# monkey0head/RePlay_cql

Measured on NVIDIA B200. Metric: CQL updates/sec (batch 1024), higher is better.
Workload: dtype f32 (f16x3: tensor-core fp16 hi/lo 3-term split with exact power-of-two row scales, fp32 accumulate, 1e-4 parity-gated)

## Files before the change

### replay_cql_b200/csrc/engine.cuh

```cuda
#pragma once
#include <cstdlib>
#include <vector>
#include <string>
#include "common.cuh"
#include "mlp_simt.cuh"
#include "dp_peer.cuh"
#include <nvtx3/nvToolsExt.h>

namespace cql {

constexpr int N_NOISE_PARTS = 8;

struct StepInfo {
  double bc1, bc2_sqrt;
  long long step;
};

struct NvtxRange {
  explicit NvtxRange(const char* name) { nvtxRangePushA(name); }
  ~NvtxRange() { nvtxRangePop(); }
  NvtxRange(const NvtxRange&) = delete;
  NvtxRange& operator=(const NvtxRange&) = delete;
};

struct Affine {
  int on;
  float off, den;
};
struct Prep {
  Affine obs[2];
  Affine act;
  Affine rew;
  __host__ __device__ bool any() const { return obs[0].on | obs[1].on | act.on | rew.on; }
};
__device__ __forceinline__ float prep_fwd(const Affine& p, float x) {
  return p.on ? __fdiv_rn(__fsub_rn(x, p.off), p.den) : x;
}
__device__ __forceinline__ float act_fwd(const Affine& p, float a) {
  return p.on ? __fsub_rn(__fmul_rn(__fdiv_rn(__fsub_rn(a, p.off), p.den), 2.f), 1.f) : a;
}
__device__ __forceinline__ float act_rev(const Affine& p, float a) {
  return p.on ? __fadd_rn(__fmul_rn(__fdiv_rn(__fadd_rn(a, 1.f), 2.f), p.den), p.off) : a;
}
__device__ __forceinline__ float4 prep_row0(const Prep& p, float4 r) {
  return make_float4(prep_fwd(p.obs[0], r.x), prep_fwd(p.obs[1], r.y), act_fwd(p.act, r.z), prep_fwd(p.rew, r.w));
}
__device__ __forceinline__ float4 prep_row1(const Prep& p, float4 r) {
  return make_float4(prep_fwd(p.obs[0], r.x), prep_fwd(p.obs[1], r.y), r.z, r.w);
}

constexpr int STATS_MAX_BLOCKS = 1024;
constexpr size_t STATS_DEV_DOUBLES = (STATS_MAX_BLOCKS + 1) * 4 * 5;

struct Switches {
  int skip;
  bool no_pdl;
  bool no_pair;
  bool no_pair_bwd1;
  bool no_pair_bwd2;
  bool no_pair_bwd2_small;
  bool no_small;
  bool no_fold;
  bool no_fused_adam;
  bool no_fork;
  int big_fork;
  int h2_cost;
  int pair_swap;
  int dp_debug;
  bool no_fused_dp;
};
inline const Switches& switches() {
  static const Switches s = [] {
    auto set = [](const char* name) { return std::getenv(name) != nullptr; };
    auto num = [](const char* name, int unset) { const char* v = std::getenv(name); return v ? std::atoi(v) : unset; };
    Switches w{};
    w.skip = num("CQL_SKIP", 0);
    w.no_pdl = set("CQL_NO_PDL");
    w.no_pair = set("CQL_NO_PAIR");
    w.no_pair_bwd1 = set("CQL_NO_PAIR_BWD1");
    w.no_pair_bwd2 = set("CQL_NO_PAIR_BWD2");
    w.no_pair_bwd2_small = set("CQL_NO_PAIR_BWD2_SMALL");
    w.no_small = set("CQL_NO_SMALL");
    w.no_fold = set("CQL_NO_FOLD");
    w.no_fused_adam = set("CQL_NO_FUSED_ADAM");
    w.no_fork = set("CQL_NO_FORK");
    w.big_fork = num("CQL_BIG_FORK", -1);
    w.h2_cost = num("CQL_H2_COST", 0);
    w.pair_swap = num("CQL_PAIR_SWAP", 0);
    w.dp_debug = num("CQL_DP_DEBUG", 0);
    w.no_fused_dp = set("CQL_NO_FUSED_DP");
    return w;
  }();
  return s;
}

struct MdpSession;
int64_t seen_csr_on_device(struct Handle& h, const int32_t* users_h, const int32_t* items_h, int64_t n, int64_t n_users,
                           const uint8_t* wanted_h, int64_t* indptr_d, int32_t* seen_d, cudaStream_t st);
void mdp_session_free(MdpSession*);

struct Handle {
  cql_config cfg{};
  std::string err;
  cudaStream_t own_stream = nullptr;
  cudaStream_t side_stream = nullptr;
  cudaEvent_t ev_fork = nullptr, ev_join = nullptr;
  int num_sms = 148;
  int64_t launches = 0;

  float* params = nullptr;
  float* adam_m = nullptr;
  float* adam_v = nullptr;
  float* grads = nullptr;
  long long* step_dev = nullptr;
  StepInfo* stepinfo = nullptr;
  float* metrics = nullptr;
  float* metrics_host = nullptr;

  float* table = nullptr;
  int64_t n_trans = 0;
  int n_steps = 1;
  int64_t table_cap = 0;
  bool table_sharded = false;
  int64_t sample_pos_host = 0;
  long long* sample_pos = nullptr;
  cql_table_stats stats{};
  double* stats_dev = nullptr;
  double* stats_host = nullptr;
  bool stats_pending = false;
  bool stats_rew_ok = false;
  cql_preprocessing prep_cfg{};
  Prep prep{};

  int B = 0, n = 0, C = 0;
  int rsA = 0, rsC = 0;
  float* batch = nullptr;
  float* batch_host = nullptr;
  float* batch_in = nullptr;
  float* noise = nullptr;
  float* noise_host = nullptr;
  int64_t noise_floats = 0;
  float4* XA = nullptr;
  float* outA = nullptr;
  float* h2A = nullptr;
  float4* XAl = nullptr;
  float* offAl = nullptr;
  float* QAl = nullptr;
  float4* XC = nullptr;
  float* offC = nullptr;
  float* QC = nullptr;
  float* h2C = nullptr;
  float* dQ = nullptr;
  float4* XT = nullptr;
  float* QT = nullptr;
  float4* XP = nullptr;
  float* QP = nullptr;
  float* h2P = nullptr;
  float* dQP = nullptr;
  float4* dXP = nullptr;
  float* dOutA = nullptr;
  float* perb = nullptr;
  float* pairv = nullptr;
  float* loss_sums = nullptr;
  float* actor_part = nullptr;
  float* smallC = nullptr;
  float* smallA = nullptr;
  float* pw2C = nullptr;
  float* pw2A = nullptr;
  int splitsC = 1, splitsA = 1;

  uint8_t* packed_fwd = nullptr;
  size_t packed_net_bytes = 0;
  size_t packed_net_bytes_bwd = 0;
  float* part = nullptr;
  size_t part_floats = 0;
  uint8_t* packed_bwd = nullptr;
  float* small1 = nullptr;
  float* small2 = nullptr;
  float* pw2_tc = nullptr;
  float4* dX_part = nullptr;
  int slots1 = 0, splits_tc = 0, tc_slices = 1;
  uint8_t* packed_fwd2 = nullptr;
  uint8_t* packed_bwd2 = nullptr;
  size_t packed_net_bytes2 = 0;
  DpPeer dp;
  bool dp_fused = false;
  int* w2max = nullptr;
  int* ap_wmax = nullptr;
  int pair_swap_b = 0;

  bool timing = false;
  bool pdl_off = false;
  cudaEvent_t ev[16] = {};

  MdpSession* mdp = nullptr;
  uint8_t* mdp_ring = nullptr;
  std::vector<void*> allocs;

  template <typename T>
  T* dalloc(size_t count) {
    void* p = nullptr;
    CQL_CUDA(cudaMalloc(&p, count * sizeof(T)));
    CQL_CUDA(cudaMemset(p, 0, count * sizeof(T)));
    allocs.push_back(p);
    return reinterpret_cast<T*>(p);
  }
  void free_all() {
    for (void* p : allocs) cudaFree(p);
    allocs.clear();
    if (mdp) { mdp_session_free(mdp); mdp = nullptr; }
    if (mdp_ring) { cudaFreeHost(mdp_ring); mdp_ring = nullptr; }
    if (table) { cudaFree(table); table = nullptr; table_cap = 0; }
    if (metrics_host) { cudaFreeHost(metrics_host); metrics_host = nullptr; }
    if (batch_host) { cudaFreeHost(batch_host); batch_host = nullptr; }
    if (stats_host) { cudaFreeHost(stats_host); stats_host = nullptr; }
    if (noise_host) { cudaFreeHost(noise_host); noise_host = nullptr; }
    if (own_stream) { cudaStreamDestroy(own_stream); own_stream = nullptr; }
    if (side_stream) { cudaStreamDestroy(side_stream); side_stream = nullptr; }
    if (ev_fork) { cudaEventDestroy(ev_fork); ev_fork = nullptr; }
    if (ev_join) { cudaEventDestroy(ev_join); ev_join = nullptr; }
    for (auto& e : ev) if (e) { cudaEventDestroy(e); e = nullptr; }
  }

  float* staged_batch() const { return prep.any() ? batch_in : batch; }
  float* net_params(int slot) const { return params + (size_t)slot * NET_STRIDE; }
  float* scalars() const { return params + scalars_off(C); }
  float* g_actor() const { return grads; }
  float* g_critics() const { return grads + NET_STRIDE; }
  float* g_scalars() const { return grads + (size_t)(1 + C) * NET_STRIDE; }
};

void mdp_begin(Handle& h, int64_t n);
void mdp_append(Handle& h, int col, int dtype, const void* host, int64_t count);
int64_t mdp_finish(Handle& h, int top_k, float noise_scale, float* obs_out, float* act_out, float* rew_out, float* term_out,
                   int64_t* order_out);

inline void ensure_table(Handle& h, int64_t n) {
  h.n_trans = 0;
  h.stats = cql_table_stats{};
  h.stats_pending = false;
  if (h.table != nullptr && h.table_cap >= n) return;
  if (h.table) { CQL_CUDA(cudaFree(h.table)); h.table = nullptr; h.table_cap = 0; }
  CQL_CUDA(cudaMalloc(&h.table, (size_t)n * 8 * sizeof(float)));
  h.table_cap = n;
}

void expand_n_steps(Handle& h, const float* one_step, int64_t n, cudaStream_t st);
int table_stats(Handle& h, const float* rows, int64_t n, bool rew_ok, cudaStream_t st);

inline void mark(Handle* h, cudaStream_t st, int i) {
  if (h->timing) CQL_CUDA(cudaEventRecord(h->ev[i], st));
}

inline cudaStream_t pick_stream(Handle* h, void* stream) {
  return stream ? reinterpret_cast<cudaStream_t>(stream) : h->own_stream;
}

#define CQL_LAUNCH_CHECK(h)                 \
  do {                                      \
    (h)->launches++;                        \
    CQL_CUDA(cudaGetLastError());           \
  } while (0)

}
```

### replay_cql_b200/csrc/mlp_tc.cuh

```cuda
#pragma once
#include "tc_common.cuh"
#include "engine.cuh"

namespace cql {
namespace tc {

constexpr int TM = 128;

template <bool TF32>
struct Cfg {
  static constexpr int ES = TF32 ? 4 : 2;
  static constexpr int EPC = 16 / ES;
  static constexpr int UK = 32 / ES;
  static constexpr int TERMS = TF32 ? 2 : 1;
  static constexpr int NS = TF32 ? 64 : 256;
  static constexpr int SLICES = H / NS;
  static constexpr uint32_t B_TERM_BYTES = NS * H * ES;
  static constexpr uint32_t B_BYTES = TERMS * B_TERM_BYTES;
  static constexpr uint32_t TMEM_COLS = 2 * NS < 32 ? 32 : 2 * NS;
  static constexpr size_t PACKED_NET_BYTES = (size_t)SLICES * B_BYTES;
};

template <bool TF32, int NPW>
struct Pipe : Cfg<TF32> {
  using C = Cfg<TF32>;
  static constexpr int KC = TF32 ? 16 : 64;
  static constexpr int STAGES = TF32 ? 5 : 4;
  static constexpr int PIECES = KC / C::EPC;
  static constexpr int GROUPS = NPW / PIECES;
  static constexpr int NCHUNK = H / KC;
  static constexpr uint32_t A_TERM_BYTES = TM * KC * C::ES;
  static constexpr uint32_t A_STAGE_BYTES = C::TERMS * A_TERM_BYTES;
  static constexpr int MMA_WARP = 4 + NPW;
  static constexpr int THREADS = (5 + NPW) * 32;
  static constexpr int PROD_THREADS = NPW * 32;
};
constexpr int FWD_NPW = 16;
constexpr int BWD1_NPW = 8;

template <bool TF32, bool TRANSPOSE>
__global__ void k_pack_w2(const float* __restrict__ params, int in_dim, int n_nets, uint8_t* __restrict__ packed) {
  using C = Cfg<TF32>;
  const int net = blockIdx.y;
  const int c = blockIdx.x * blockDim.x + threadIdx.x;
  if (net >= n_nets || c >= H * (H / C::EPC)) return;
  const int n = c / (H / C::EPC), kc = c % (H / C::EPC);
  const float* W2 = params + (size_t)net * NET_STRIDE + off_W2(in_dim);
  float v[C::EPC];
#pragma unroll
  for (int i = 0; i < C::EPC; ++i) {
    const int k = kc * C::EPC + i;
    v[i] = TRANSPOSE ? W2[(size_t)k * H + n] : W2[(size_t)n * H + k];
  }
  const int slice = n / C::NS, nl = n % C::NS;
  uint8_t* base = packed + (size_t)net * C::PACKED_NET_BYTES + (size_t)slice * C::B_BYTES + chunk_off(C::NS, nl, kc);
  if (TF32) {
    float4 h, l;
    split_tf32(v[0], h.x, l.x); split_tf32(v[1], h.y, l.y); split_tf32(v[2], h.z, l.z); split_tf32(v[3], h.w, l.w);
    *reinterpret_cast<float4*>(base) = h;
    *reinterpret_cast<float4*>(base + C::B_TERM_BYTES) = l;
  } else {
    __nv_bfloat162 p[4];
#pragma unroll
    for (int i = 0; i < 4; ++i) p[i] = __floats2bfloat162_rn(v[2 * i], v[2 * i + 1]);
    *reinterpret_cast<uint4*>(base) = *reinterpret_cast<uint4*>(p);
  }
}

struct PackJobs {
  struct J { const float* net; uint8_t* dst; int in_dim, transpose; } j[12];
  int n;
};
template <bool TF32>
__global__ void k_pack_multi(const PackJobs jobs) {
  using C = Cfg<TF32>;
  const PackJobs::J jb = jobs.j[blockIdx.y];
  const int c = blockIdx.x * blockDim.x + threadIdx.x;
  if (c >= H * (H / C::EPC)) return;
  const int n = c / (H / C::EPC), kc = c % (H / C::EPC);
  const float* W2 = jb.net + off_W2(jb.in_dim);
  float v[C::EPC];
#pragma unroll
  for (int i = 0; i < C::EPC; ++i) {
    const int k = kc * C::EPC + i;
    v[i] = jb.transpose ? W2[(size_t)k * H + n] : W2[(size_t)n * H + k];
  }
  const int slice = n / C::NS, nl = n % C::NS;
  uint8_t* base = jb.dst + (size_t)slice * C::B_BYTES + chunk_off(C::NS, nl, kc);
  if constexpr (TF32) {
    float4 h, l;
    split_tf32(v[0], h.x, l.x); split_tf32(v[1], h.y, l.y); split_tf32(v[2], h.z, l.z); split_tf32(v[3], h.w, l.w);
    *reinterpret_cast<float4*>(base) = h;
    *reinterpret_cast<float4*>(base + C::B_TERM_BYTES) = l;
  } else {
    __nv_bfloat162 p[4];
#pragma unroll
    for (int i = 0; i < 4; ++i) p[i] = __floats2bfloat162_rn(v[2 * i], v[2 * i + 1]);
    *reinterpret_cast<uint4*>(base) = *reinterpret_cast<uint4*>(p);
  }
}

struct TcFwdJob {
  const float4* X;
  const float* params;
  const uint8_t* packed;
  float* out_part;
  float* h2;
  int rows, n_nets;
};
struct TcFwdJobs {
  TcFwdJob j[3];
  int n;
  int item_begin[4];
  int h2_cost = 0;
};

struct ItemInfo { int job, net, slice, tile, pair_id; };

template <bool TF32>
__device__ __forceinline__ ItemInfo decode_item(const TcFwdJobs& jobs, int item) {
  using C = Cfg<TF32>;
  ItemInfo it;
  it.job = 0;
  while (it.job + 1 < jobs.n && item >= jobs.item_begin[it.job + 1]) ++it.job;
  const int local = item - jobs.item_begin[it.job];
  const int tiles = (jobs.j[it.job].rows + TM - 1) / TM;
  const int pair = local / tiles;
  it.tile = local % tiles;
  it.net = pair / C::SLICES;
  it.slice = pair % C::SLICES;
  it.pair_id = it.job * 64 + pair;
  return it;
}

template <bool TF32, int NPW>
struct FwdSmem {
  using C = Pipe<TF32, NPW>;
  static constexpr uint32_t OFF_B = 0;
  static constexpr uint32_t OFF_A = C::B_BYTES;
  static constexpr uint32_t OFF_W1 = OFF_A + C::STAGES * C::A_STAGE_BYTES;
  static constexpr uint32_t OFF_EB = OFF_W1 + H * 16;
  static constexpr uint32_t OFF_BAR = OFF_EB + C::NS * 16;
  static constexpr uint32_t N_BARS = 2 * C::STAGES + 4 + 2;
  static constexpr uint32_t OFF_SLOT = OFF_BAR + N_BARS * 8;
  static constexpr uint32_t BYTES = OFF_SLOT + 16;
};

__device__ __forceinline__ float2 ffma2(float2 a, float2 b, float2 c) {
  float2 d;
  asm("{\n\t.reg .b64 ra, rb, rc, rd;\n\tmov.b64 ra, {%2, %3};\n\tmov.b64 rb, {%4, %5};\n\tmov.b64 rc, {%6, %7};\n\t"
      "fma.rn.f32x2 rd, ra, rb, rc;\n\tmov.b64 {%0, %1}, rd;\n\t}"
      : "=f"(d.x), "=f"(d.y)
      : "f"(a.x), "f"(a.y), "f"(b.x), "f"(b.y), "f"(c.x), "f"(c.y));
  return d;
}
__device__ __forceinline__ void split_tf32_fast(float x, float& hi, float& lo) {
  hi = rn_tf32(x);
  lo = x - hi;
}

template <bool TF32, int IN, int OUT>
__global__ void __launch_bounds__(Pipe<TF32, FWD_NPW>::THREADS, 1) tc_fwd_kernel(const TcFwdJobs jobs) {
  using C = Pipe<TF32, FWD_NPW>;
  using S = FwdSmem<TF32, FWD_NPW>;
  extern __shared__ __align__(1024) uint8_t sm[];
  uint8_t* Bs = sm + S::OFF_B;
  uint8_t* As = sm + S::OFF_A;
  float4* w1s = reinterpret_cast<float4*>(sm + S::OFF_W1);
  float4* ebs = reinterpret_cast<float4*>(sm + S::OFF_EB);
  uint64_t* bars = reinterpret_cast<uint64_t*>(sm + S::OFF_BAR);
  uint64_t* full = bars;
  uint64_t* empty = bars + C::STAGES;
  uint64_t* tfull = bars + 2 * C::STAGES;
  uint64_t* tempty = tfull + 2;
  uint64_t* bload = tempty + 2;
  uint64_t* drain = bload + 1;
  uint32_t* slot = reinterpret_cast<uint32_t*>(sm + S::OFF_SLOT);

  const int tid = threadIdx.x, warp = tid >> 5, lane = tid & 31;
  const int total = jobs.item_begin[jobs.n];
  const int item_lo = (int)((long long)total * blockIdx.x / gridDim.x);
  const int item_hi = (int)((long long)total * (blockIdx.x + 1) / gridDim.x);

  if (warp == C::MMA_WARP) {
    tmem_alloc(slot, C::TMEM_COLS);
    if (lane == 0) {
      for (int s = 0; s < C::STAGES; ++s) { mbar_init(&full[s], C::PIECES); mbar_init(&empty[s], 1); }
      for (int a = 0; a < 2; ++a) { mbar_init(&tfull[a], 1); mbar_init(&tempty[a], 4); }
      mbar_init(bload, 1);
      mbar_init(drain, 1);
      fence_mbar_init();
    }
  }
  tc_fence_before();
  __syncthreads();
  tc_fence_after();
  const uint32_t tmem = *slot;

  if (warp == C::MMA_WARP) {
    {
      const uint32_t idesc = instr_desc(TF32 ? FMT_TF32 : FMT_BF16, TM, C::NS);
      const uint32_t a_lbo = TM * 16, b_lbo = C::NS * 16;
      const uint32_t b_base = smem_u32(Bs);
      int cur_pair = -1;
      uint32_t it = 0, nb = 0, nd = 0, tcount = 0;
      for (int item = item_lo; item < item_hi; ++item) {
        const ItemInfo ii = decode_item<TF32>(jobs, item);
        if (ii.pair_id != cur_pair) {
          if (cur_pair >= 0) {
            if (elect_one()) umma_commit(drain);
            __syncwarp();
            mbar_wait(drain, nd & 1);
            ++nd;
          }
          const TcFwdJob& jb = jobs.j[ii.job];
          const uint8_t* src = jb.packed + (size_t)ii.net * C::PACKED_NET_BYTES + (size_t)ii.slice * C::B_BYTES;
          if (elect_one()) {
            mbar_arrive_expect_tx(bload, C::B_BYTES);
            for (uint32_t o = 0; o < C::B_BYTES; o += 32768) bulk_g2s(Bs + o, src + o, 32768, bload);
          }
          __syncwarp();
          mbar_wait(bload, nb & 1);
          ++nb;
          cur_pair = ii.pair_id;
        }
        const uint32_t acc = tcount & 1;
        mbar_wait(&tempty[acc], ((tcount >> 1) & 1) ^ 1);
        tc_fence_after();
        const uint32_t d_tmem = tmem + acc * C::NS;
        for (int c = 0; c < C::NCHUNK; ++c, ++it) {
          const uint32_t s = it % C::STAGES;
          mbar_wait(&full[s], (it / C::STAGES) & 1);
          tc_fence_after();
          const uint32_t a_base = smem_u32(As + s * C::A_STAGE_BYTES);
          if (elect_one()) {
#pragma unroll
          for (int j = 0; j < C::KC / C::UK; ++j) {
            const uint32_t g = c * (C::KC / C::UK) + j;
            const uint64_t a_hi = smem_desc(a_base + 2 * j * a_lbo, a_lbo, 128);
            const uint64_t b_hi = smem_desc(b_base + 2 * g * b_lbo, b_lbo, 128);
            const uint32_t first = (c == 0 && j == 0) ? 0u : 1u;
            if constexpr (TF32) {
              const uint64_t a_lo = smem_desc(a_base + C::A_TERM_BYTES + 2 * j * a_lbo, a_lbo, 128);
              const uint64_t b_lo = smem_desc(b_base + C::B_TERM_BYTES + 2 * g * b_lbo, b_lbo, 128);
              umma<TF32>(d_tmem, a_lo, b_hi, idesc, first);
              umma<TF32>(d_tmem, a_hi, b_lo, idesc, 1u);
              umma<TF32>(d_tmem, a_hi, b_hi, idesc, 1u);
            } else {
              umma<TF32>(d_tmem, a_hi, b_hi, idesc, first);
            }
          }
          umma_commit(&empty[s]);
          if (c == C::NCHUNK - 1) umma_commit(&tfull[acc]);
          }
          __syncwarp();
        }
        ++tcount;
      }
    }
  } else if (warp >= 4) {
    const int pw = warp - 4, ptid = tid - 128;
    int cur_pair = -1, cur_netkey = -1;
    uint32_t it = 0;
    for (int item = item_lo; item < item_hi; ++item) {
      const ItemInfo ii = decode_item<TF32>(jobs, item);
      const TcFwdJob& jb = jobs.j[ii.job];
      const int netkey = ii.job * 64 + ii.net;
// ... 154 lines not shown
```

### replay_cql_b200/csrc/mlp_tc_bwd1.cuh

```cuda
#pragma once
#include "mlp_tc.cuh"
#include "mlp_tc_ts.cuh"

namespace cql {
namespace tc {

struct Bwd1Job {
  const float4* X;
  const float* dOut;
  const float* h2;
  const float* params;
  const uint8_t* packedT;
  float* small1;
  float4* dX_part;
  int rows, n_nets, slots;
  const float* q_part = nullptr;
  int q_parts = 0;
  float dq_scale = 0.f;
  int zero_small1 = 0;
};
template <int IN>
__device__ __forceinline__ void zero_small1_slots(const Bwd1Job& jb, int per_cta) {
  if (!jb.zero_small1) return;
  constexpr int NF4 = off_W2(IN) / 4;
  for (int net = 0; net < jb.n_nets; ++net)
    for (int s = 0; s < per_cta; ++s) {
      float4* o = reinterpret_cast<float4*>(jb.small1 + ((size_t)net * jb.slots + (size_t)blockIdx.x * per_cta + s) * SMALL_STRIDE);
      for (int f = threadIdx.x; f < NF4; f += blockDim.x) o[f] = make_float4(0.f, 0.f, 0.f, 0.f);
    }
  __syncthreads();
}
template <int IN, int OUT>
__device__ __forceinline__ float actor_dq_of(const Bwd1Job& jb, int net_i, int r) {
  constexpr int MAXP = 8;
  int arg = 0;
  float qm = 0.f;
  for (int c = 0; c < jb.n_nets; ++c) {
    float part[MAXP];
#pragma unroll
    for (int p = 0; p < MAXP; ++p)
      if (p < jb.q_parts) part[p] = __ldg(jb.q_part + ((size_t)c * jb.q_parts + p) * jb.rows + r);
    const float bias = __ldg(jb.params + (size_t)c * NET_STRIDE + off_b3(IN, OUT));
    float v = 0.f;
#pragma unroll
    for (int p = 0; p < MAXP; ++p)
      if (p < jb.q_parts) v += part[p];
    const float q = v + bias;
    if (c == 0 || q < qm) { qm = q; arg = c; }
  }
  return net_i == arg ? jb.dq_scale : 0.f;
}

__device__ __forceinline__ float warp_reduce_scatter32(float (&v)[32]) {
  const int lane = threadIdx.x & 31;
#pragma unroll
  for (int off = 16; off >= 1; off >>= 1) {
    const bool upper = (lane & off) != 0;
#pragma unroll
    for (int i = 0; i < off; ++i) {
      const float send = upper ? v[i] : v[i + off];
      const float keep = upper ? v[i + off] : v[i];
      v[i] = keep + __shfl_xor_sync(0xffffffffu, send, off);
    }
  }
  return v[0];
}

template <bool TF32, int IN, int OUT, bool WGRADS, bool DX>
__global__ void __launch_bounds__(Pipe<TF32, BWD1_NPW>::THREADS, 1) tc_bwd1_kernel(const Bwd1Job jb) {
  using C = Pipe<TF32, BWD1_NPW>;
  using S = FwdSmem<TF32, BWD1_NPW>;
  extern __shared__ __align__(1024) uint8_t sm[];
  uint8_t* Bs = sm + S::OFF_B;
  uint8_t* As = sm + S::OFF_A;
  float2* w3s = reinterpret_cast<float2*>(sm + S::OFF_W1);
  float4* ebs = reinterpret_cast<float4*>(sm + S::OFF_EB);
  uint64_t* bars = reinterpret_cast<uint64_t*>(sm + S::OFF_BAR);
  uint64_t* full = bars;
  uint64_t* empty = bars + C::STAGES;
  uint64_t* tfull = bars + 2 * C::STAGES;
  uint64_t* tempty = tfull + 2;
  uint64_t* bload = tempty + 2;
  uint64_t* drain = bload + 1;
  uint32_t* slot = reinterpret_cast<uint32_t*>(sm + S::OFF_SLOT);

  const int tid = threadIdx.x, warp = tid >> 5, lane = tid & 31;
  const int tiles = (jb.rows + TM - 1) / TM;
  const int tiles64 = (jb.rows + 63) / 64;
  const int total = jb.n_nets * C::SLICES * tiles;
  const int item_lo = (int)((long long)total * blockIdx.x / gridDim.x);
  const int item_hi = (int)((long long)total * (blockIdx.x + 1) / gridDim.x);

  if (warp == C::MMA_WARP) {
    tmem_alloc(slot, C::TMEM_COLS);
    if (lane == 0) {
      for (int s = 0; s < C::STAGES; ++s) { mbar_init(&full[s], C::PIECES); mbar_init(&empty[s], 1); }
      for (int a = 0; a < 2; ++a) { mbar_init(&tfull[a], 1); mbar_init(&tempty[a], 4); }
      mbar_init(bload, 1);
      mbar_init(drain, 1);
      fence_mbar_init();
    }
  }
  tc_fence_before();
  __syncthreads();
  tc_fence_after();
  const uint32_t tmem = *slot;

  if (warp == C::MMA_WARP) {
    {
      const uint32_t idesc = instr_desc(TF32 ? FMT_TF32 : FMT_BF16, TM, C::NS);
      const uint32_t a_lbo = TM * 16, b_lbo = C::NS * 16;
      const uint32_t b_base = smem_u32(Bs);
      int cur_pair = -1;
      uint32_t it = 0, nb = 0, nd = 0, tcount = 0;
      for (int item = item_lo; item < item_hi; ++item) {
        const int pair = item / tiles;
        if (pair != cur_pair) {
          if (cur_pair >= 0) { if (elect_one()) umma_commit(drain); __syncwarp(); mbar_wait(drain, nd & 1); ++nd; }
          const uint8_t* src = jb.packedT + (size_t)(pair / C::SLICES) * C::PACKED_NET_BYTES + (size_t)(pair % C::SLICES) * C::B_BYTES;
          if (elect_one()) {
            mbar_arrive_expect_tx(bload, C::B_BYTES);
            for (uint32_t o = 0; o < C::B_BYTES; o += 32768) bulk_g2s(Bs + o, src + o, 32768, bload);
          }
          __syncwarp();
          mbar_wait(bload, nb & 1);
          ++nb;
          cur_pair = pair;
        }
        const uint32_t acc = tcount & 1;
        mbar_wait(&tempty[acc], ((tcount >> 1) & 1) ^ 1);
        tc_fence_after();
        const uint32_t d_tmem = tmem + acc * C::NS;
        for (int c = 0; c < C::NCHUNK; ++c, ++it) {
          const uint32_t s = it % C::STAGES;
          mbar_wait(&full[s], (it / C::STAGES) & 1);
          tc_fence_after();
          const uint32_t a_base = smem_u32(As + s * C::A_STAGE_BYTES);
          if (elect_one()) {
#pragma unroll
          for (int j = 0; j < C::KC / C::UK; ++j) {
            const uint32_t g = c * (C::KC / C::UK) + j;
            const uint64_t a_hi = smem_desc(a_base + 2 * j * a_lbo, a_lbo, 128);
            const uint64_t b_hi = smem_desc(b_base + 2 * g * b_lbo, b_lbo, 128);
            const uint32_t first = (c == 0 && j == 0) ? 0u : 1u;
            if constexpr (TF32) {
              const uint64_t a_lo = smem_desc(a_base + C::A_TERM_BYTES + 2 * j * a_lbo, a_lbo, 128);
              const uint64_t b_lo = smem_desc(b_base + C::B_TERM_BYTES + 2 * g * b_lbo, b_lbo, 128);
              umma<TF32>(d_tmem, a_lo, b_hi, idesc, first);
              umma<TF32>(d_tmem, a_hi, b_lo, idesc, 1u);
              umma<TF32>(d_tmem, a_hi, b_hi, idesc, 1u);
            } else {
              umma<TF32>(d_tmem, a_hi, b_hi, idesc, first);
            }
          }
          umma_commit(&empty[s]);
          if (c == C::NCHUNK - 1) umma_commit(&tfull[acc]);
          }
          __syncwarp();
        }
        ++tcount;
      }
    }
  } else if (warp >= 4) {
    const int pw = warp - 4, ptid = tid - 128;
    int cur_net = -1;
    uint32_t it = 0;
    for (int item = item_lo; item < item_hi; ++item) {
      const int pair = item / tiles, tile = item % tiles, net_i = pair / C::SLICES;
      if (net_i != cur_net) {
        cur_net = net_i;
        asm volatile("bar.sync 1, %0;" ::"n"(C::PROD_THREADS));
        const float* net = jb.params + (size_t)net_i * NET_STRIDE;
// ... 482 lines not shown
```

### replay_cql_b200/csrc/mlp_tc_bwd2.cuh

```cuda
#pragma once
#include "tc_common.cuh"
#include "mlp_simt.cuh"

namespace cql {
namespace tc {

constexpr int B2_PROD_WARPS = 8;
constexpr int B2_THREADS = (B2_PROD_WARPS + 1) * 32;

template <bool TF32>
struct B2Cfg {
  static constexpr int ES = TF32 ? 4 : 2;
  static constexpr int EPC = 16 / ES;
  static constexpr int UK = 32 / ES;
  static constexpr int TERMS = TF32 ? 2 : 1;
  static constexpr int RS = TF32 ? 16 : 64;
  static constexpr int STAGES = 3;
  static constexpr uint32_t OP_TERM_BYTES = H * RS * ES;
  static constexpr uint32_t OP_BYTES = TERMS * OP_TERM_BYTES;
  static constexpr uint32_t STAGE_BYTES = 2 * OP_BYTES;
  static constexpr uint32_t OFF_X = STAGES * STAGE_BYTES;
  static constexpr uint32_t OFF_DO = OFF_X + STAGES * RS * 16;
  static constexpr uint32_t OFF_BAR = OFF_DO + STAGES * RS * 8;
  static constexpr uint32_t OFF_SLOT = OFF_BAR + (2 * STAGES + 1) * 8;
  static constexpr uint32_t BYTES = OFF_SLOT + 16;
};

struct Bwd2Job {
  const float4* X;
  const float* dOut;
  const float* h2;
  const float* params;
  float* pw2;
  float* small2;
  int rows, n_nets, splits;
};

template <bool TF32, int IN, int OUT>
__global__ void __launch_bounds__(B2_THREADS, 1) tc_bwd2_kernel(const Bwd2Job jb) {
  using C = B2Cfg<TF32>;
  extern __shared__ __align__(1024) uint8_t sm[];
  float4* xs = reinterpret_cast<float4*>(sm + C::OFF_X);
  float* dos = reinterpret_cast<float*>(sm + C::OFF_DO);
  uint64_t* full = reinterpret_cast<uint64_t*>(sm + C::OFF_BAR);
  uint64_t* empty = full + C::STAGES;
  uint64_t* done = empty + C::STAGES;
  uint32_t* slot = reinterpret_cast<uint32_t*>(sm + C::OFF_SLOT);
  const int tid = threadIdx.x, warp = tid >> 5, lane = tid & 31;
  const int split = blockIdx.x, net_i = blockIdx.y;
  const float* net = jb.params + (size_t)net_i * NET_STRIDE;
  const int tiles64 = (jb.rows + 63) / 64;
  const int n_stage_total = (jb.rows + C::RS - 1) / C::RS;
  const int st_lo = (int)((long long)n_stage_total * split / jb.splits);
  const int st_hi = (int)((long long)n_stage_total * (split + 1) / jb.splits);

  if (warp == B2_PROD_WARPS) {
    tmem_alloc(slot, 512);
    if (lane == 0) {
      for (int s = 0; s < C::STAGES; ++s) { mbar_init(&full[s], B2_PROD_WARPS); mbar_init(&empty[s], 1); }
      mbar_init(done, 1);
      fence_mbar_init();
    }
  }
  tc_fence_before();
  __syncthreads();
  tc_fence_after();
  const uint32_t tmem = *slot;

  if (warp == B2_PROD_WARPS) {
    {
      const uint32_t idesc = instr_desc(TF32 ? FMT_TF32 : FMT_BF16, 128, 256);
      const uint32_t lbo = H * 16;
      uint32_t it = 0;
      for (int sg = st_lo; sg < st_hi; ++sg, ++it) {
        const uint32_t s = it % C::STAGES;
        mbar_wait(&full[s], (it / C::STAGES) & 1);
        tc_fence_after();
        const uint32_t a_base = smem_u32(sm + s * C::STAGE_BYTES);
        const uint32_t b_base = a_base + C::OP_BYTES;
        if (elect_one()) {
#pragma unroll
        for (int half = 0; half < 2; ++half) {
#pragma unroll
          for (int j = 0; j < C::RS / C::UK; ++j) {
            const uint32_t acc = (it == 0 && j == 0) ? 0u : 1u;
            const uint64_t a_hi = smem_desc(a_base + half * 2048 + 2 * j * lbo, lbo, 128);
            const uint64_t b_hi = smem_desc(b_base + 2 * j * lbo, lbo, 128);
            const uint32_t d = tmem + half * 256;
            if constexpr (TF32) {
              const uint64_t a_lo = smem_desc(a_base + C::OP_TERM_BYTES + half * 2048 + 2 * j * lbo, lbo, 128);
              const uint64_t b_lo = smem_desc(b_base + C::OP_TERM_BYTES + 2 * j * lbo, lbo, 128);
              umma<TF32>(d, a_lo, b_hi, idesc, acc);
              umma<TF32>(d, a_hi, b_lo, idesc, 1u);
              umma<TF32>(d, a_hi, b_hi, idesc, 1u);
            } else {
              umma<TF32>(d, a_hi, b_hi, idesc, acc);
            }
          }
        }
        umma_commit(&empty[s]);
        if (sg == st_hi - 1) umma_commit(done);
        }
        __syncwarp();
      }
    }
  } else {
    const int t = tid;
    float w3[OUT];
#pragma unroll
    for (int o = 0; o < OUT; ++o) w3[o] = net[off_W3(IN) + o * H + t];
    const float w1x = net[off_W1(IN) + t * IN], w1y = net[off_W1(IN) + t * IN + 1];
    const float w1z = IN == 3 ? net[off_W1(IN) + t * IN + 2] : 0.f;
    const float b1v = net[off_b1(IN) + t];
    float s_db2 = 0.f, s_dw3[OUT], s_db3[OUT];
#pragma unroll
    for (int o = 0; o < OUT; ++o) { s_dw3[o] = 0.f; s_db3[o] = 0.f; }
    uint32_t it = 0;
    constexpr int NV = C::RS / 4;
    constexpr bool PREFETCH = NV <= 4;
    float4 hnext[PREFETCH ? NV : 1];
    auto h2_ptr = [&](int sg) {
      const int row0 = sg * C::RS;
      return jb.h2 + (((size_t)net_i * tiles64 + (row0 >> 6)) * H + t) * 64 + (row0 & 63);
    };
    if (PREFETCH && st_lo < st_hi) {
      const float* hp = h2_ptr(st_lo);
#pragma unroll
      for (int q = 0; q < NV; ++q) hnext[q] = __ldg(reinterpret_cast<const float4*>(hp) + q);
    }
    for (int sg = st_lo; sg < st_hi; ++sg, ++it) {
      const uint32_t s = it % C::STAGES;
      float4 hcur[PREFETCH ? NV : 1];
      if (PREFETCH) {
#pragma unroll
        for (int q = 0; q < NV; ++q) hcur[q] = hnext[q];
        if (sg + 1 < st_hi) {
          const float* hp = h2_ptr(sg + 1);
#pragma unroll
          for (int q = 0; q < NV; ++q) hnext[q] = __ldg(reinterpret_cast<const float4*>(hp) + q);
        }
      }
      mbar_wait(&empty[s], ((it / C::STAGES) & 1) ^ 1);
      const int row0 = sg * C::RS;
      float4* xst = xs + s * C::RS;
      float* dost = dos + s * C::RS * 2;
      if (t < C::RS) {
        const int r = row0 + t;
        xst[t] = r < jb.rows ? __ldg(jb.X + r) : make_float4(0.f, 0.f, 0.f, 0.f);
#pragma unroll
        for (int o = 0; o < OUT; ++o)
          dost[t * 2 + o] = r < jb.rows ? __ldg(jb.dOut + ((size_t)net_i * jb.rows + r) * OUT + o) : 0.f;
      }
      asm volatile("bar.sync 1, 256;");
      uint8_t* Ast = sm + s * C::STAGE_BYTES;
      uint8_t* Bst = Ast + C::OP_BYTES;
      const float* h2p = h2_ptr(sg);
#pragma unroll
      for (int kc = 0; kc < C::RS / C::EPC; ++kc) {
        float hv[C::EPC], dz[C::EPC], h1[C::EPC];
        if constexpr (C::EPC == 8) {
          const float4 p0 = __ldg(reinterpret_cast<const float4*>(h2p + kc * 8));
          const float4 p1 = __ldg(reinterpret_cast<const float4*>(h2p + kc * 8 + 4));
          hv[0] = p0.x; hv[1] = p0.y; hv[2] = p0.z; hv[3] = p0.w;
          hv[4] = p1.x; hv[5] = p1.y; hv[6] = p1.z; hv[7] = p1.w;
        } else {
          const float4 p0 = PREFETCH ? hcur[kc % NV] : __ldg(reinterpret_cast<const float4*>(h2p + kc * 4));
          hv[0] = p0.x; hv[1] = p0.y; hv[2] = p0.z; hv[3] = p0.w;
        }
#pragma unroll
        for (int e = 0; e < C::EPC; ++e) {
          const int rl = kc * C::EPC + e;
          float g = 0.f;
#pragma unroll
          for (int o = 0; o < OUT; ++o) {
            const float d = dost[rl * 2 + o];
            g = fmaf(d, w3[o], g);
            s_dw3[o] = fmaf(d, hv[e], s_dw3[o]);
            if (t == 0) s_db3[o] += d;
          }
          dz[e] = hv[e] > 0.f ? g : 0.f;
          s_db2 += dz[e];
          const float4 x = xst[rl];
          float z = fmaf(x.y, w1y, x.x * w1x);
          if (IN == 3) z = fmaf(x.z, w1z, z);
          h1[e] = fmaxf(z + b1v, 0.f);
        }
        const uint32_t off = chunk_off(H, t, kc);
        if constexpr (TF32) {
// ... 63 lines not shown
```

### replay_cql_b200/csrc/mlp_tc_h.cuh

```cuda
#pragma once
#include <cuda_fp16.h>
#include "mlp_tc.cuh"
#include "mlp_tc_bwd1.cuh"
#include "mlp_tc_bwd2.cuh"

namespace cql {
namespace tc {

template <int NEW_, int NS_ = 128>
struct HCfgT {
  static constexpr int ES = 2, EPC = 8, UK = 16;
  static constexpr int NS = NS_;
  static constexpr int SLICES = H / NS;
  static constexpr int NPW = 16;
  static constexpr int KC = 64;
  static constexpr int STAGES = 4;
  static constexpr int NCHUNK = H / KC;
  static constexpr int KPW = KC / (NPW / 4);
  static constexpr int NEW = NEW_;
  static constexpr int MMA_WARP = NEW + NPW;
  static constexpr int THREADS = (NEW + 1 + NPW) * 32;
  static constexpr int PROD_THREADS = NPW * 32;
  static constexpr uint32_t B_TERM_BYTES = NS * H * ES;
  static constexpr uint32_t B_BYTES = 2 * B_TERM_BYTES;
  static constexpr size_t META_OFF = (size_t)SLICES * B_BYTES;
  static constexpr size_t PACKED_NET_BYTES = META_OFF + 2048;
  static constexpr uint32_t A_COL0 = 256;
  static constexpr uint32_t A_STAGE_COLS = KC;
  static constexpr uint32_t A_LO_COLS = KC / 2;
  static constexpr uint32_t TMEM_ALLOC = 512;
  static constexpr uint32_t OFF_B = 0;
  static constexpr uint32_t OFF_W1 = B_BYTES;
  static constexpr uint32_t OFF_EB = OFF_W1 + H * 16;
  static constexpr uint32_t OFF_BAR = OFF_EB + 2 * NS * 16;
  static constexpr uint32_t N_BARS = 2 * STAGES + 4 + 2;
  static constexpr uint32_t OFF_SLOT = OFF_BAR + N_BARS * 8;
  static constexpr uint32_t OFF_FLUSH = OFF_SLOT + 16;
  static constexpr uint32_t OFF_RED = OFF_FLUSH + 2 * 4 * 16 * 32 * 4;
  static constexpr uint32_t RED_WARP_BYTES = 32 * 33 * 4 + 32 * 16;
  static constexpr uint32_t SMEM_BYTES = OFF_RED + NEW_ * RED_WARP_BYTES;
};
using HCfg = HCfgT<8>;
using HCfgS = HCfgT<8, 32>;
using HCfg4 = HCfgT<4>;

template <class C>
__device__ __forceinline__ void load_operand_slice(uint8_t* Bs, const uint8_t* packed_net, int slice, uint64_t* bar) {
  if constexpr (C::NS == HCfg::NS) {
    const uint8_t* src = packed_net + (size_t)slice * HCfg::B_BYTES;
    mbar_arrive_expect_tx(bar, C::B_BYTES);
    for (uint32_t o = 0; o < C::B_BYTES; o += 32768) bulk_g2s(Bs + o, src + o, 32768, bar);
  } else {
    constexpr int PER = HCfg::NS / C::NS;
    const uint8_t* src = packed_net + (size_t)(slice / PER) * HCfg::B_BYTES + (size_t)(slice % PER) * (C::NS * 16);
    mbar_arrive_expect_tx(bar, C::B_BYTES);
    for (int term = 0; term < 2; ++term)
      for (int kc = 0; kc < H / 8; ++kc)
        bulk_g2s(Bs + term * C::B_TERM_BYTES + kc * (C::NS * 16), src + (size_t)term * HCfg::B_TERM_BYTES + (size_t)kc * (HCfg::NS * 16),
                 C::NS * 16, bar);
  }
}

struct HMeta {
  float inv_s[H];
  float wmax[8];
};

__device__ __forceinline__ void pow2_scale(float bound, float& s, float& inv_s) {
  int e = (int)((__float_as_uint(bound) >> 23) & 0xffu);
  e = max(e, 20);
  s = __uint_as_float((uint32_t)(268 - e) << 23);
  inv_s = __uint_as_float((uint32_t)(e - 14) << 23);
}

__device__ __forceinline__ void split_h2(float x0, float x1, uint32_t& hi, uint32_t& lo) {
  const __half2 h = __floats2half2_rn(x0, x1);
  const float2 hf = __half22float2(h);
  const __half2 l = __floats2half2_rn(x0 - hf.x, x1 - hf.y);
  hi = *reinterpret_cast<const uint32_t*>(&h);
  lo = *reinterpret_cast<const uint32_t*>(&l);
}

__device__ __forceinline__ void split_h2_trunc(float2 x, uint32_t& hi, uint32_t& lo) {
  const float h0 = __uint_as_float(__float_as_uint(x.x) & 0xFFFFE000u);
  const float h1 = __uint_as_float(__float_as_uint(x.y) & 0xFFFFE000u);
  float2 l;
  asm("{\n\t.reg .b64 ra, rb, rd;\n\tmov.b64 ra, {%2, %3};\n\tmov.b64 rb, {%4, %5};\n\t"
      "sub.rn.f32x2 rd, ra, rb;\n\tmov.b64 {%0, %1}, rd;\n\t}"
      : "=f"(l.x), "=f"(l.y)
      : "f"(x.x), "f"(x.y), "f"(h0), "f"(h1));
  const __half2 hh = __floats2half2_rn(h0, h1);
  const __half2 ll = __floats2half2_rn(l.x, l.y);
  hi = *reinterpret_cast<const uint32_t*>(&hh);
  lo = *reinterpret_cast<const uint32_t*>(&ll);
}

__device__ __forceinline__ float2 fmul2(float2 a, float2 b) {
  float2 d;
  asm("{\n\t.reg .b64 ra, rb, rd;\n\tmov.b64 ra, {%2, %3};\n\tmov.b64 rb, {%4, %5};\n\t"
      "mul.rn.f32x2 rd, ra, rb;\n\tmov.b64 {%0, %1}, rd;\n\t}"
      : "=f"(d.x), "=f"(d.y)
      : "f"(a.x), "f"(a.y), "f"(b.x), "f"(b.y));
  return d;
}

__global__ void __launch_bounds__(256) k_pack_multi_h(const PackJobs jobs, int out_dim_actor) {
  tc::grid_dep_wait();
 
  using C = HCfg;
  const PackJobs::J jb = jobs.j[blockIdx.y];
  const int c = blockIdx.x * blockDim.x + threadIdx.x;
  const int n = c >> 5, kc = c & 31;
  const float* W2 = jb.net + off_W2(jb.in_dim);
  float v[8];
  float mx = 0.f;
#pragma unroll
  for (int i = 0; i < 8; ++i) {
    const int k = kc * 8 + i;
    v[i] = jb.transpose ? W2[(size_t)k * H + n] : W2[(size_t)n * H + k];
    mx = fmaxf(mx, fabsf(v[i]));
  }
#pragma unroll
  for (int o = 16; o > 0; o >>= 1) mx = fmaxf(mx, __shfl_xor_sync(0xffffffffu, mx, o));
  float s, inv_s;
  pow2_scale(mx, s, inv_s);
  uint32_t hi[4], lo[4];
#pragma unroll
  for (int i = 0; i < 4; ++i) split_h2(v[2 * i] * s, v[2 * i + 1] * s, hi[i], lo[i]);
  const int slice = n / C::NS, nl = n % C::NS;
  uint8_t* base = jb.dst + (size_t)slice * C::B_BYTES + chunk_off(C::NS, nl, kc);
  *reinterpret_cast<uint4*>(base) = make_uint4(hi[0], hi[1], hi[2], hi[3]);
  *reinterpret_cast<uint4*>(base + C::B_TERM_BYTES) = make_uint4(lo[0], lo[1], lo[2], lo[3]);
  HMeta* meta = reinterpret_cast<HMeta*>(jb.dst + C::META_OFF);
  if (kc == 0) meta->inv_s[n] = inv_s;
  if (blockIdx.x == 0) {
    __shared__ int wm[8];
    if (threadIdx.x < 8) wm[threadIdx.x] = 0;
    __syncthreads();
    const int out_dim = jb.in_dim == 2 ? out_dim_actor : 1;
    const int k = threadIdx.x;
    const float* W1 = jb.net + off_W1(jb.in_dim);
    for (int cc = 0; cc < jb.in_dim; ++cc) atomicMax(&wm[cc], __float_as_int(fabsf(W1[k * jb.in_dim + cc])));
    atomicMax(&wm[3], __float_as_int(fabsf(jb.net[off_b1(jb.in_dim) + k])));
    for (int o = 0; o < out_dim; ++o) atomicMax(&wm[4 + o], __float_as_int(fabsf(jb.net[off_W3(jb.in_dim) + o * H + k])));
    __syncthreads();
    if (threadIdx.x < 8) meta->wmax[threadIdx.x] = __int_as_float(wm[threadIdx.x]);
  }
}

constexpr int FWD_H2_COST = 13;

struct HItem { int job, net, slice, tile, pair_id; };
template <int SLICES = HCfg::SLICES>
__device__ __forceinline__ HItem decode_item_h(const TcFwdJobs& jobs, int item) {
  HItem it;
  it.job = 0;
  while (it.job + 1 < jobs.n && item >= jobs.item_begin[it.job + 1]) ++it.job;
  const int local = item - jobs.item_begin[it.job];
  const int tiles = (jobs.j[it.job].rows + TM - 1) / TM;
  const int pair = local / tiles;
  it.tile = local % tiles;
  it.net = pair / SLICES;
  it.slice = pair % SLICES;
  it.pair_id = it.job * 64 + pair;
  return it;
}

__device__ __forceinline__ float h1_row_bound(const float4& x, const float4& wm) {
  return fmaf(fabsf(x.x), wm.x, fmaf(fabsf(x.y), wm.y, fmaf(fabsf(x.z), wm.z, wm.w)));
}

template <int IN, int OUT, class C = HCfg>
__global__ void __launch_bounds__(HCfg::THREADS, 1) tc_fwd_h_kernel(const TcFwdJobs jobs) {
  extern __shared__ __align__(1024) uint8_t sm[];
  uint8_t* Bs = sm + C::OFF_B;
  float4* w1p = reinterpret_cast<float4*>(sm + C::OFF_W1);
  float4* ebs = reinterpret_cast<float4*>(sm + C::OFF_EB);
  uint64_t* bars = reinterpret_cast<uint64_t*>(sm + C::OFF_BAR);
  uint64_t* full = bars;
  uint64_t* empty = bars + C::STAGES;
  uint64_t* tfull = bars + 2 * C::STAGES;
  uint64_t* tempty = tfull + 2;
  uint64_t* bload = tempty + 2;
  uint64_t* drain = bload + 1;
  uint32_t* slot = reinterpret_cast<uint32_t*>(sm + C::OFF_SLOT);

  const int tid = threadIdx.x, warp = tid >> 5, lane = tid & 31;
  int item_lo, item_hi;
  {
    long long cb[4];
    int wj[3];
    cb[0] = 0;
    for (int j = 0; j < jobs.n; ++j) {
      wj[j] = jobs.j[j].h2 != nullptr ? (jobs.h2_cost > 0 ? jobs.h2_cost : FWD_H2_COST) : 10;
      cb[j + 1] = cb[j] + (long long)(jobs.item_begin[j + 1] - jobs.item_begin[j]) * wj[j];
    }
    auto item_at = [&](long long cost) {
      int j = 0;
      while (j + 1 < jobs.n && cost >= cb[j + 1]) ++j;
      const int it = jobs.item_begin[j] + (int)((cost - cb[j]) / wj[j]);
      return it < jobs.item_begin[j + 1] ? it : jobs.item_begin[j + 1];
    };
    const long long total_cost = cb[jobs.n];
    item_lo = blockIdx.x == 0 ? 0 : item_at(total_cost * blockIdx.x / gridDim.x);
    item_hi = blockIdx.x == gridDim.x - 1 ? jobs.item_begin[jobs.n] : item_at(total_cost * (blockIdx.x + 1) / gridDim.x);
  }

  if (warp == C::MMA_WARP) {
    tmem_alloc(slot, C::TMEM_ALLOC);
    if (lane == 0) {
      for (int s = 0; s < C::STAGES; ++s) { mbar_init(&full[s], C::NPW); mbar_init(&empty[s], 1); }
      for (int a = 0; a < 2; ++a) { mbar_init(&tfull[a], 1); mbar_init(&tempty[a], 4); }
      mbar_init(bload, 1);
      mbar_init(drain, 1);
      fence_mbar_init();
    }
  }
  tc_fence_before();
  __syncthreads();
  tc_fence_after();
  const uint32_t tmem = *slot;
  grid_dep_wait();

  if (warp == C::MMA_WARP) {
    const uint32_t idesc = instr_desc(FMT_F16, TM, C::NS);
    const uint32_t b_lbo = C::NS * 16;
    const uint32_t b_base = smem_u32(Bs);
    int cur_pair = -1;
    uint32_t it = 0, nb = 0, nd = 0, tcount = 0;
    for (int item = item_lo; item < item_hi; ++item) {
      const HItem ii = decode_item_h<C::SLICES>(jobs, item);
      if (ii.pair_id != cur_pair) {
        if (cur_pair >= 0) {
          if (elect_one()) umma_commit(drain);
          __syncwarp();
          mbar_wait(drain, nd & 1);
          ++nd;
        }
        const TcFwdJob& jb = jobs.j[ii.job];
        if (elect_one()) load_operand_slice<C>(Bs, jb.packed + (size_t)ii.net * HCfg::PACKED_NET_BYTES, ii.slice, bload);
        __syncwarp();
        mbar_wait(bload, nb & 1);
        ++nb;
        cur_pair = ii.pair_id;
      }
      const uint32_t acc = tcount & 1;
      mbar_wait(&tempty[acc], ((tcount >> 1) & 1) ^ 1);
      tc_fence_after();
      const uint32_t d_tmem = tmem + acc * C::NS;
      for (int c = 0; c < C::NCHUNK; ++c, ++it) {
        const uint32_t s = it % C::STAGES;
        mbar_wait(&full[s], (it / C::STAGES) & 1);
        tc_fence_after();
        if (elect_one()) {
          const uint32_t a_stage = tmem + C::A_COL0 + s * C::A_STAGE_COLS;
#pragma unroll
          for (int j = 0; j < C::KC / C::UK; ++j) {
            const uint32_t g = c * (C::KC / C::UK) + j;
            const uint64_t b_hi = smem_desc(b_base + 2 * g * b_lbo, b_lbo, 128);
            const uint64_t b_lo = smem_desc(b_base + C::B_TERM_BYTES + 2 * g * b_lbo, b_lbo, 128);
            const uint32_t a_hi = a_stage + j * 8, a_lo = a_hi + C::A_LO_COLS;
            umma_ts<false>(d_tmem, a_lo, b_hi, idesc, (c == 0 && j == 0) ? 0u : 1u);
            umma_ts<false>(d_tmem, a_hi, b_lo, idesc, 1u);
            umma_ts<false>(d_tmem, a_hi, b_hi, idesc, 1u);
          }
          umma_commit(&empty[s]);
          if (c == C::NCHUNK - 1) umma_commit(&tfull[acc]);
        }
        __syncwarp();
      }
      ++tcount;
    }
  } else if (warp >= C::NEW) {
    const int pw = warp - C::NEW, ptid = tid - C::NEW * 32;
    const int kq = pw >> 2;
    const uint32_t lane_base = tmem + ((uint32_t)((warp & 3) * 32) << 16) + C::A_COL0 + kq * (C::KPW / 2);
    int cur_netkey = -1;
    float4 wm = make_float4(0.f, 0.f, 0.f, 0.f);
    uint32_t it = 0;
    auto load_x = [&](const HItem& ni) {
      const TcFwdJob& nj = jobs.j[ni.job];
      const int r = ni.tile * TM + (warp & 3) * 32 + lane;
      return r < nj.rows ? __ldg(nj.X + r) : make_float4(0.f, 0.f, 0.f, 0.f);
    };
    float4 x_next = make_float4(0.f, 0.f, 0.f, 0.f);
    HItem ii_next = item_lo < item_hi ? decode_item_h<C::SLICES>(jobs, item_lo) : HItem{};
    for (int item = item_lo; item < item_hi; ++item) {
      const HItem ii = ii_next;
      if (item + 1 < item_hi) ii_next = decode_item_h<C::SLICES>(jobs, item + 1);
      const TcFwdJob& jb = jobs.j[ii.job];
      const int netkey = ii.job * 64 + ii.net;
      if (netkey != cur_netkey) {
        cur_netkey = netkey;
        asm volatile("bar.sync 1, %0;" ::"n"(C::PROD_THREADS));
        const float* net = jb.params + (size_t)ii.net * NET_STRIDE;
        for (int pr = ptid; pr < H / 2; pr += C::PROD_THREADS) {
          const int k = 2 * pr;
          const float* wa = net + off_W1(IN) + k * IN;
          const float* wb = wa + IN;
          w1p[2 * pr] = make_float4(wa[0], wb[0], wa[1], wb[1]);
          w1p[2 * pr + 1] = make_float4(IN == 3 ? wa[2] : 0.f, IN == 3 ? wb[2] : 0.f, net[off_b1(IN) + k], net[off_b1(IN) + k + 1]);
        }
        const HMeta* meta = reinterpret_cast<const HMeta*>(jb.packed + (size_t)ii.net * HCfg::PACKED_NET_BYTES + HCfg::META_OFF);
        wm = make_float4(__ldg(&meta->wmax[0]), __ldg(&meta->wmax[1]), IN == 3 ? __ldg(&meta->wmax[2]) : 0.f, __ldg(&meta->wmax[3]));
        asm volatile("bar.sync 1, %0;" ::"n"(C::PROD_THREADS));
      }
      const float4 x = (item == item_lo) ? load_x(ii) : x_next;
      if (item + 1 < item_hi) x_next = load_x(ii_next);
      float sa, inv_sa;
      pow2_scale(h1_row_bound(x, wm), sa, inv_sa);
      const float2 xx = make_float2(x.x, x.x), xy = make_float2(x.y, x.y), xz = make_float2(x.z, x.z), ss = make_float2(sa, sa);
      for (int c = 0; c < C::NCHUNK; ++c, ++it) {
        const uint32_t s = it % C::STAGES;
        uint32_t hi[C::KPW / 2], lo[C::KPW / 2];
#pragma unroll
        for (int pp = 0; pp < C::KPW / 2; ++pp) {
          const int pr = (c * C::KC + kq * C::KPW) / 2 + pp;
          const float4 wA = w1p[2 * pr], wB = w1p[2 * pr + 1];
          float2 v = ffma2(xx, make_float2(wA.x, wA.y), make_float2(wB.z, wB.w));
          v = ffma2(xy, make_float2(wA.z, wA.w), v);
          if (IN == 3) v = ffma2(xz, make_float2(wB.x, wB.y), v);
          v = fmul2(make_float2(fmaxf(v.x, 0.f), fmaxf(v.y, 0.f)), ss);
          split_h2_trunc(v, hi[pp], lo[pp]);
        }
        mbar_wait(&empty[s], ((it / C::STAGES) & 1) ^ 1);
        tc_fence_after();
        tmem_st8(lane_base + s * C::A_STAGE_COLS, hi);
        tmem_st8(lane_base + s * C::A_STAGE_COLS + C::A_LO_COLS, lo);
        tmem_st_wait();
        tc_fence_before();
        __syncwarp();
        if (lane == 0) mbar_arrive(&full[s]);
      }
    }
  } else {
    const int grp = warp >> 2, qw = warp & 3, gtid = tid & 127;
    float4* ebg = ebs + grp * C::NS;
    float2* efg = reinterpret_cast<float2*>(sm + C::OFF_FLUSH) + grp * C::NS;
    int cur_pair = -1;
    const int row_in_tile = qw * 32 + lane;
    float4 wm = make_float4(0.f, 0.f, 0.f, 0.f);
    for (int item = item_lo + grp; item < item_hi; item += 2) {
      const uint32_t tcount = (uint32_t)(item - item_lo);
      const HItem ii = decode_item_h<C::SLICES>(jobs, item);
      const TcFwdJob& jb = jobs.j[ii.job];
      if (ii.pair_id != cur_pair) {
        cur_pair = ii.pair_id;
        asm volatile("bar.sync %0, 128;" ::"r"(2 + grp));
        const float* net = jb.params + (size_t)ii.net * NET_STRIDE;
        const HMeta* meta = reinterpret_cast<const HMeta*>(jb.packed + (size_t)ii.net * HCfg::PACKED_NET_BYTES + HCfg::META_OFF);
        for (int cidx = gtid; cidx < C::NS; cidx += 128) {
          const int col = ii.slice * C::NS + cidx;
          const float inv_n = __ldg(&meta->inv_s[col]);
          ebg[cidx] = make_float4(net[off_b2(IN) + col], net[off_W3(IN) + col],
                                  OUT == 2 ? net[off_W3(IN) + H + col] : 0.f, inv_n);
          if (OUT == 1) efg[cidx] = make_float2(net[off_b2(IN) + col] / inv_n, net[off_W3(IN) + col] * inv_n);
        }
        wm = make_float4(__ldg(&meta->wmax[0]), __ldg(&meta->wmax[1]), IN == 3 ? __ldg(&meta->wmax[2]) : 0.f, __ldg(&meta->wmax[3]));
        asm volatile("bar.sync %0, 128;" ::"r"(2 + grp));
      }
      const uint32_t acc = grp;
      const int row = ii.tile * TM + row_in_tile;
      const float4 x = row < jb.rows ? __ldg(jb.X + row) : make_float4(0.f, 0.f, 0.f, 0.f);
      float sa, inv_sa;
      pow2_scale(h1_row_bound(x, wm), sa, inv_sa);
      mbar_wait(&tfull[acc], (tcount >> 1) & 1);
      tc_fence_after();
      const bool store_h2 = jb.h2 != nullptr;
      const int tiles64 = (jb.rows + 63) / 64;
      float* h2row = store_h2 ? jb.h2 + (((size_t)ii.net * tiles64 + (row >> 6)) * H + ii.slice * C::NS) * 64 + (row & 63)
                              : nullptr;
      float q0 = 0.f, q1 = 0.f;
      if (OUT == 1 && !store_h2) {
#pragma unroll 1
        for (int c0 = 0; c0 < C::NS; c0 += 32) {
          float v[32];
          tmem_ld32(tmem + ((uint32_t)(qw * 32) << 16) + acc * C::NS + c0, v);
          tmem_ld_wait();
#pragma unroll
          for (int i = 0; i < 32; i += 2) {
            const float4 e = reinterpret_cast<const float4*>(efg)[(c0 + i) >> 1];
            q0 = fmaf(fmaxf(fmaf(v[i], inv_sa, e.x), 0.f), e.y, q0);
            q0 = fmaf(fmaxf(fmaf(v[i + 1], inv_sa, e.z), 0.f), e.w, q0);
          }
        }
      } else
#pragma unroll 1
      for (int c0 = 0; c0 < C::NS; c0 += 32) {
        float v[32];
        tmem_ld32(tmem + ((uint32_t)(qw * 32) << 16) + acc * C::NS + c0, v);
        tmem_ld_wait();
#pragma unroll
        for (int i = 0; i < 32; ++i) {
          const float4 e = ebg[c0 + i];
          const float hv = fmaxf(fmaf(v[i] * inv_sa, e.w, e.x), 0.f);
          v[i] = hv;
          q0 = fmaf(hv, e.y, q0);
          if (OUT == 2) q1 = fmaf(hv, e.z, q1);
        }
        if (store_h2 && (row >> 6) < tiles64) {
#pragma unroll
          for (int i = 0; i < 32; ++i) h2row[(size_t)(c0 + i) * 64] = v[i];
        }
      }
      tc_fence_before();
      __syncwarp();
      if (lane == 0) mbar_arrive(&tempty[acc]);
      if (row < jb.rows) {
        float* o = jb.out_part + (((size_t)ii.net * C::SLICES + ii.slice) * jb.rows + row) * OUT;
        o[0] = q0;
        if (OUT == 2) o[1] = q1;
      }
    }
  }
  tc_fence_before();
  __syncthreads();
  if (warp == C::MMA_WARP) tmem_dealloc(tmem, C::TMEM_ALLOC);
}


template <int IN, int OUT, bool WGRADS, bool DX, class C = HCfg>
__global__ void __launch_bounds__(HCfg::THREADS, 1) tc_bwd1_h_kernel(const Bwd1Job jb) {
  extern __shared__ __align__(1024) uint8_t sm[];
  uint8_t* Bs = sm + C::OFF_B;
  float2* w3s = reinterpret_cast<float2*>(sm + C::OFF_W1);
  float4* ebs = reinterpret_cast<float4*>(sm + C::OFF_EB);
  float* invs = reinterpret_cast<float*>(sm + C::OFF_W1 + H * 8);
  uint64_t* bars = reinterpret_cast<uint64_t*>(sm + C::OFF_BAR);
  uint64_t* full = bars;
  uint64_t* empty = bars + C::STAGES;
  uint64_t* tfull = bars + 2 * C::STAGES;
  uint64_t* tempty = tfull + 2;
  uint64_t* bload = tempty + 2;
  uint64_t* drain = bload + 1;
  uint32_t* slot = reinterpret_cast<uint32_t*>(sm + C::OFF_SLOT);

  const int tid = threadIdx.x, warp = tid >> 5, lane = tid & 31;
  const int tiles = (jb.rows + TM - 1) / TM;
  const int tiles64 = (jb.rows + 63) / 64;
  const int total = jb.n_nets * C::SLICES * tiles;
  const int item_lo = (int)((long long)total * blockIdx.x / gridDim.x);
  const int item_hi = (int)((long long)total * (blockIdx.x + 1) / gridDim.x);

  if (warp == C::MMA_WARP) {
    tmem_alloc(slot, C::TMEM_ALLOC);
    if (lane == 0) {
      for (int s = 0; s < C::STAGES; ++s) { mbar_init(&full[s], C::NPW); mbar_init(&empty[s], 1); }
      for (int q = 0; q < 2; ++q) { mbar_init(&tfull[q], 1); mbar_init(&tempty[q], 4); }
      mbar_init(bload, 1);
      mbar_init(drain, 1);
      fence_mbar_init();
    }
  }
  tc_fence_before();
  __syncthreads();
  tc_fence_after();
  const uint32_t tmem = *slot;
  grid_dep_wait();
  if (WGRADS) zero_small1_slots<IN>(jb, 2);

  if (warp == C::MMA_WARP) {
    const uint32_t idesc = instr_desc(FMT_F16, TM, C::NS);
    const uint32_t b_lbo = C::NS * 16;
    const uint32_t b_base = smem_u32(Bs);
    int cur_pair = -1;
    uint32_t it = 0, nb = 0, nd = 0, tcount = 0;
    for (int item = item_lo; item < item_hi; ++item) {
      const int pair = item / tiles;
      if (pair != cur_pair) {
        if (cur_pair >= 0) { if (elect_one()) umma_commit(drain); __syncwarp(); mbar_wait(drain, nd & 1); ++nd; }
        if (elect_one()) load_operand_slice<C>(Bs, jb.packedT + (size_t)(pair / C::SLICES) * HCfg::PACKED_NET_BYTES, pair % C::SLICES, bload);
        __syncwarp();
        mbar_wait(bload, nb & 1);
        ++nb;
        cur_pair = pair;
      }
      const uint32_t acc = tcount & 1;
      mbar_wait(&tempty[acc], ((tcount >> 1) & 1) ^ 1);
      tc_fence_after();
      const uint32_t d_tmem = tmem + acc * C::NS;
      for (int c = 0; c < C::NCHUNK; ++c, ++it) {
        const uint32_t s = it % C::STAGES;
        mbar_wait(&full[s], (it / C::STAGES) & 1);
        tc_fence_after();
        if (elect_one()) {
          const uint32_t a_stage = tmem + C::A_COL0 + s * C::A_STAGE_COLS;
#pragma unroll
          for (int j = 0; j < C::KC / C::UK; ++j) {
            const uint32_t g = c * (C::KC / C::UK) + j;
            const uint64_t b_hi = smem_desc(b_base + 2 * g * b_lbo, b_lbo, 128);
            const uint64_t b_lo = smem_desc(b_base + C::B_TERM_BYTES + 2 * g * b_lbo, b_lbo, 128);
            const uint32_t a_hi = a_stage + j * 8, a_lo = a_hi + C::A_LO_COLS;
            umma_ts<false>(d_tmem, a_lo, b_hi, idesc, (c == 0 && j == 0) ? 0u : 1u);
            umma_ts<false>(d_tmem, a_hi, b_lo, idesc, 1u);
            umma_ts<false>(d_tmem, a_hi, b_hi, idesc, 1u);
          }
          umma_commit(&empty[s]);
          if (c == C::NCHUNK - 1) umma_commit(&tfull[acc]);
        }
        __syncwarp();
      }
      ++tcount;
    }
  } else if (warp >= C::NEW) {
    const int pw = warp - C::NEW, ptid = tid - C::NEW * 32;
    const int kq = pw >> 2;
    const uint32_t lane_base = tmem + ((uint32_t)((warp & 3) * 32) << 16) + C::A_COL0 + kq * (C::KPW / 2);
    int cur_net = -1;
    float w3m0 = 0.f, w3m1 = 0.f;
    uint32_t it = 0;
    for (int item = item_lo; item < item_hi; ++item) {
      const int pair = item / tiles, tile = item % tiles, net_i = pair / C::SLICES;
      if (net_i != cur_net) {
        cur_net = net_i;
        asm volatile("bar.sync 1, %0;" ::"n"(C::PROD_THREADS));
        const float* net = jb.params + (size_t)net_i * NET_STRIDE;
        for (int j = ptid; j < H; j += C::PROD_THREADS)
          w3s[j] = make_float2(net[off_W3(IN) + j], OUT == 2 ? net[off_W3(IN) + H + j] : 0.f);
        const HMeta* meta = reinterpret_cast<const HMeta*>(jb.packedT + (size_t)net_i * HCfg::PACKED_NET_BYTES + HCfg::META_OFF);
        w3m0 = __ldg(&meta->wmax[4]);
        w3m1 = OUT == 2 ? __ldg(&meta->wmax[5]) : 0.f;
        asm volatile("bar.sync 1, %0;" ::"n"(C::PROD_THREADS));
      }
      const int r = tile * TM + (warp & 3) * 32 + lane;
      const bool ok = r < jb.rows;
      float d0 = 0.f;
      if (OUT == 1 && DX && !WGRADS && jb.q_parts > 0) { if (ok) d0 = actor_dq_of<IN, OUT>(jb, net_i, r); }
      else if (ok) d0 = __ldg(jb.dOut + ((size_t)net_i * jb.rows + r) * OUT);
      const float d1 = (ok && OUT == 2) ? __ldg(jb.dOut + ((size_t)net_i * jb.rows + r) * OUT + 1) : 0.f;
      float sa, inv_sa;
      pow2_scale(fmaf(fabsf(d0), w3m0, fabsf(d1) * w3m1), sa, inv_sa);
      const float d0s = d0 * sa, d1s = d1 * sa;
      const int rc = ok ? r : 0;
      const float* h2r = jb.h2 + ((size_t)net_i * tiles64 + (rc >> 6)) * H * 64 + (rc & 63);
      float hn[C::KPW];
#pragma unroll
      for (int e = 0; e < C::KPW; ++e) hn[e] = __ldg(h2r + (size_t)(kq * C::KPW + e) * 64);
      for (int c = 0; c < C::NCHUNK; ++c, ++it) {
        const uint32_t s = it % C::STAGES;
        const int j0 = c * C::KC + kq * C::KPW;
        float hv[C::KPW];
#pragma unroll
        for (int e = 0; e < C::KPW; ++e) hv[e] = hn[e];
        if (c + 1 < C::NCHUNK) {
#pragma unroll
          for (int e = 0; e < C::KPW; ++e) hn[e] = __ldg(h2r + (size_t)(j0 + C::KC + e) * 64);
        }
        uint32_t hi[C::KPW / 2], lo[C::KPW / 2];
#pragma unroll
        for (int e = 0; e < C::KPW; e += 2) {
          const float2 wa = w3s[j0 + e], wb = w3s[j0 + e + 1];
          float ga = d0s * wa.x, gb = d0s * wb.x;
          if (OUT == 2) { ga = fmaf(d1s, wa.y, ga); gb = fmaf(d1s, wb.y, gb); }
          split_h2_trunc(make_float2(hv[e] > 0.f ? ga : 0.f, hv[e + 1] > 0.f ? gb : 0.f), hi[e / 2], lo[e / 2]);
        }
        mbar_wait(&empty[s], ((it / C::STAGES) & 1) ^ 1);
        tc_fence_after();
        tmem_st8(lane_base + s * C::A_STAGE_COLS, hi);
        tmem_st8(lane_base + s * C::A_STAGE_COLS + C::A_LO_COLS, lo);
        tmem_st_wait();
        tc_fence_before();
        __syncwarp();
        if (lane == 0) mbar_arrive(&full[s]);
      }
    }
  } else {
    constexpr int NCH = C::NS / 32;
    const int grp = warp >> 2, qw = warp & 3, gtid = tid & 127;
    float4* ebg = ebs + grp * C::NS;
    float* ivg = invs + grp * C::NS;
    float a_b[NCH], a_w0[NCH], a_w1[NCH], a_w2[NCH];
#pragma unroll
    for (int q = 0; q < NCH; ++q) { a_b[q] = 0.f; a_w0[q] = 0.f; a_w1[q] = 0.f; a_w2[q] = 0.f; }
    float* flbuf = reinterpret_cast<float*>(sm + C::OFF_FLUSH) + grp * (4 * 16 * 32);
    float* red_t = reinterpret_cast<float*>(sm + C::OFF_RED + warp * C::RED_WARP_BYTES);
    float4* red_x = reinterpret_cast<float4*>(red_t + 32 * 33);
    auto flush = [&](int pair) {
      if (!WGRADS || pair < 0) return;
      const int net_i = pair / C::SLICES, slice = pair % C::SLICES;
#pragma unroll
      for (int q = 0; q < NCH; ++q) {
        float* f = flbuf + (qw * 16 + q * 4) * 32 + lane;
        f[0] = a_w0[q]; f[32] = a_w1[q]; f[64] = a_w2[q]; f[96] = a_b[q];
        a_b[q] = 0.f; a_w0[q] = 0.f; a_w1[q] = 0.f; a_w2[q] = 0.f;
      }
      asm volatile("bar.sync %0, 128;" ::"r"(2 + grp));
      float* o = jb.small1 + ((size_t)net_i * jb.slots + blockIdx.x * 2 + grp) * SMALL_STRIDE;
      if (qw < NCH) {
        const int q = qw;
        float t0 = 0.f, t1 = 0.f, t2 = 0.f, t3 = 0.f;
#pragma unroll
        for (int w = 0; w < 4; ++w) {
          const float* f = flbuf + (w * 16 + q * 4) * 32 + lane;
          t0 += f[0]; t1 += f[32]; t2 += f[64]; t3 += f[96];
        }
        const int k = slice * C::NS + q * 32 + lane;
        o[k * IN + 0] = t0;
        o[k * IN + 1] = t1;
        if (IN == 3) o[k * IN + 2] = t2;
        o[H * IN + k] = t3;
      }
      asm volatile("bar.sync %0, 128;" ::"r"(2 + grp));
    };
    int cur_pair = -1;
    float w3m0 = 0.f, w3m1 = 0.f;
    for (int item = item_lo + grp; item < item_hi; item += 2) {
      const uint32_t tcount = (uint32_t)(item - item_lo);
      const int pair = item / tiles, tile = item % tiles, net_i = pair / C::SLICES, slice = pair % C::SLICES;
      if (pair != cur_pair) {
        flush(cur_pair);
        cur_pair = pair;
        asm volatile("bar.sync %0, 128;" ::"r"(2 + grp));
        const float* net = jb.params + (size_t)net_i * NET_STRIDE;
        const HMeta* meta = reinterpret_cast<const HMeta*>(jb.packedT + (size_t)net_i * HCfg::PACKED_NET_BYTES + HCfg::META_OFF);
        for (int cidx = gtid; cidx < C::NS; cidx += 128) {
          const int k = slice * C::NS + cidx;
          ebg[cidx] = make_float4(net[off_W1(IN) + k * IN], net[off_W1(IN) + k * IN + 1],
                                  IN == 3 ? net[off_W1(IN) + k * IN + 2] : 0.f, net[off_b1(IN) + k]);
          ivg[cidx] = __ldg(&meta->inv_s[k]);
        }
        w3m0 = __ldg(&meta->wmax[4]);
        w3m1 = OUT == 2 ? __ldg(&meta->wmax[5]) : 0.f;
        asm volatile("bar.sync %0, 128;" ::"r"(2 + grp));
      }
      const uint32_t acc = grp;
      const int row = tile * TM + qw * 32 + lane;
      const bool ok = row < jb.rows;
      const float4 x = ok ? __ldg(jb.X + row) : make_float4(0.f, 0.f, 0.f, 0.f);
      float d0 = 0.f;
      if (OUT == 1 && DX && !WGRADS && jb.q_parts > 0) { if (ok) d0 = actor_dq_of<IN, OUT>(jb, net_i, row); }
      else if (ok) d0 = __ldg(jb.dOut + ((size_t)net_i * jb.rows + row) * OUT);
      const float d1 = (ok && OUT == 2) ? __ldg(jb.dOut + ((size_t)net_i * jb.rows + row) * OUT + 1) : 0.f;
      float sa, inv_sa;
      pow2_scale(fmaf(fabsf(d0), w3m0, fabsf(d1) * w3m1), sa, inv_sa);
      if (WGRADS) {
        __syncwarp();
        red_x[lane] = x;
      }
      mbar_wait(&tfull[acc], (tcount >> 1) & 1);
      tc_fence_after();
      float dx0 = 0.f, dx1 = 0.f, dx2 = 0.f;
#pragma unroll
      for (int q = 0; q < NCH; ++q) {
        float v[32];
        tmem_ld32(tmem + ((uint32_t)(qw * 32) << 16) + acc * C::NS + q * 32, v);
        tmem_ld_wait();
#pragma unroll
        for (int i = 0; i < 32; ++i) {
          const float4 w = ebg[q * 32 + i];
          float z = fmaf(x.y, w.y, fmaf(x.x, w.x, w.w));
          if (IN == 3) z = fmaf(x.z, w.z, z);
          const float d = z > 0.f ? (DX ? v[i] * inv_sa * ivg[q * 32 + i] : v[i] * inv_sa) : 0.f;
          v[i] = d;
          if (DX) {
            dx0 = fmaf(d, w.x, dx0);
            dx1 = fmaf(d, w.y, dx1);
            if (IN == 3) dx2 = fmaf(d, w.z, dx2);
          }
        }
        if (WGRADS) {
          __syncwarp();
#pragma unroll
          for (int i = 0; i < 32; ++i) red_t[lane * 33 + i] = v[i];
          __syncwarp();
          float s0 = 0.f, s1 = 0.f, s2 = 0.f, sb = 0.f;
#pragma unroll 8
          for (int r = 0; r < 32; ++r) {
            const float dv = red_t[r * 33 + lane];
            const float4 xr = red_x[r];
            s0 = fmaf(dv, xr.x, s0);
            s1 = fmaf(dv, xr.y, s1);
            if (IN == 3) s2 = fmaf(dv, xr.z, s2);
            sb += dv;
          }
// ... 285 lines not shown
```

### replay_cql_b200/csrc/mlp_tc_h2.cuh

```cuda
#pragma once
#include "mlp_tc_h.cuh"

namespace cql {
namespace tc {

__device__ __forceinline__ uint32_t cluster_ctarank() {
  uint32_t r;
  asm volatile("mov.u32 %0, %%cluster_ctarank;" : "=r"(r));
  return r;
}
__device__ __forceinline__ void cluster_sync_all() {
  asm volatile("barrier.cluster.arrive.release.aligned;" ::: "memory");
  asm volatile("barrier.cluster.wait.acquire.aligned;" ::: "memory");
}
__device__ __forceinline__ void mbar_arrive_cluster(uint64_t* bar, uint32_t cta) {
  asm volatile(
      "{\n\t.reg .b32 ra;\n\tmapa.shared::cluster.u32 ra, %0, %1;\n\t"
      "mbarrier.arrive.shared::cluster.b64 _, [ra];\n\t}" ::"r"(smem_u32(bar)),
      "r"(cta)
      : "memory");
}
__device__ __forceinline__ void mbar_wait_cluster(uint64_t* bar, uint32_t parity) { mbar_wait(bar, parity); }
__device__ __forceinline__ void tmem_alloc2(uint32_t* smem_slot, uint32_t ncols) {
  asm volatile("tcgen05.alloc.cta_group::2.sync.aligned.shared::cta.b32 [%0], %1;" ::"r"(smem_u32(smem_slot)), "r"(ncols)
// ... 29 lines not shown
  asm("cvt.rn.relu.f16x2.f32 %0, %1, %2;" : "=r"(lo) : "f"(l.y), "f"(l.x));
}

struct H2Cfg {
  static constexpr int NPW = 16, NEW = 8;
  static constexpr int KC = 64, STAGES = 4, NCHUNK = H / KC, UK = 16;
  static constexpr int KPW = KC / (NPW / 4);
  static constexpr int NP = 128;
  static constexpr int NLOC = NP / 2;
  static constexpr int PASSES = H / NP;
  static constexpr int PARTS = 2 * PASSES;
  static constexpr int TMP = 2 * TM;
  static constexpr int MMA_WARP = NEW + NPW;
  static constexpr int THREADS = (NEW + NPW + 1) * 32;
  static constexpr int PROD_THREADS = NPW * 32;
  static constexpr uint32_t B_TERM_BYTES = NLOC * H * 2;
  static constexpr uint32_t B_PASS_BYTES = 2 * B_TERM_BYTES;
  static constexpr uint32_t B_BYTES = PASSES * B_PASS_BYTES;
  static constexpr size_t META_OFF = 2 * (size_t)B_BYTES;
  static constexpr size_t PACKED_NET_BYTES = META_OFF + 2048;
  static constexpr uint32_t A_COL0 = 256, A_STAGE_COLS = KC, A_LO_COLS = KC / 2;
  static constexpr uint32_t OFF_B = 0;
  static constexpr uint32_t OFF_W1 = B_BYTES;
  static constexpr uint32_t OFF_EB = OFF_W1 + H * 16;
  static constexpr uint32_t OFF_EF = OFF_EB + PASSES * NP * 16;
  static constexpr uint32_t OFF_BAR = OFF_EF + PASSES * NP * 8;
  static constexpr uint32_t N_BARS = 2 * STAGES + 2 + 2 + 3;
  static constexpr uint32_t OFF_SLOT = OFF_BAR + N_BARS * 8;
  static constexpr uint32_t SMEM_BYTES = OFF_SLOT + 16;
};

__host__ __device__ constexpr size_t pair_chunk_off(int n, int kc, int term) {
  return (size_t)((n & 127) >> 6) * H2Cfg::B_BYTES + (size_t)(n >> 7) * H2Cfg::B_PASS_BYTES +
         (size_t)term * H2Cfg::B_TERM_BYTES + chunk_off(H2Cfg::NLOC, n & 63, kc);
}

__global__ void __launch_bounds__(256) k_pack_pair_h(const PackJobs jobs, int out_dim_actor) {
  grid_dep_wait();
  using C = H2Cfg;
  const PackJobs::J jb = jobs.j[blockIdx.y];
  const int c = blockIdx.x * blockDim.x + threadIdx.x;
  const int n = c >> 5, kc = c & 31;
  const float* W2 = jb.net + off_W2(jb.in_dim);
  float v[8];
  float mx = 0.f;
#pragma unroll
  for (int i = 0; i < 8; ++i) {
    const int k = kc * 8 + i;
    v[i] = jb.transpose ? W2[(size_t)k * H + n] : W2[(size_t)n * H + k];
    mx = fmaxf(mx, fabsf(v[i]));
  }
#pragma unroll
  for (int o = 16; o > 0; o >>= 1) mx = fmaxf(mx, __shfl_xor_sync(0xffffffffu, mx, o));
  float s, inv_s;
  pow2_scale(mx, s, inv_s);
  uint32_t hi[4], lo[4];
#pragma unroll
  for (int i = 0; i < 4; ++i) split_h2(v[2 * i] * s, v[2 * i + 1] * s, hi[i], lo[i]);
  *reinterpret_cast<uint4*>(jb.dst + pair_chunk_off(n, kc, 0)) = make_uint4(hi[0], hi[1], hi[2], hi[3]);
  *reinterpret_cast<uint4*>(jb.dst + pair_chunk_off(n, kc, 1)) = make_uint4(lo[0], lo[1], lo[2], lo[3]);
  HMeta* meta = reinterpret_cast<HMeta*>(jb.dst + C::META_OFF);
  if (kc == 0) meta->inv_s[n] = inv_s;
  if (blockIdx.x == 0) {
    __shared__ int wm[8];
    if (threadIdx.x < 8) wm[threadIdx.x] = 0;
    __syncthreads();
    const int out_dim = jb.in_dim == 2 ? out_dim_actor : 1;
    const int k = threadIdx.x;
    const float* W1 = jb.net + off_W1(jb.in_dim);
    for (int cc = 0; cc < jb.in_dim; ++cc) atomicMax(&wm[cc], __float_as_int(fabsf(W1[k * jb.in_dim + cc])));
    atomicMax(&wm[3], __float_as_int(fabsf(jb.net[off_b1(jb.in_dim) + k])));
    for (int o = 0; o < out_dim; ++o) atomicMax(&wm[4 + o], __float_as_int(fabsf(jb.net[off_W3(jb.in_dim) + o * H + k])));
    __syncthreads();
    if (threadIdx.x < 8) meta->wmax[threadIdx.x] = __int_as_float(wm[threadIdx.x]);
  }
}

struct H2Item { int job, net, tp, netkey; };
__device__ __forceinline__ int pair_tiles(int rows) { return (rows + H2Cfg::TMP - 1) / H2Cfg::TMP; }
__device__ __forceinline__ H2Item decode_item_h2(const TcFwdJobs& jobs, const int* pbeg, int item) {
  H2Item it;
  it.job = 0;
  while (it.job + 1 < jobs.n && item >= pbeg[it.job + 1]) ++it.job;
  const int local = item - pbeg[it.job];
  const int tiles = pair_tiles(jobs.j[it.job].rows);
  it.net = local / tiles;
  it.tp = local % tiles;
  it.netkey = it.job * 64 + it.net;
  return it;
}

template <int IN, int OUT>
__global__ void __cluster_dims__(2, 1, 1) __launch_bounds__(H2Cfg::THREADS, 1) tc_fwd_h2_kernel(const TcFwdJobs jobs, int swap_b) {
  using C = H2Cfg;
  extern __shared__ __align__(1024) uint8_t sm[];
  uint8_t* Bs = sm + C::OFF_B;
  float4* w1p = reinterpret_cast<float4*>(sm + C::OFF_W1);
  float4* ebs = reinterpret_cast<float4*>(sm + C::OFF_EB);
  float2* efs = reinterpret_cast<float2*>(sm + C::OFF_EF);
  uint64_t* bars = reinterpret_cast<uint64_t*>(sm + C::OFF_BAR);
  uint64_t* full = bars;
  uint64_t* empty = bars + C::STAGES;
  uint64_t* tfull = bars + 2 * C::STAGES;
  uint64_t* tempty = tfull + 2;
  uint64_t* bload = tempty + 2;
  uint64_t* bready = bload + 1;
  uint64_t* drain = bready + 1;
  uint32_t* slot = reinterpret_cast<uint32_t*>(sm + C::OFF_SLOT);

  const int tid = threadIdx.x, warp = tid >> 5, lane = tid & 31;
  const uint32_t rank = cluster_ctarank();
  const bool leader = rank == 0;
  const int cluster_id = blockIdx.x >> 1, n_clusters = gridDim.x >> 1;

  int pbeg[4];
  int item_lo, item_hi;
  {
    long long cb[4];
    int wj[3];
    cb[0] = 0;
    pbeg[0] = 0;
    for (int j = 0; j < jobs.n; ++j) {
      pbeg[j + 1] = pbeg[j] + jobs.j[j].n_nets * pair_tiles(jobs.j[j].rows);
      wj[j] = jobs.j[j].h2 != nullptr ? (jobs.h2_cost > 0 ? jobs.h2_cost : FWD_H2_COST) : 10;
      cb[j + 1] = cb[j] + (long long)(pbeg[j + 1] - pbeg[j]) * wj[j];
    }
    auto item_at = [&](long long cost) {
      int j = 0;
      while (j + 1 < jobs.n && cost >= cb[j + 1]) ++j;
      const int it = pbeg[j] + (int)((cost - cb[j]) / wj[j]);
      return it < pbeg[j + 1] ? it : pbeg[j + 1];
    };
    const long long total_cost = cb[jobs.n];
    item_lo = cluster_id == 0 ? 0 : item_at(total_cost * cluster_id / n_clusters);
    item_hi = cluster_id == n_clusters - 1 ? pbeg[jobs.n] : item_at(total_cost * (cluster_id + 1) / n_clusters);
  }

  if (warp == C::MMA_WARP) {
    tmem_alloc2(slot, 512);
    if (lane == 0) {
      for (int s = 0; s < C::STAGES; ++s) { mbar_init(&full[s], 2 * C::NPW); mbar_init(&empty[s], 1); }
      for (int a = 0; a < 2; ++a) { mbar_init(&tfull[a], 1); mbar_init(&tempty[a], 2 * C::NEW); }
      mbar_init(bload, 1);
      mbar_init(bready, 2);
      mbar_init(drain, 1);
      fence_mbar_init();
    }
  }
  tc_fence_before();
  __syncthreads();
  cluster_sync_all();
  tc_fence_after();
  const uint32_t tmem = *slot;
  grid_dep_wait();

  if (warp == C::MMA_WARP) {
    const uint32_t idesc = instr_desc(FMT_F16, C::TMP, C::NP);
    const uint32_t b_lbo = C::NLOC * 16;
    const uint32_t b_base = smem_u32(Bs);
    int cur_key = -1;
    uint32_t nb = 0, nd = 0, tcount = 0;
    for (int item = item_lo; item < item_hi; ++item) {
      const H2Item ii = decode_item_h2(jobs, pbeg, item);
      if (ii.netkey != cur_key) {
        if (cur_key >= 0) {
          if (leader && elect_one()) umma_commit2(drain, 3);
          __syncwarp();
          mbar_wait_cluster(drain, nd & 1);
          ++nd;
        }
        const TcFwdJob& jb = jobs.j[ii.job];
        const uint8_t* src = jb.packed + (size_t)ii.net * C::PACKED_NET_BYTES + (size_t)(rank ^ (uint32_t)swap_b) * C::B_BYTES;
        if (elect_one()) {
          mbar_arrive_expect_tx(bload, C::B_BYTES);
          for (uint32_t o = 0; o < C::B_BYTES; o += 32768) bulk_g2s(Bs + o, src + o, 32768, bload);
        }
        __syncwarp();
        mbar_wait(bload, nb & 1);
        if (elect_one()) mbar_arrive_cluster(bready, 0);
        __syncwarp();
        if (leader) mbar_wait_cluster(bready, nb & 1);
        ++nb;
        cur_key = ii.netkey;
      }
      if (!leader) continue;
      for (int p = 0; p < C::PASSES; ++p) {
        mbar_wait_cluster(&tempty[p], (tcount & 1) ^ 1);
        tc_fence_after();
        const uint32_t d_tmem = tmem + p * C::NP;
        const uint32_t bp = b_base + p * C::B_PASS_BYTES;
        for (int c = 0; c < C::NCHUNK; ++c) {
          if (p == 0) {
            mbar_wait_cluster(&full[c], tcount & 1);
            tc_fence_after();
          }
          if (elect_one()) {
            const uint32_t a_stage = tmem + C::A_COL0 + c * C::A_STAGE_COLS;
#pragma unroll
            for (int j = 0; j < C::KC / C::UK; ++j) {
              const uint32_t g = c * (C::KC / C::UK) + j;
              const uint64_t b_hi = smem_desc(bp + 2 * g * b_lbo, b_lbo, 128);
              const uint64_t b_lo = smem_desc(bp + C::B_TERM_BYTES + 2 * g * b_lbo, b_lbo, 128);
              const uint32_t a_hi = a_stage + j * 8, a_lo = a_hi + C::A_LO_COLS;
              umma_ts2(d_tmem, a_lo, b_hi, idesc, (c == 0 && j == 0) ? 0u : 1u);
              umma_ts2(d_tmem, a_hi, b_lo, idesc, 1u);
              umma_ts2(d_tmem, a_hi, b_hi, idesc, 1u);
            }
            if (p == C::PASSES - 1) umma_commit2(&empty[c], 3);
            if (c == C::NCHUNK - 1) umma_commit2(&tfull[p], 3);
          }
          __syncwarp();
        }
      }
      ++tcount;
    }
  } else if (warp >= C::NEW) {
    const int pw = warp - C::NEW, ptid = tid - C::NEW * 32;
    const int kq = pw >> 2;
    const uint32_t lane_base = tmem + ((uint32_t)((warp & 3) * 32) << 16) + C::A_COL0 + kq * (C::KPW / 2);
    int cur_key = -1;
    float4 wm = make_float4(0.f, 0.f, 0.f, 0.f);
    uint32_t tcount = 0;
    auto load_x = [&](const H2Item& ni) {
      const TcFwdJob& nj = jobs.j[ni.job];
      const int r = ni.tp * C::TMP + (int)rank * TM + (warp & 3) * 32 + lane;
      return r < nj.rows ? __ldg(nj.X + r) : make_float4(0.f, 0.f, 0.f, 0.f);
    };
    float4 x_next = make_float4(0.f, 0.f, 0.f, 0.f);
    H2Item ii_next = item_lo < item_hi ? decode_item_h2(jobs, pbeg, item_lo) : H2Item{};
    for (int item = item_lo; item < item_hi; ++item, ++tcount) {
      const H2Item ii = ii_next;
      if (item + 1 < item_hi) ii_next = decode_item_h2(jobs, pbeg, item + 1);
      const TcFwdJob& jb = jobs.j[ii.job];
      if (ii.netkey != cur_key) {
        cur_key = ii.netkey;
        asm volatile("bar.sync 1, %0;" ::"n"(C::PROD_THREADS));
        const float* net = jb.params + (size_t)ii.net * NET_STRIDE;
        for (int pr = ptid; pr < H / 2; pr += C::PROD_THREADS) {
          const int k = 2 * pr;
          const float* wa = net + off_W1(IN) + k * IN;
          const float* wb = wa + IN;
          w1p[2 * pr] = make_float4(wa[0], wb[0], wa[1], wb[1]);
          w1p[2 * pr + 1] = make_float4(IN == 3 ? wa[2] : 0.f, IN == 3 ? wb[2] : 0.f, net[off_b1(IN) + k], net[off_b1(IN) + k + 1]);
        }
        const HMeta* meta = reinterpret_cast<const HMeta*>(jb.packed + (size_t)ii.net * C::PACKED_NET_BYTES + C::META_OFF);
        wm = make_float4(__ldg(&meta->wmax[0]), __ldg(&meta->wmax[1]), IN == 3 ? __ldg(&meta->wmax[2]) : 0.f, __ldg(&meta->wmax[3]));
        asm volatile("bar.sync 1, %0;" ::"n"(C::PROD_THREADS));
      }
      const float4 x = (item == item_lo) ? load_x(ii) : x_next;
      if (item + 1 < item_hi) x_next = load_x(ii_next);
      float sa, inv_sa;
      pow2_scale(h1_row_bound(x, wm), sa, inv_sa);
      const float2 xx = make_float2(x.x, x.x), xy = make_float2(x.y, x.y), xz = make_float2(x.z, x.z), ss = make_float2(sa, sa);
      for (int c = 0; c < C::NCHUNK; ++c) {
        uint32_t hi[C::KPW / 2], lo[C::KPW / 2];
#pragma unroll
        for (int pp = 0; pp < C::KPW / 2; ++pp) {
          const int pr = (c * C::KC + kq * C::KPW) / 2 + pp;
          const float4 wA = w1p[2 * pr], wB = w1p[2 * pr + 1];
          float2 v = ffma2(xx, make_float2(wA.x, wA.y), make_float2(wB.z, wB.w));
          v = ffma2(xy, make_float2(wA.z, wA.w), v);
          if (IN == 3) v = ffma2(xz, make_float2(wB.x, wB.y), v);
          split_h2_trunc_relu(fmul2(v, ss), hi[pp], lo[pp]);
        }
        mbar_wait_cluster(&empty[c], (tcount & 1) ^ 1);
        tc_fence_after();
        tmem_st8(lane_base + c * C::A_STAGE_COLS, hi);
        tmem_st8(lane_base + c * C::A_STAGE_COLS + C::A_LO_COLS, lo);
        tmem_st_wait();
        tc_fence_before();
        __syncwarp();
        if (lane == 0) mbar_arrive_cluster(&full[c], 0);
      }
    }
    if (item_hi > item_lo)
      for (int c = 0; c < C::NCHUNK; ++c) mbar_wait_cluster(&empty[c], (tcount & 1) ^ 1);
  } else {
    const int hh = warp >> 2, qw = warp & 3;
    int cur_key = -1;
    const int row_in_tile = (int)rank * TM + qw * 32 + lane;
    float4 wm = make_float4(0.f, 0.f, 0.f, 0.f);
    uint32_t tcount = 0;
    for (int item = item_lo; item < item_hi; ++item, ++tcount) {
      const H2Item ii = decode_item_h2(jobs, pbeg, item);
      const TcFwdJob& jb = jobs.j[ii.job];
      if (ii.netkey != cur_key) {
        cur_key = ii.netkey;
        asm volatile("bar.sync 2, 256;");
        const float* net = jb.params + (size_t)ii.net * NET_STRIDE;
        const HMeta* meta = reinterpret_cast<const HMeta*>(jb.packed + (size_t)ii.net * C::PACKED_NET_BYTES + C::META_OFF);
        {
          const int col = tid;
          const float inv_n = __ldg(&meta->inv_s[col]);
          ebs[col] = make_float4(net[off_b2(IN) + col], net[off_W3(IN) + col],
                                 OUT == 2 ? net[off_W3(IN) + H + col] : 0.f, inv_n);
          if (OUT == 1) {
            float* ef = reinterpret_cast<float*>(efs) + (col >> 1) * 4 + (col & 1);
            ef[0] = net[off_b2(IN) + col] / inv_n;
            ef[2] = net[off_W3(IN) + col] * inv_n;
          }
        }
        wm = make_float4(__ldg(&meta->wmax[0]), __ldg(&meta->wmax[1]), IN == 3 ? __ldg(&meta->wmax[2]) : 0.f, __ldg(&meta->wmax[3]));
        asm volatile("bar.sync 2, 256;");
      }
      const int row = ii.tp * C::TMP + row_in_tile;
      const float4 x = row < jb.rows ? __ldg(jb.X + row) : make_float4(0.f, 0.f, 0.f, 0.f);
      float sa, inv_sa;
      pow2_scale(h1_row_bound(x, wm), sa, inv_sa);
      const bool store_h2 = jb.h2 != nullptr;
      const int tiles64 = (jb.rows + 63) / 64;
#pragma unroll 1
      for (int p = 0; p < C::PASSES; ++p) {
        constexpr int NC = C::NP / 2;
        const int cb = p * C::NP + hh * NC;
        mbar_wait(&tfull[p], tcount & 1);
        tc_fence_after();
        float* h2row = store_h2 ? jb.h2 + (((size_t)ii.net * tiles64 + (row >> 6)) * H + cb) * 64 + (row & 63) : nullptr;
        const uint32_t t_acc = tmem + ((uint32_t)(qw * 32) << 16) + cb;
        float q0 = 0.f, q1 = 0.f;
        if (OUT == 1 && !store_h2) {
          const float2 isa2 = make_float2(inv_sa, inv_sa);
          const float4* ef4 = reinterpret_cast<const float4*>(efs) + (cb >> 1);
          float2 qa = make_float2(0.f, 0.f), qb = make_float2(0.f, 0.f);
#pragma unroll 1
          for (int c0 = 0; c0 < NC; c0 += 16) {
            float v[16];
            float4 e[8];
            tmem_ld16(t_acc + c0, v);
#pragma unroll
            for (int j = 0; j < 8; ++j) e[j] = ef4[(c0 >> 1) + j];
            tmem_ld_wait();
#pragma unroll
            for (int j = 0; j < 8; j += 2) {
              float2 ha = ffma2(make_float2(v[2 * j], v[2 * j + 1]), isa2, make_float2(e[j].x, e[j].y));
              float2 hb = ffma2(make_float2(v[2 * j + 2], v[2 * j + 3]), isa2, make_float2(e[j + 1].x, e[j + 1].y));
              ha.x = fmaxf(ha.x, 0.f); ha.y = fmaxf(ha.y, 0.f);
              hb.x = fmaxf(hb.x, 0.f); hb.y = fmaxf(hb.y, 0.f);
              qa = ffma2(ha, make_float2(e[j].z, e[j].w), qa);
              qb = ffma2(hb, make_float2(e[j + 1].z, e[j + 1].w), qb);
            }
          }
          q0 = (qa.x + qa.y) + (qb.x + qb.y);
        } else {
          const float4* ebg = ebs + cb;
          float q0b = 0.f, q1b = 0.f;
#pragma unroll 1
          for (int c0 = 0; c0 < NC; c0 += 8) {
            float v[8];
            float4 e[8];
            tmem_ld8(t_acc + c0, v);
#pragma unroll
            for (int i = 0; i < 8; ++i) e[i] = ebg[c0 + i];
            tmem_ld_wait();
#pragma unroll
            for (int i = 0; i < 8; i += 2) {
              const float ha = fmaxf(fmaf(v[i] * inv_sa, e[i].w, e[i].x), 0.f);
              const float hb = fmaxf(fmaf(v[i + 1] * inv_sa, e[i + 1].w, e[i + 1].x), 0.f);
              v[i] = ha;
              v[i + 1] = hb;
              q0 = fmaf(ha, e[i].y, q0);
              q0b = fmaf(hb, e[i + 1].y, q0b);
              if (OUT == 2) { q1 = fmaf(ha, e[i].z, q1); q1b = fmaf(hb, e[i + 1].z, q1b); }
            }
            if (store_h2 && (row >> 6) < tiles64) {
#pragma unroll
              for (int i = 0; i < 8; ++i) h2row[(size_t)(c0 + i) * 64] = v[i];
            }
          }
          q0 += q0b;
          q1 += q1b;
        }
        tc_fence_before();
        __syncwarp();
        if (lane == 0) mbar_arrive_cluster(&tempty[p], 0);
        if (row < jb.rows) {
          float* o = jb.out_part + (((size_t)ii.net * C::PARTS + p * 2 + hh) * jb.rows + row) * OUT;
          o[0] = q0;
          if (OUT == 2) o[1] = q1;
        }
      }
    }
  }
  tc_fence_before();
  __syncthreads();
  cluster_sync_all();
  if (warp == C::MMA_WARP) tmem_dealloc2(tmem, 512);
}


struct H2B1Cfg : H2Cfg {
  static constexpr uint32_t OFF_W3 = B_BYTES;
  static constexpr uint32_t OFF_EB = OFF_W3 + H * 8;
  static constexpr uint32_t OFF_IV = OFF_EB + PASSES * NP * 16;
  static constexpr uint32_t OFF_BAR = OFF_IV + PASSES * NP * 4;
  static constexpr uint32_t OFF_SLOT = OFF_BAR + 128;
  static constexpr uint32_t OFF_FLUSH = OFF_SLOT + 16;
  static constexpr uint32_t OFF_RED = OFF_FLUSH + 2 * 4 * 16 * 32 * 4;
  static constexpr int RED_LD = 34;
  static constexpr uint32_t RED_WARP_BYTES = 32 * RED_LD * 4 + 32 * 16;
  static constexpr uint32_t SMEM_BYTES = OFF_RED + NEW * RED_WARP_BYTES;
};

template <int IN, int OUT, bool WGRADS, bool DX>
__global__ void __cluster_dims__(2, 1, 1) __launch_bounds__(H2Cfg::THREADS, 1) tc_bwd1_h2_kernel(const Bwd1Job jb, int swap_b) {
  using C = H2B1Cfg;
  extern __shared__ __align__(1024) uint8_t sm[];
  uint8_t* Bs = sm + C::OFF_B;
  float2* w3s = reinterpret_cast<float2*>(sm + C::OFF_W3);
  float4* ebs = reinterpret_cast<float4*>(sm + C::OFF_EB);
  float* invs = reinterpret_cast<float*>(sm + C::OFF_IV);
  uint64_t* bars = reinterpret_cast<uint64_t*>(sm + C::OFF_BAR);
  uint64_t* full = bars;
  uint64_t* empty = bars + C::STAGES;
  uint64_t* tfull = bars + 2 * C::STAGES;
  uint64_t* tempty = tfull + 2;
  uint64_t* bload = tempty + 2;
  uint64_t* bready = bload + 1;
  uint64_t* drain = bready + 1;
  uint32_t* slot = reinterpret_cast<uint32_t*>(sm + C::OFF_SLOT);

  const int tid = threadIdx.x, warp = tid >> 5, lane = tid & 31;
  const uint32_t rank = cluster_ctarank();
  const bool leader = rank == 0;
  const int cluster_id = blockIdx.x >> 1, n_clusters = gridDim.x >> 1;
  const int tiles = pair_tiles(jb.rows);
  const int tiles64 = (jb.rows + 63) / 64;
  const int total = jb.n_nets * tiles;
  const int item_lo = (int)((long long)total * cluster_id / n_clusters);
  const int item_hi = (int)((long long)total * (cluster_id + 1) / n_clusters);

  if (warp == C::MMA_WARP) {
    tmem_alloc2(slot, 512);
    if (lane == 0) {
      for (int s = 0; s < C::STAGES; ++s) { mbar_init(&full[s], 2 * C::NPW); mbar_init(&empty[s], 1); }
      for (int a = 0; a < 2; ++a) { mbar_init(&tfull[a], 1); mbar_init(&tempty[a], 2 * C::NEW); }
      mbar_init(bload, 1);
      mbar_init(bready, 2);
      mbar_init(drain, 1);
      fence_mbar_init();
    }
  }
  tc_fence_before();
  __syncthreads();
  cluster_sync_all();
  tc_fence_after();
  const uint32_t tmem = *slot;
  grid_dep_wait();
  if (WGRADS) zero_small1_slots<IN>(jb, 2);

  if (warp == C::MMA_WARP) {
    const uint32_t idesc = instr_desc(FMT_F16, C::TMP, C::NP);
    const uint32_t b_lbo = C::NLOC * 16;
    const uint32_t b_base = smem_u32(Bs);
    int cur_net = -1;
    uint32_t nb = 0, nd = 0, tcount = 0;
    for (int item = item_lo; item < item_hi; ++item) {
      const int net_i = item / tiles;
      if (net_i != cur_net) {
        if (cur_net >= 0) {
          if (leader && elect_one()) umma_commit2(drain, 3);
          __syncwarp();
          mbar_wait_cluster(drain, nd & 1);
          ++nd;
        }
        const uint8_t* src = jb.packedT + (size_t)net_i * C::PACKED_NET_BYTES + (size_t)(rank ^ (uint32_t)swap_b) * C::B_BYTES;
        if (elect_one()) {
          mbar_arrive_expect_tx(bload, C::B_BYTES);
          for (uint32_t o = 0; o < C::B_BYTES; o += 32768) bulk_g2s(Bs + o, src + o, 32768, bload);
        }
        __syncwarp();
        mbar_wait(bload, nb & 1);
        if (elect_one()) mbar_arrive_cluster(bready, 0);
        __syncwarp();
        if (leader) mbar_wait_cluster(bready, nb & 1);
        ++nb;
        cur_net = net_i;
      }
      if (!leader) continue;
      for (int p = 0; p < C::PASSES; ++p) {
        mbar_wait_cluster(&tempty[p], (tcount & 1) ^ 1);
        tc_fence_after();
        const uint32_t d_tmem = tmem + p * C::NP;
        const uint32_t bp = b_base + p * C::B_PASS_BYTES;
        for (int c = 0; c < C::NCHUNK; ++c) {
          if (p == 0) {
            mbar_wait_cluster(&full[c], tcount & 1);
            tc_fence_after();
          }
          if (elect_one()) {
            const uint32_t a_stage = tmem + C::A_COL0 + c * C::A_STAGE_COLS;
#pragma unroll
            for (int j = 0; j < C::KC / C::UK; ++j) {
              const uint32_t g = c * (C::KC / C::UK) + j;
              const uint64_t b_hi = smem_desc(bp + 2 * g * b_lbo, b_lbo, 128);
              const uint64_t b_lo = smem_desc(bp + C::B_TERM_BYTES + 2 * g * b_lbo, b_lbo, 128);
              const uint32_t a_hi = a_stage + j * 8, a_lo = a_hi + C::A_LO_COLS;
              umma_ts2(d_tmem, a_lo, b_hi, idesc, (c == 0 && j == 0) ? 0u : 1u);
              umma_ts2(d_tmem, a_hi, b_lo, idesc, 1u);
              umma_ts2(d_tmem, a_hi, b_hi, idesc, 1u);
            }
            if (p == C::PASSES - 1) umma_commit2(&empty[c], 3);
            if (c == C::NCHUNK - 1) umma_commit2(&tfull[p], 3);
          }
          __syncwarp();
        }
      }
      ++tcount;
    }
  } else if (warp >= C::NEW) {
    const int pw = warp - C::NEW, ptid = tid - C::NEW * 32;
    const int kq = pw >> 2;
    const uint32_t lane_base = tmem + ((uint32_t)((warp & 3) * 32) << 16) + C::A_COL0 + kq * (C::KPW / 2);
    int cur_net = -1;
    float w3m0 = 0.f, w3m1 = 0.f;
    uint32_t tcount = 0;
    for (int item = item_lo; item < item_hi; ++item, ++tcount) {
      const int net_i = item / tiles, tp = item % tiles;
      if (net_i != cur_net) {
        cur_net = net_i;
        asm volatile("bar.sync 1, %0;" ::"n"(C::PROD_THREADS));
        const float* net = jb.params + (size_t)net_i * NET_STRIDE;
        for (int j = ptid; j < H; j += C::PROD_THREADS)
          w3s[j] = make_float2(net[off_W3(IN) + j], OUT == 2 ? net[off_W3(IN) + H + j] : 0.f);
        const HMeta* meta = reinterpret_cast<const HMeta*>(jb.packedT + (size_t)net_i * C::PACKED_NET_BYTES + C::META_OFF);
        w3m0 = __ldg(&meta->wmax[4]);
        w3m1 = OUT == 2 ? __ldg(&meta->wmax[5]) : 0.f;
        asm volatile("bar.sync 1, %0;" ::"n"(C::PROD_THREADS));
      }
      const int r = tp * C::TMP + (int)rank * TM + (warp & 3) * 32 + lane;
      const bool ok = r < jb.rows;
      float d0 = 0.f;
      if (OUT == 1 && DX && !WGRADS && jb.q_parts > 0) { if (ok) d0 = actor_dq_of<IN, OUT>(jb, net_i, r); }
      else if (ok) d0 = __ldg(jb.dOut + ((size_t)net_i * jb.rows + r) * OUT);
      const float d1 = (ok && OUT == 2) ? __ldg(jb.dOut + ((size_t)net_i * jb.rows + r) * OUT + 1) : 0.f;
      float sa, inv_sa;
      pow2_scale(fmaf(fabsf(d0), w3m0, fabsf(d1) * w3m1), sa, inv_sa);
      const float d0s = d0 * sa, d1s = d1 * sa;
      const int rc = ok ? r : 0;
      const float* h2r = jb.h2 + ((size_t)net_i * tiles64 + (rc >> 6)) * H * 64 + (rc & 63);
      float hn[C::KPW];
#pragma unroll
      for (int e = 0; e < C::KPW; ++e) hn[e] = __ldg(h2r + (size_t)(kq * C::KPW + e) * 64);
      for (int c = 0; c < C::NCHUNK; ++c) {
        const int j0 = c * C::KC + kq * C::KPW;
        float hv[C::KPW];
#pragma unroll
        for (int e = 0; e < C::KPW; ++e) hv[e] = hn[e];
        if (c + 1 < C::NCHUNK) {
#pragma unroll
          for (int e = 0; e < C::KPW; ++e) hn[e] = __ldg(h2r + (size_t)(j0 + C::KC + e) * 64);
        }
        uint32_t hi[C::KPW / 2], lo[C::KPW / 2];
#pragma unroll
        for (int e = 0; e < C::KPW; e += 2) {
          const float2 wa = w3s[j0 + e], wb = w3s[j0 + e + 1];
          float ga = d0s * wa.x, gb = d0s * wb.x;
          if (OUT == 2) { ga = fmaf(d1s, wa.y, ga); gb = fmaf(d1s, wb.y, gb); }
          split_h2_trunc(make_float2(hv[e] > 0.f ? ga : 0.f, hv[e + 1] > 0.f ? gb : 0.f), hi[e / 2], lo[e / 2]);
        }
        mbar_wait_cluster(&empty[c], (tcount & 1) ^ 1);
        tc_fence_after();
        tmem_st8(lane_base + c * C::A_STAGE_COLS, hi);
        tmem_st8(lane_base + c * C::A_STAGE_COLS + C::A_LO_COLS, lo);
        tmem_st_wait();
        tc_fence_before();
        __syncwarp();
        if (lane == 0) mbar_arrive_cluster(&full[c], 0);
      }
    }
    if (item_hi > item_lo)
      for (int c = 0; c < C::NCHUNK; ++c) mbar_wait_cluster(&empty[c], (tcount & 1) ^ 1);
  } else {
    constexpr int NC = C::NP / 2;
    constexpr int NCH = NC / 32;
    const int hh = warp >> 2, qw = warp & 3, gtid = tid & 127;
    float a_b[C::PASSES][NCH], a_w0[C::PASSES][NCH], a_w1[C::PASSES][NCH], a_w2[C::PASSES][NCH];
#pragma unroll
    for (int p = 0; p < C::PASSES; ++p)
#pragma unroll
      for (int q = 0; q < NCH; ++q) { a_b[p][q] = 0.f; a_w0[p][q] = 0.f; a_w1[p][q] = 0.f; a_w2[p][q] = 0.f; }
    float* flbuf = reinterpret_cast<float*>(sm + C::OFF_FLUSH) + hh * (4 * 16 * 32);
    float* red_t = reinterpret_cast<float*>(sm + C::OFF_RED + warp * C::RED_WARP_BYTES);
    float4* red_x = reinterpret_cast<float4*>(red_t + 32 * C::RED_LD);
    auto flush = [&](int net_i) {
      if (!WGRADS || net_i < 0) return;
#pragma unroll
      for (int p = 0; p < C::PASSES; ++p)
#pragma unroll
        for (int q = 0; q < NCH; ++q) {
          float* f = flbuf + (qw * 16 + (p * NCH + q) * 4) * 32 + lane;
          f[0] = a_w0[p][q]; f[32] = a_w1[p][q]; f[64] = a_w2[p][q]; f[96] = a_b[p][q];
          a_b[p][q] = 0.f; a_w0[p][q] = 0.f; a_w1[p][q] = 0.f; a_w2[p][q] = 0.f;
        }
      asm volatile("bar.sync %0, 128;" ::"r"(2 + hh));
      float* o = jb.small1 + ((size_t)net_i * jb.slots + blockIdx.x * 2 + hh) * SMALL_STRIDE;
      {
        const int pq = qw;
        float t0 = 0.f, t1 = 0.f, t2 = 0.f, t3 = 0.f;
#pragma unroll
        for (int w = 0; w < 4; ++w) {
          const float* f = flbuf + (w * 16 + pq * 4) * 32 + lane;
          t0 += f[0]; t1 += f[32]; t2 += f[64]; t3 += f[96];
        }
        const int k = (pq / NCH) * C::NP + hh * NC + (pq % NCH) * 32 + lane;
        o[k * IN + 0] = t0;
        o[k * IN + 1] = t1;
        if (IN == 3) o[k * IN + 2] = t2;
        o[H * IN + k] = t3;
      }
      asm volatile("bar.sync %0, 128;" ::"r"(2 + hh));
    };
    int cur_net = -1;
    float w3m0 = 0.f, w3m1 = 0.f;
    uint32_t tcount = 0;
    for (int item = item_lo; item < item_hi; ++item, ++tcount) {
      const int net_i = item / tiles, tp = item % tiles;
      if (net_i != cur_net) {
        flush(cur_net);
        cur_net = net_i;
        asm volatile("bar.sync 4, 256;");
        const float* net = jb.params + (size_t)net_i * NET_STRIDE;
        const HMeta* meta = reinterpret_cast<const HMeta*>(jb.packedT + (size_t)net_i * C::PACKED_NET_BYTES + C::META_OFF);
        {
          const int k = tid;
          float* e = reinterpret_cast<float*>(ebs) + (k >> 1) * 8 + (k & 1);
          e[0] = net[off_W1(IN) + k * IN];
          e[2] = net[off_W1(IN) + k * IN + 1];
          e[4] = IN == 3 ? net[off_W1(IN) + k * IN + 2] : 0.f;
          e[6] = net[off_b1(IN) + k];
          invs[k] = __ldg(&meta->inv_s[k]);
        }
        w3m0 = __ldg(&meta->wmax[4]);
        w3m1 = OUT == 2 ? __ldg(&meta->wmax[5]) : 0.f;
        asm volatile("bar.sync 4, 256;");
      }
      const int row = tp * C::TMP + (int)rank * TM + qw * 32 + lane;
      const bool ok = row < jb.rows;
      const float4 x = ok ? __ldg(jb.X + row) : make_float4(0.f, 0.f, 0.f, 0.f);
      float d0 = 0.f;
      if (OUT == 1 && DX && !WGRADS && jb.q_parts > 0) { if (ok) d0 = actor_dq_of<IN, OUT>(jb, net_i, row); }
      else if (ok) d0 = __ldg(jb.dOut + ((size_t)net_i * jb.rows + row) * OUT);
      const float d1 = (ok && OUT == 2) ? __ldg(jb.dOut + ((size_t)net_i * jb.rows + row) * OUT + 1) : 0.f;
      float sa, inv_sa;
      pow2_scale(fmaf(fabsf(d0), w3m0, fabsf(d1) * w3m1), sa, inv_sa);
      if (WGRADS) {
        __syncwarp();
        red_x[lane] = make_float4(x.x, x.y, x.z, 1.f);
      }
#pragma unroll
      for (int p = 0; p < C::PASSES; ++p) {
        const int cb = p * C::NP + hh * NC;
        const float4* ebg = ebs + cb;
        const float* ivg = invs + cb;
        mbar_wait(&tfull[p], tcount & 1);
        tc_fence_after();
        const uint32_t t_acc = tmem + ((uint32_t)(qw * 32) << 16) + cb;
        float dx0 = 0.f, dx1 = 0.f, dx2 = 0.f;
#pragma unroll
        for (int q = 0; q < NCH; ++q) {
          if (WGRADS) __syncwarp();
#pragma unroll 1
          for (int c8 = 0; c8 < 32; c8 += 8) {
            float v[8];
            float4 w[8];
            float iv[8];
            tmem_ld8(t_acc + q * 32 + c8, v);
#pragma unroll
            for (int i = 0; i < 8; ++i) w[i] = ebg[q * 32 + c8 + i];
            if (DX) {
              const float4 i0 = *reinterpret_cast<const float4*>(ivg + q * 32 + c8);
              const float4 i1 = *reinterpret_cast<const float4*>(ivg + q * 32 + c8 + 4);
              iv[0] = i0.x; iv[1] = i0.y; iv[2] = i0.z; iv[3] = i0.w; iv[4] = i1.x; iv[5] = i1.y; iv[6] = i1.z; iv[7] = i1.w;
            }
            tmem_ld_wait();
            const float2 xx2 = make_float2(x.x, x.x), xy2 = make_float2(x.y, x.y), xz2 = make_float2(x.z, x.z);
            const float2 isa2 = make_float2(inv_sa, inv_sa);
#pragma unroll
            for (int i = 0; i < 8; i += 2) {
              const float4 wa = w[i], wb = w[i + 1];
              float2 z = ffma2(xy2, make_float2(wa.z, wa.w), ffma2(xx2, make_float2(wa.x, wa.y), make_float2(wb.z, wb.w)));
              if (IN == 3) z = ffma2(xz2, make_float2(wb.x, wb.y), z);
              float2 vs = fmul2(make_float2(v[i], v[i + 1]), isa2);
              if (DX) vs = fmul2(vs, make_float2(iv[i], iv[i + 1]));
              const float2 d = make_float2(z.x > 0.f ? vs.x : 0.f, z.y > 0.f ? vs.y : 0.f);
              if (DX) {
                dx0 = fmaf(d.x, wa.x, dx0); dx0 = fmaf(d.y, wa.y, dx0);
                dx1 = fmaf(d.x, wa.z, dx1); dx1 = fmaf(d.y, wa.w, dx1);
                if (IN == 3) { dx2 = fmaf(d.x, wb.x, dx2); dx2 = fmaf(d.y, wb.y, dx2); }
              }
              if (WGRADS) *reinterpret_cast<float2*>(red_t + lane * C::RED_LD + c8 + i) = d;
            }
          }
          if (WGRADS) {
            __syncwarp();
            float2 s01 = make_float2(0.f, 0.f), s2b = make_float2(0.f, 0.f);
#pragma unroll 8
            for (int r = 0; r < 32; ++r) {
              const float dv = red_t[r * C::RED_LD + lane];
              const float4 xr = red_x[r];
              const float2 dd = make_float2(dv, dv);
              s01 = ffma2(dd, make_float2(xr.x, xr.y), s01);
              s2b = ffma2(dd, make_float2(xr.z, xr.w), s2b);
            }
            const float cs = DX ? 1.f : ivg[q * 32 + lane];
            a_w0[p][q] = fmaf(s01.x, cs, a_w0[p][q]); a_w1[p][q] = fmaf(s01.y, cs, a_w1[p][q]);
            a_w2[p][q] = fmaf(s2b.x, cs, a_w2[p][q]); a_b[p][q] = fmaf(s2b.y, cs, a_b[p][q]);
          }
        }
        tc_fence_before();
        __syncwarp();
        if (lane == 0) mbar_arrive_cluster(&tempty[p], 0);
        if (DX && ok)
          jb.dX_part[((size_t)net_i * C::PARTS + p * 2 + hh) * jb.rows + row] = make_float4(dx0, dx1, dx2, 0.f);
      }
    }
    flush(cur_net);
  }
  tc_fence_before();
  __syncthreads();
  cluster_sync_all();
  if (warp == C::MMA_WARP) tmem_dealloc2(tmem, 512);
}


struct B2PCfg {
  static constexpr int RS = 32;
  static constexpr int STAGES = 4;
  static constexpr int PROD_WARPS = 16;
  static constexpr int PROD_THREADS = PROD_WARPS * 32;
  static constexpr int MMA_WARP = PROD_WARPS;
  static constexpr int THREADS = PROD_THREADS + 32;
  static constexpr int HU = H / 2;
  static constexpr uint32_t B_TERM_BYTES = HU * RS * 2;
  static constexpr uint32_t B_STAGE_BYTES = 2 * B_TERM_BYTES;
  static constexpr uint32_t A_COL0 = 256, A_STAGE_COLS = RS, A_LO_COLS = RS / 2;
  static constexpr int SS_ROWS = 4 * RS;
  static constexpr uint32_t OFF_X = STAGES * B_STAGE_BYTES;
  static constexpr uint32_t OFF_SS = OFF_X + 3 * 2 * SS_ROWS * 4;
  static constexpr uint32_t OFF_INV = OFF_SS + 2 * 2 * SS_ROWS * 4;
  static constexpr uint32_t OFF_SMALL = OFF_INV + (HU + H) * 4;
  static constexpr uint32_t OFF_MAX = OFF_SMALL + 3 * HU * 16;
  static constexpr uint32_t OFF_BAR = OFF_MAX + 32;
  static constexpr uint32_t OFF_SLOT = OFF_BAR + (2 * STAGES + 1) * 8 + 8;
  static constexpr uint32_t BYTES = OFF_SLOT + 16;
};

template <int IN, int OUT>
__global__ void __cluster_dims__(2, 1, 1) __launch_bounds__(B2PCfg::THREADS, 1) tc_bwd2_h2_kernel(const Bwd2Job jb) {
  using C = B2PCfg;
  extern __shared__ __align__(1024) uint8_t sm[];
  float4* xs = reinterpret_cast<float4*>(sm + C::OFF_X);
  float* invA = reinterpret_cast<float*>(sm + C::OFF_INV);
  float* invB = invA + C::HU;
  float4* small_g = reinterpret_cast<float4*>(sm + C::OFF_SMALL);
  int* rmax = reinterpret_cast<int*>(sm + C::OFF_MAX);
  uint64_t* full = reinterpret_cast<uint64_t*>(sm + C::OFF_BAR);
  uint64_t* empty = full + C::STAGES;
  uint64_t* done = empty + C::STAGES;
  uint32_t* slot = reinterpret_cast<uint32_t*>(sm + C::OFF_SLOT);
  const int tid = threadIdx.x, warp = tid >> 5, lane = tid & 31;
  const uint32_t rank = cluster_ctarank();
  const bool leader = rank == 0;
  const int split = blockIdx.x >> 1, net_i = blockIdx.y;
  const float* net = jb.params + (size_t)net_i * NET_STRIDE;
  const int tiles64 = (jb.rows + 63) / 64;
  const int n_stage_total = (jb.rows + C::RS - 1) / C::RS;
  const int st_lo = (int)((long long)n_stage_total * split / jb.splits);
  const int st_hi = (int)((long long)n_stage_total * (split + 1) / jb.splits);

  if (warp == C::MMA_WARP) {
    tmem_alloc2(slot, 512);
    if (lane == 0) {
      for (int s = 0; s < C::STAGES; ++s) { mbar_init(&full[s], 2 * C::PROD_WARPS); mbar_init(&empty[s], 1); }
      mbar_init(done, 1);
      fence_mbar_init();
    }
  }
  if (tid < 8) rmax[tid] = 0;
  tc_fence_before();
  __syncthreads();
  cluster_sync_all();
  tc_fence_after();
  const uint32_t tmem = *slot;
  grid_dep_wait();

  if (warp == C::MMA_WARP) {
    if (leader) {
      const uint32_t idesc = instr_desc(FMT_F16, 256, 256);
      const uint32_t lbo = C::HU * 16;
      uint32_t it = 0;
      for (int sg = st_lo; sg < st_hi; ++sg, ++it) {
        const uint32_t s = it % C::STAGES;
        mbar_wait(&full[s], (it / C::STAGES) & 1);
        tc_fence_after();
        const uint32_t b_base = smem_u32(sm + s * C::B_STAGE_BYTES);
        const uint32_t a_stage = tmem + C::A_COL0 + s * C::A_STAGE_COLS;
        if (elect_one()) {
#pragma unroll
          for (int j = 0; j < C::RS / 16; ++j) {
            const uint64_t b_hi = smem_desc(b_base + 2 * j * lbo, lbo, 128);
            const uint64_t b_lo = smem_desc(b_base + C::B_TERM_BYTES + 2 * j * lbo, lbo, 128);
            const uint32_t a_hi = a_stage + j * 8, a_lo = a_hi + C::A_LO_COLS;
            umma_ts2(tmem, a_lo, b_hi, idesc, (it == 0 && j == 0) ? 0u : 1u);
            umma_ts2(tmem, a_hi, b_lo, idesc, 1u);
            umma_ts2(tmem, a_hi, b_hi, idesc, 1u);
          }
          umma_commit2(&empty[s], 3);
          if (sg == st_hi - 1) umma_commit2(done, 3);
        }
        __syncwarp();
      }
    }
  } else {
    const int u = (warp & 3) * 32 + lane, g = warp >> 2;
    const int t = (int)rank * C::HU + u;
    float w3[OUT];
#pragma unroll
    for (int o = 0; o < OUT; ++o) w3[o] = net[off_W3(IN) + o * H + t];
    const float w1x = net[off_W1(IN) + t * IN], w1y = net[off_W1(IN) + t * IN + 1];
    const float w1z = IN == 3 ? net[off_W1(IN) + t * IN + 2] : 0.f;
    const float b1v = net[off_b1(IN) + t];
    {
      float mx0 = 0.f, mx1 = 0.f, mx2 = 0.f, md0 = 0.f, md1 = 0.f;
      const int r_lo = st_lo * C::RS, r_hi = min(jb.rows, st_hi * C::RS);
      for (int r = r_lo + tid; r < r_hi; r += C::PROD_THREADS) {
        const float4 x = __ldg(jb.X + r);
        mx0 = fmaxf(mx0, fabsf(x.x)); mx1 = fmaxf(mx1, fabsf(x.y)); mx2 = fmaxf(mx2, fabsf(x.z));
        md0 = fmaxf(md0, fabsf(__ldg(jb.dOut + ((size_t)net_i * jb.rows + r) * OUT)));
        if (OUT == 2) md1 = fmaxf(md1, fabsf(__ldg(jb.dOut + ((size_t)net_i * jb.rows + r) * OUT + 1)));
      }
#pragma unroll
      for (int o = 16; o > 0; o >>= 1) {
        mx0 = fmaxf(mx0, __shfl_xor_sync(0xffffffffu, mx0, o)); mx1 = fmaxf(mx1, __shfl_xor_sync(0xffffffffu, mx1, o));
        mx2 = fmaxf(mx2, __shfl_xor_sync(0xffffffffu, mx2, o)); md0 = fmaxf(md0, __shfl_xor_sync(0xffffffffu, md0, o));
        md1 = fmaxf(md1, __shfl_xor_sync(0xffffffffu, md1, o));
      }
      if (lane == 0) {
        atomicMax(&rmax[0], __float_as_int(mx0)); atomicMax(&rmax[1], __float_as_int(mx1)); atomicMax(&rmax[2], __float_as_int(mx2));
        atomicMax(&rmax[3], __float_as_int(md0)); atomicMax(&rmax[4], __float_as_int(md1));
      }
      asm volatile("bar.sync 1, %0;" ::"n"(C::PROD_THREADS));
    }
    float sA, sB;
    {
      float ia, ib;
      float bA = fabsf(w3[0]) * __int_as_float(rmax[3]);
      if (OUT == 2) bA = fmaf(fabsf(w3[OUT - 1]), __int_as_float(rmax[4]), bA);
      pow2_scale(bA, sA, ia);
      const float bB = fmaf(fabsf(w1x), __int_as_float(rmax[0]), fmaf(fabsf(w1y), __int_as_float(rmax[1]),
                       fmaf(fabsf(w1z), __int_as_float(rmax[2]), fabsf(b1v))));
      pow2_scale(bB, sB, ib);
      if (g == 0) { invA[u] = ia; invB[t] = ib; }
      if (g == 1) {
        const int tp = (int)(rank ^ 1u) * C::HU + u;
        const float px = net[off_W1(IN) + tp * IN], py = net[off_W1(IN) + tp * IN + 1];
        const float pz = IN == 3 ? net[off_W1(IN) + tp * IN + 2] : 0.f;
        const float pb = fmaf(fabsf(px), __int_as_float(rmax[0]), fmaf(fabsf(py), __int_as_float(rmax[1]),
                         fmaf(fabsf(pz), __int_as_float(rmax[2]), fabsf(net[off_b1(IN) + tp]))));
        float ps, pi;
        pow2_scale(pb, ps, pi);
        invB[tp] = pi;
      }
    }
    float2 s_db2 = make_float2(0.f, 0.f), s_dw3[OUT];
    float s_db3[OUT];
#pragma unroll
    for (int o = 0; o < OUT; ++o) { s_dw3[o] = make_float2(0.f, 0.f); s_db3[o] = 0.f; }
    const uint32_t a_lane = tmem + ((uint32_t)((warp & 3) * 32) << 16) + C::A_COL0 + g * 4;
    float* sxx = reinterpret_cast<float*>(xs);
    float* sxy = sxx + 2 * C::SS_ROWS;
    float* sxz = sxy + 2 * C::SS_ROWS;
    float* sd0 = reinterpret_cast<float*>(sm + C::OFF_SS);
    float* sd1 = sd0 + 2 * C::SS_ROWS;
    auto h2_ptr = [&](int sg) {
      const int row0 = sg * C::RS + g * 8;
      return jb.h2 + (((size_t)net_i * tiles64 + (row0 >> 6)) * H + t) * 64 + (row0 & 63);
    };
    const float2 w1x2 = make_float2(w1x, w1x), w1y2 = make_float2(w1y, w1y), w1z2 = make_float2(w1z, w1z), b12 = make_float2(b1v, b1v);
    const float2 sA2 = make_float2(sA, sA), sB2 = make_float2(sB, sB);
    float4 xr = make_float4(0.f, 0.f, 0.f, 0.f);
    float dr[OUT];
#pragma unroll
    for (int o = 0; o < OUT; ++o) dr[o] = 0.f;
    const int r_end = min(jb.rows, st_hi * C::RS);
    auto fetch_rows = [&](int k) {
      if (tid < C::SS_ROWS) {
        const int r = (st_lo + 4 * k) * C::RS + tid;
        const bool ok = r < r_end;
        xr = ok ? __ldg(jb.X + r) : make_float4(0.f, 0.f, 0.f, 0.f);
#pragma unroll
        for (int o = 0; o < OUT; ++o) dr[o] = ok ? __ldg(jb.dOut + ((size_t)net_i * jb.rows + r) * OUT + o) : 0.f;
      }
    };
    const int n_st = st_hi - st_lo, n_ss = (n_st + 3) / 4;
    constexpr int AH = 2;
    float4 hs[AH][2];
#pragma unroll
    for (int i = 0; i < AH; ++i) hs[i][0] = hs[i][1] = make_float4(0.f, 0.f, 0.f, 0.f);
    auto fetch_h2 = [&](int sg, float4& a, float4& b) {
      const float* h2p = h2_ptr(sg);
      a = __ldg(reinterpret_cast<const float4*>(h2p));
      b = __ldg(reinterpret_cast<const float4*>(h2p) + 1);
    };
    if (n_st > 0) fetch_rows(0);
#pragma unroll
    for (int i = 0; i < AH; ++i)
      if (n_st > i) fetch_h2(st_lo + i, hs[i][0], hs[i][1]);
    uint32_t it = 0;
    for (int k = 0; k < n_ss; ++k) {
      const int buf = (k & 1) * C::SS_ROWS;
      if (tid < C::SS_ROWS) {
        sxx[buf + tid] = xr.x; sxy[buf + tid] = xr.y; sxz[buf + tid] = xr.z;
        sd0[buf + tid] = dr[0];
        if (OUT == 2) sd1[buf + tid] = dr[OUT - 1];
      }
      if (k + 1 < n_ss) fetch_rows(k + 1);
      asm volatile("bar.sync 1, %0;" ::"n"(C::PROD_THREADS));
#pragma unroll
      for (int q = 0; q < 4; ++q, ++it) {
        const int sg = st_lo + 4 * k + q;
        if (sg >= st_hi) break;
        const uint32_t s = it % C::STAGES;
        float4& h0 = hs[q % AH][0];
        float4& h1r = hs[q % AH][1];
        const float hv[8] = {h0.x, h0.y, h0.z, h0.w, h1r.x, h1r.y, h1r.z, h1r.w};
        if (sg + AH < st_hi) fetch_h2(sg + AH, h0, h1r);
        uint32_t ahi[4], alo[4], bhi[4], blo[4];
        const int rl0 = buf + q * C::RS + g * 8;
#pragma unroll
        for (int e = 0; e < 4; ++e) {
          const float2 d0 = *reinterpret_cast<const float2*>(sd0 + rl0 + 2 * e);
          const float2 hp = make_float2(hv[2 * e], hv[2 * e + 1]);
          float2 gs = fmul2(d0, make_float2(w3[0], w3[0]));
          s_dw3[0] = ffma2(d0, hp, s_dw3[0]);
          if (t == 0) s_db3[0] += d0.x + d0.y;
          if (OUT == 2) {
            const float2 d1 = *reinterpret_cast<const float2*>(sd1 + rl0 + 2 * e);
            gs = ffma2(d1, make_float2(w3[OUT - 1], w3[OUT - 1]), gs);
            s_dw3[OUT - 1] = ffma2(d1, hp, s_dw3[OUT - 1]);
            if (t == 0) s_db3[OUT - 1] += d1.x + d1.y;
          }
          const float2 dz = make_float2(hp.x > 0.f ? gs.x : 0.f, hp.y > 0.f ? gs.y : 0.f);
          s_db2.x += dz.x; s_db2.y += dz.y;
          const float2 xxp = *reinterpret_cast<const float2*>(sxx + rl0 + 2 * e);
          const float2 xyp = *reinterpret_cast<const float2*>(sxy + rl0 + 2 * e);
          float2 z = ffma2(xyp, w1y2, ffma2(xxp, w1x2, b12));
          if (IN == 3) z = ffma2(*reinterpret_cast<const float2*>(sxz + rl0 + 2 * e), w1z2, z);
          split_h2_trunc(fmul2(dz, sA2), ahi[e], alo[e]);
          split_h2_trunc_relu(fmul2(z, sB2), bhi[e], blo[e]);
        }
        mbar_wait(&empty[s], ((it / C::STAGES) & 1) ^ 1);
        tc_fence_after();
        tmem_st4(a_lane + s * C::A_STAGE_COLS, ahi);
        tmem_st4(a_lane + s * C::A_STAGE_COLS + C::A_LO_COLS, alo);
        uint8_t* Bst = sm + s * C::B_STAGE_BYTES + chunk_off(C::HU, u, g);
        *reinterpret_cast<uint4*>(Bst) = make_uint4(bhi[0], bhi[1], bhi[2], bhi[3]);
        *reinterpret_cast<uint4*>(Bst + C::B_TERM_BYTES) = make_uint4(blo[0], blo[1], blo[2], blo[3]);
        tmem_st_wait();
        fence_proxy_async_smem();
        tc_fence_before();
        __syncwarp();
        if (lane == 0) mbar_arrive_cluster(&full[s], 0);
      }
    }
    const float s_db2s = s_db2.x + s_db2.y;
    float s_dw3s[OUT];
#pragma unroll
    for (int o = 0; o < OUT; ++o) s_dw3s[o] = s_dw3[o].x + s_dw3[o].y;
    if (g > 0) small_g[(g - 1) * C::HU + u] = make_float4(s_db2s, s_dw3s[0], OUT == 2 ? s_dw3s[OUT - 1] : 0.f, s_db3[0]);
    if (OUT == 2 && t == 0 && g > 0) rmax[4 + g] = __float_as_int(s_db3[OUT - 1]);
    asm volatile("bar.sync 1, %0;" ::"n"(C::PROD_THREADS));
    if (g == 0) {
      float db3_1 = s_db3[OUT - 1];
      float a0 = s_db2s, a1 = s_dw3s[0], a2 = OUT == 2 ? s_dw3s[OUT - 1] : 0.f, a3 = s_db3[0];
// ... 52 lines not shown
```

### replay_cql_b200/csrc/update.cuh

```cuda
#pragma once
#include <algorithm>
#include <utility>
#include "engine.cuh"
#include "mlp_tc.cuh"
#include "mlp_tc_ts.cuh"
#include <type_traits>
#include "mlp_tc_bwd1.cuh"
#include "mlp_tc_bwd2.cuh"
#include "mlp_tc_h.cuh"
#include "mlp_tc_h2.cuh"
#include "adam_pack.cuh"

namespace cql {

__host__ __device__ inline uint32_t mix32(uint32_t x) {
  x ^= x >> 16; x *= 0x7feb352du; x ^= x >> 15; x *= 0x846ca68bu; x ^= x >> 16;
  return x;
}
__host__ __device__ inline uint64_t feistel_perm(uint64_t x, uint64_t n, uint64_t key) {
  int bits = 2;
  while (bits < 62 && (1ull << bits) < n) bits += 2;
  const int hb = bits / 2;
  const uint64_t mask = (1ull << hb) - 1;
  do {
// ... 498 lines not shown
  float lt = sums[8], la = sums[9];
  float mt = sums[10], vt = sums[11], ma = sums[12], va = sums[13];
  float g_t = g_scalars[0], g_a = g_scalars[1];
  if (dp.world > 1) {
    __shared__ float gsh[2];
    if (threadIdx.x == 0) dp_wait_scalars(dp, g_t, g_a, gsh[0], gsh[1]);
    __syncthreads();
    g_t = gsh[0];
    g_a = gsh[1];
  }
  if (k.temp_lr > 0.f) lt = adam_scalar(lt, g_t, mt, vt, k.temp_lr, k, *si);
  if (k.alpha_lr > 0.f) la = adam_scalar(la, g_a, ma, va, k.alpha_lr, k, *si);
  const float alpha = fminf(fmaxf(expf(la), 0.f), 1e6f);
  const float inv = 1.f / ((float)k.C * (float)k.B);
  const float coef = alpha * k.cw * inv;
  const int64_t i = (int64_t)blockIdx.x * blockDim.x + threadIdx.x;
  const int rsC = 3 * k.n + 1;
  if (i < (int64_t)k.C * k.B * rsC) {
    const int j = (int)(i % rsC);
    dQ[i] = j < rsC - 1 ? coef * dQ[i] : 2.f * pairv[i / rsC].err / (float)k.B - coef;
  }
  if (i == 0) {
    if (k.temp_lr > 0.f) { scalars[0] = lt; sc_m[0] = mt; sc_v[0] = vt; }
    if (k.alpha_lr > 0.f) { scalars[1] = la; sc_m[1] = ma; sc_v[1] = va; }
    sums[3] = coef;
    metrics[1] = expf(lt);
    metrics[3] = expf(la);
    const float td = sums[0] / (float)k.B;
    const float cons = alpha * (k.cw * (sums[1] * inv - sums[2] * inv) - k.thr);
    metrics[4] = td + cons;
    metrics[6] = td;
  }
  if (dp.world > 1) dp_consume_done(dp, 0, gridDim.x);
}

__global__ void __launch_bounds__(1024) k_actor_dq(const QSrc srcP, const float4* __restrict__ perb,
                                                   const float* __restrict__ scalars, int B, int C,
                                                   float* __restrict__ dQP, float* __restrict__ metrics) {
  tc::grid_dep_wait();
 
  __shared__ float red[32];
  const float T = expf(scalars[0]);
  float s = 0.f;
  for (int b = threadIdx.x; b < B; b += 1024) {
    int arg = 0;
    float qm = q_at(srcP, 0, b);
    for (int c = 1; c < C; ++c) {
      const float q = q_at(srcP, c, b);
      if (q < qm) { qm = q; arg = c; }
    }
    for (int c = 0; c < C; ++c) dQP[(int64_t)c * B + b] = c == arg ? -1.f / (float)B : 0.f;
    s += T * perb[b].y - qm;
  }
  s = block_sum<1024>(s, red);
  if (threadIdx.x == 0) metrics[5] = s / (float)B;
}

__global__ void k_actor_dout(const float* __restrict__ outA, const float* __restrict__ noise_actor,
                             const float4* __restrict__ dXP, const float* __restrict__ scalars, int B, int n_parts,
                             int squash, float* __restrict__ dOutA, const QSrc srcP, const float4* __restrict__ perb,
                             int C, float* __restrict__ part, unsigned int* __restrict__ ticket, float* __restrict__ metrics) {
  tc::grid_dep_wait();
 
  const int b = blockIdx.x * blockDim.x + threadIdx.x;
  if (srcP.q != nullptr) {
    float v = 0.f;
    if (b < B) {
      float qm = q_at(srcP, 0, b);
      for (int c = 1; c < C; ++c) qm = fminf(qm, q_at(srcP, c, b));
      v = expf(scalars[0]) * perb[b].y - qm;
    }
    v = warp_sum(v);
    if ((threadIdx.x & 31) == 0) part[b >> 5] = v;
    __shared__ bool last;
    __threadfence();
    __syncthreads();
    if (threadIdx.x == 0) {
      const unsigned int t = atomicAdd(ticket, 1u);
      last = t == gridDim.x - 1;
      if (last) *ticket = 0;
    }
    __syncthreads();
    if (last && threadIdx.x < 32) {
      __threadfence();
      const int n_w = (gridDim.x * blockDim.x) >> 5;
      float s = 0.f;
      for (int i = threadIdx.x; i < n_w; i += 32) s += part[i];
      s = warp_sum(s);
      if (threadIdx.x == 0) metrics[5] = s / (float)B;
    }
  }
  if (b >= B) return;
  float da = 0.f;
  for (int c = 0; c < n_parts; ++c) da += dXP[(int64_t)c * B + b].z;
  const float mu = outA[2 * b], ls_raw = outA[2 * b + 1], ls = clamp_ls(ls_raw);
  const float eps = noise_actor[b];
  const Sample s = policy_sample(mu, ls, eps, squash);
  const float w = __fdiv_rn(expf(scalars[0]), (float)B);
  const float one_m_a2 = __fsub_rn(1.f, __fmul_rn(s.a, s.a));
  const float dt_std = __fmul_rn(w, __fdiv_rn(s.t, s.std_));
  float g_tanh;
  if (squash == CQL_SQUASH_EPS) {
    const float g_a = __fadd_rn(da, __fmul_rn(w, __fdiv_rn(__fmul_rn(2.f, s.a), __fadd_rn(one_m_a2, 1e-6f))));
    g_tanh = __fmul_rn(g_a, one_m_a2);
  } else {
    const float sig = __fdiv_rn(1.f, __fadd_rn(1.f, expf(__fmul_rn(2.f, s.raw))));
    g_tanh = __fadd_rn(__fmul_rn(w, __fsub_rn(2.f, __fmul_rn(4.f, sig))), __fmul_rn(da, one_m_a2));
  }
  const float g_raw = __fadd_rn(g_tanh, -dt_std);
  const float g_mu = __fadd_rn(g_raw, dt_std);
  const float g_std = __fadd_rn(__fmul_rn(g_raw, eps), __fmul_rn(w, __fdiv_rn(__fmul_rn(s.t, s.t), s.std_)));
  const float g_ls = __fsub_rn(__fmul_rn(g_std, s.std_), w);
  dOutA[2 * b] = g_mu;
  dOutA[2 * b + 1] = (ls_raw >= -20.f && ls_raw <= 2.f) ? g_ls : 0.f;
}

__global__ void k_reduce_grads(const float* __restrict__ small, const float* __restrict__ pw2, int in_dim, int out_dim,
                               int tiles, int splits, float* __restrict__ grads) {
  const int net = blockIdx.y;
  const int idx = blockIdx.x * blockDim.x + threadIdx.x;
  if (idx >= NET_STRIDE) return;
  const int w2_lo = off_W2(in_dim), w2_hi = w2_lo + H * H, total = net_floats(in_dim, out_dim);
  float s = 0.f;
  if (idx >= w2_lo && idx < w2_hi) {
    const float* p = pw2 + (size_t)net * splits * H * H + (idx - w2_lo);
    for (int i = 0; i < splits; ++i) s += p[(size_t)i * H * H];
  } else if (idx < total) {
    const int sidx = idx < w2_lo ? idx : idx - H * H;
    const float* p = small + (size_t)net * tiles * SMALL_STRIDE + sidx;
    for (int i = 0; i < tiles; ++i) s += p[(size_t)i * SMALL_STRIDE];
  }
  grads[(size_t)net * NET_STRIDE + idx] = s;
}

__global__ void k_adam_polyak(float* __restrict__ p, float* __restrict__ m, float* __restrict__ v,
                              const float* __restrict__ g, float* __restrict__ targ, int64_t count, float lr,
                              float beta1, float beta2, float eps, float tau, const StepInfo* __restrict__ si) {
  tc::grid_dep_wait();
 
  const int64_t i = (int64_t)blockIdx.x * blockDim.x + threadIdx.x;
  if (i >= count) return;
  const float step_size = (float)((double)lr / si->bc1);
  const float bc2s = (float)si->bc2_sqrt;
  const float gi = g[i];
  const float mi = m[i] + (gi - m[i]) * (1.f - beta1);
  const float vi = v[i] * beta2 + (1.f - beta2) * gi * gi;
  m[i] = mi;
  v[i] = vi;
  const float pn = p[i] - step_size * (mi / (sqrtf(vi) / bc2s + eps));
  p[i] = pn;
  if (targ) targ[i] = targ[i] * (1.f - tau) + tau * pn;
}

struct LaunchMode { bool pdl; int skip; };
constexpr LaunchMode PLAIN{false, 0}, PDL{true, 0};
constexpr LaunchMode pdl_skip(int bit) { return LaunchMode{true, bit}; }

template <typename... KArgs, typename... Args>
inline void launch(Handle* h, cudaStream_t st, LaunchMode mode, void (*kernel)(KArgs...), dim3 grid, dim3 block,
                   size_t smem, Args&&... args) {
  if (switches().skip & mode.skip) return;
  cudaLaunchConfig_t cfg{};
  cfg.gridDim = grid; cfg.blockDim = block; cfg.dynamicSmemBytes = smem; cfg.stream = st;
  cudaLaunchAttribute attr[1];
  attr[0].id = cudaLaunchAttributeProgrammaticStreamSerialization;
  attr[0].val.programmaticStreamSerializationAllowed = 1;
  cfg.attrs = attr;
  cfg.numAttrs = mode.pdl && !switches().no_pdl && !h->pdl_off ? 1 : 0;
  CQL_CUDA(cudaLaunchKernelEx(&cfg, kernel, KArgs(std::forward<Args>(args))...));
  CQL_LAUNCH_CHECK(h);
}

enum class Prec { FP32, TF32X3, BF16, F16X3 };
template <typename F>
inline void with_precision(const Handle* h, F&& f) {
  switch (h->cfg.precision) {
    case CQL_PREC_FP32: f(std::integral_constant<Prec, Prec::FP32>{}); break;
    case CQL_PREC_TF32X3: f(std::integral_constant<Prec, Prec::TF32X3>{}); break;
    case CQL_PREC_BF16: f(std::integral_constant<Prec, Prec::BF16>{}); break;
    case CQL_PREC_F16X3: f(std::integral_constant<Prec, Prec::F16X3>{}); break;
    default: throw Error{"internal: bad precision"};
  }
}
template <Prec P>
using TcCfg = std::conditional_t<P == Prec::F16X3, tc::HCfg, tc::Cfg<P != Prec::BF16>>;

template <Prec P, int IN, int OUT>
inline void launch_fwd(Handle* h, FwdJobs& jobs, cudaStream_t st, QSrc* src) {
  if constexpr (P == Prec::FP32) {
    int t = 0;
    for (int i = 0; i < jobs.n; ++i) {
      jobs.j[i].tile_begin = t;
      t += tiles_of(jobs.j[i].rows) * jobs.j[i].n_nets;
    }
    jobs.total_tiles = t;
    if (t > 0) launch(h, st, PLAIN, mlp_fwd_kernel<IN, OUT>, dim3(t), dim3(NT), FWD_SMEM, jobs);
    for (int i = 0; i < jobs.n; ++i) src[i] = QSrc{jobs.j[i].out, jobs.j[i].params, 0, jobs.j[i].rows, IN, OUT};
  } else {
    constexpr bool F16X3 = P == Prec::F16X3;
    const Switches& sw = switches();
    tc::TcFwdJobs tj{};
    tj.n = jobs.n;
    int pair_items = 0, items128 = 0;
    for (int i = 0; i < jobs.n; ++i) {
      pair_items += jobs.j[i].n_nets * ((jobs.j[i].rows + 2 * tc::TM - 1) / (2 * tc::TM));
      items128 += jobs.j[i].n_nets * tc::HCfg::SLICES * ((jobs.j[i].rows + tc::TM - 1) / tc::TM);
    }
    const bool pair = F16X3 && !sw.no_pair && IN == 3 && pair_items >= h->num_sms / 2;
    const bool small = F16X3 && !pair && !sw.no_small && items128 * 2 <= h->num_sms;
    const int n_slices = small ? tc::HCfgS::SLICES : TcCfg<P>::SLICES;
    const int n_parts = pair ? tc::H2Cfg::PARTS : n_slices;
    size_t part_off = 0;
    int items = 0;
    float* part_of[4] = {nullptr, nullptr, nullptr, nullptr};
    for (int i = 0; i < jobs.n; ++i) {
      const FwdJob& j = jobs.j[i];
      const int slot = (int)((j.params - h->params) / NET_STRIDE);
      tj.item_begin[i] = items;
      items += j.n_nets * n_slices * ((j.rows + tc::TM - 1) / tc::TM);
      part_of[i] = h->part + part_off;
      part_off += (size_t)j.n_nets * n_parts * j.rows * OUT;
      tj.j[i] = tc::TcFwdJob{j.X, j.params,
                             pair ? h->packed_fwd2 + (size_t)slot * h->packed_net_bytes2 : h->packed_fwd + (size_t)slot * h->packed_net_bytes,
                             part_of[i], j.h2, j.rows, j.n_nets};
    }
    tj.item_begin[jobs.n] = items;
    tj.h2_cost = sw.h2_cost;
    CQL_REQUIRE(part_off <= h->part_floats, "internal: partial-sum scratch too small");
    if (items == 0) return;
    const int grid = items < h->num_sms ? items : h->num_sms;
    if constexpr (F16X3) {
      if (pair)
        launch(h, st, PDL, tc::tc_fwd_h2_kernel<IN, OUT>, dim3(2 * (h->num_sms / 2)), dim3(tc::H2Cfg::THREADS),
               tc::H2Cfg::SMEM_BYTES, tj, h->pair_swap_b);
      else if (small)
        launch(h, st, PDL, tc::tc_fwd_h_kernel<IN, OUT, tc::HCfgS>, dim3(grid), dim3(tc::HCfgS::THREADS), tc::HCfgS::SMEM_BYTES, tj);
      else
        launch(h, st, PDL, tc::tc_fwd_h_kernel<IN, OUT>, dim3(grid), dim3(tc::HCfg::THREADS), tc::HCfg::SMEM_BYTES, tj);
      for (int i = 0; i < jobs.n; ++i) src[i] = QSrc{part_of[i], jobs.j[i].params, n_parts, jobs.j[i].rows, IN, OUT};
    } else {
      if constexpr (P == Prec::TF32X3)
        launch(h, st, PLAIN, tc::tc_fwd_ts_kernel<IN, OUT>, dim3(grid), dim3(tc::TsCfg::THREADS), tc::TsCfg::SMEM_BYTES, tj);
      else
        launch(h, st, PLAIN, tc::tc_fwd_kernel<false, IN, OUT>, dim3(grid), dim3(tc::Pipe<false, tc::FWD_NPW>::THREADS),
               tc::FwdSmem<false, tc::FWD_NPW>::BYTES, tj);
      tc::SumJobs sj{};
      sj.n = jobs.n;
      int max_n = 0;
      for (int i = 0; i < jobs.n; ++i) {
        const FwdJob& j = jobs.j[i];
        sj.j[i] = {part_of[i], j.params, j.out, j.rows, j.n_nets};
        max_n = std::max(max_n, j.n_nets * j.rows * OUT);
        src[i] = QSrc{j.out, j.params, 0, j.rows, IN, OUT};
      }
      launch(h, st, PDL, tc::k_sum_partials_multi<IN, OUT>, dim3((max_n + 255) / 256, jobs.n), dim3(256), 0, sj, n_parts);
    }
  }
}

template <Prec P>
inline void pack_slots(Handle* h, const int* slots, int n_slots, cudaStream_t st) {
  if (P == Prec::FP32 || n_slots == 0) return;
  tc::PackJobs jobs{};
  for (int i = 0; i < n_slots; ++i) {
    const int slot = slots[i];
    const bool is_actor = slot == slot_actor() || slot == slot_targ_actor(h->C);
    const int in_dim = is_actor ? 2 : 3;
    jobs.j[jobs.n++] = {h->net_params(slot), h->packed_fwd + (size_t)slot * h->packed_net_bytes, in_dim, 0};
    if (slot <= h->C) jobs.j[jobs.n++] = {h->net_params(slot), h->packed_bwd + (size_t)slot * h->packed_net_bytes_bwd, in_dim, 1};
  }
  if constexpr (P == Prec::F16X3) {
    launch(h, st, PDL, tc::k_pack_multi_h, dim3(H * 32 / 256, jobs.n), dim3(256), 0, jobs, 2);
    tc::PackJobs jp{};
    for (int i = 0; i < n_slots; ++i) {
      const int slot = slots[i];
      const bool is_actor = slot == slot_actor() || slot == slot_targ_actor(h->C);
      if (is_actor) continue;
      jp.j[jp.n++] = {h->net_params(slot), h->packed_fwd2 + (size_t)slot * h->packed_net_bytes2, 3, 0};
      if (slot <= h->C) jp.j[jp.n++] = {h->net_params(slot), h->packed_bwd2 + (size_t)slot * h->packed_net_bytes2, 3, 1};
    }
    if (jp.n) launch(h, st, PDL, tc::k_pack_pair_h, dim3(H * 32 / 256, jp.n), dim3(256), 0, jp, 2);
  } else {
    constexpr bool TF32 = P == Prec::TF32X3;
    const int chunks = H * (H / tc::Cfg<TF32>::EPC);
    launch(h, st, PLAIN, tc::k_pack_multi<TF32>, dim3((chunks + 255) / 256, jobs.n), dim3(256), 0, jobs);
  }
}
template <Prec P>
inline void pack_weights(Handle* h, int slot, int n_slots, cudaStream_t st) {
  int slots[8];
  for (int i = 0; i < n_slots; ++i) slots[i] = slot + i;
  pack_slots<P>(h, slots, n_slots, st);
}

template <Prec P>
inline void pack_all_weights(Handle* h, cudaStream_t st) {
  if constexpr (P == Prec::F16X3)
    launch(h, st, PLAIN, tc::k_w2max_init, dim3(2 + 2 * h->C), dim3(256), 0, h->params, 2 + 2 * h->C, h->w2max);
  pack_weights<P>(h, slot_actor(), 1, st);
  pack_weights<P>(h, slot_critic(0), h->C, st);
  pack_weights<P>(h, slot_targ_actor(h->C), 1, st);
  pack_weights<P>(h, slot_targ_critic(h->C, 0), h->C, st);
}

template <Prec P>
inline bool fold_grads(const Handle* h) {
  const Switches& sw = switches();
  return P == Prec::F16X3 && !sw.no_fold && !sw.no_fused_adam && h->cfg.world_size <= 1 && h->dp.world <= 1;
}

inline BwdJob critic_bwd_job(Handle* h) {
  return BwdJob{h->XC, h->dQ, h->h2C, h->net_params(slot_critic(0)), h->smallC, nullptr, h->pw2C, h->B * (3 * h->n + 1),
                h->C, h->splitsC};
}
inline BwdJob actor_bwd_job(Handle* h) {
  return BwdJob{h->XA, h->dOutA, h->h2A, h->net_params(slot_actor()), h->smallA, nullptr, h->pw2A, h->B, 1, h->splitsA};
}

struct BwdPlan {
  bool pair = false, small = false, pair2 = false, fork = false, fold = false;
  int clusters1 = 0, grid1 = 0, slots1 = 0, splits = 0;
  const float4* dx = nullptr;
  int dx_parts = 0;
};
template <Prec P, int IN, int OUT, bool WGRADS, bool DX>
inline BwdPlan bwd_plan(const Handle* h, const BwdJob& jb) {
  BwdPlan p{};
  if constexpr (P == Prec::FP32) {
    p.splits = jb.splits;
    p.dx = jb.dX;
    p.dx_parts = jb.n_nets;
  } else {
    constexpr bool F16X3 = P == Prec::F16X3;
    const Switches& sw = switches();
    const int tiles = (jb.rows + tc::TM - 1) / tc::TM;
    const int items = jb.n_nets * TcCfg<P>::SLICES * tiles;
    p.pair = F16X3 && !sw.no_pair && !sw.no_pair_bwd1 && IN == 3 &&
             jb.n_nets * ((jb.rows + 2 * tc::TM - 1) / (2 * tc::TM)) >= h->num_sms / 2;
    p.small = F16X3 && !p.pair && !sw.no_small && items * 2 <= h->num_sms;
    const int n_slices = p.small ? tc::HCfgS::SLICES : TcCfg<P>::SLICES;
    const int items_s = jb.n_nets * n_slices * tiles;
    const bool may_fork = WGRADS && !sw.no_fork && !h->timing && h->side_stream != nullptr;
    const int fork_pairs = sw.big_fork >= 0 ? sw.big_fork : (h->num_sms / 2) * 30 / 74;
    p.clusters1 = (p.pair && may_fork && fork_pairs > 0 && fork_pairs < h->num_sms / 2) ? fork_pairs : h->num_sms / 2;
    p.grid1 = p.pair ? 2 * p.clusters1 : (items_s < h->num_sms ? items_s : h->num_sms);
    p.slots1 = (F16X3 ? 2 : 4) * p.grid1;
    p.dx = h->dX_part;
    p.dx_parts = jb.n_nets * (p.pair ? (int)tc::H2Cfg::PARTS : n_slices);
    p.fold = WGRADS && fold_grads<P>(h);
    constexpr int RS2 = F16X3 ? tc::B2HCfg::RS : tc::B2Cfg<P != Prec::BF16>::RS;
    const int n_stage = (jb.rows + RS2 - 1) / RS2;
    int splits = h->num_sms / jb.n_nets;
    if (splits > n_stage) splits = n_stage;
    if (splits > h->splits_tc) splits = h->splits_tc;
    if (splits < 1) splits = 1;
    if constexpr (F16X3) {
      p.pair2 = !sw.no_pair && !sw.no_pair_bwd2 && (p.pair || !sw.no_pair_bwd2_small);
      if (p.pair2) splits = std::max(1, std::min(n_stage, (h->num_sms / 2) / jb.n_nets));
      if (p.pair2 && p.pair && p.clusters1 < h->num_sms / 2)
        splits = std::max(1, (h->num_sms / 2 - p.clusters1) / jb.n_nets);
    }
    p.splits = splits;
    p.fork = may_fork && p.grid1 + (p.pair2 ? 2 : 1) * splits * jb.n_nets <= h->num_sms;
  }
  return p;
}

struct BwdMarks { int mid = -1, end = -1, done = -1; };

template <Prec P, int IN, int OUT, bool WGRADS, bool DX>
inline BwdPlan launch_bwd(Handle* h, const BwdJob& jb, float* grads_out, cudaStream_t st, BwdMarks mk = {}) {
  auto mark_at = [&](int i) { if (i >= 0) mark(h, st, i); };
  const BwdPlan p = bwd_plan<P, IN, OUT, WGRADS, DX>(h, jb);
  if constexpr (P == Prec::FP32) {
    launch(h, st, PLAIN, mlp_bwd1_kernel<IN, OUT, WGRADS, DX>, dim3(tiles_of(jb.rows) * jb.n_nets), dim3(NT), BWD1_SMEM, jb);
    mark_at(mk.mid);
    if (!WGRADS) return p;
    launch(h, st, PLAIN, mlp_bwd2_kernel<IN, OUT>, dim3(4, jb.splits, jb.n_nets), dim3(NT), BWD2_SMEM, jb);
    mark_at(mk.end);
    mark_at(mk.done);
    launch(h, st, PLAIN, k_reduce_grads, dim3((NET_STRIDE + 255) / 256, jb.n_nets), dim3(256), 0, jb.small, jb.pw2, IN, OUT,
           tiles_of(jb.rows), jb.splits, grads_out);
  } else {
    constexpr bool F16X3 = P == Prec::F16X3;
    const int slot = (int)((jb.params - h->params) / NET_STRIDE);
    if (WGRADS && !p.fold) CQL_CUDA(cudaMemsetAsync(h->small1, 0, (size_t)jb.n_nets * p.slots1 * SMALL_STRIDE * sizeof(float), st));
    tc::Bwd1Job j1{jb.X, jb.dOut, jb.h2, jb.params,
                   p.pair ? h->packed_bwd2 + (size_t)slot * h->packed_net_bytes2 : h->packed_bwd + (size_t)slot * h->packed_net_bytes_bwd,
                   h->small1, DX ? h->dX_part : nullptr, jb.rows, jb.n_nets, p.slots1};
    j1.q_part = jb.q_part; j1.q_parts = jb.q_parts; j1.dq_scale = jb.dq_scale;
    j1.zero_small1 = p.fold ? 1 : 0;
    cudaStream_t st2 = st;
    if (p.fork) {
      CQL_CUDA(cudaEventRecord(h->ev_fork, st));
      CQL_CUDA(cudaStreamWaitEvent(h->side_stream, h->ev_fork, 0));
      st2 = h->side_stream;
    }
    if constexpr (F16X3) {
      if (p.pair)
        launch(h, st, PDL, tc::tc_bwd1_h2_kernel<IN, OUT, WGRADS, DX>, dim3(2 * p.clusters1), dim3(tc::H2Cfg::THREADS),
               tc::H2B1Cfg::SMEM_BYTES, j1, h->pair_swap_b);
      else if (p.small)
        launch(h, st, PDL, tc::tc_bwd1_h_kernel<IN, OUT, WGRADS, DX, tc::HCfgS>, dim3(p.grid1), dim3(tc::HCfgS::THREADS),
               tc::HCfgS::SMEM_BYTES, j1);
      else
        launch(h, st, PDL, tc::tc_bwd1_h_kernel<IN, OUT, WGRADS, DX>, dim3(p.grid1), dim3(tc::HCfg::THREADS), tc::HCfg::SMEM_BYTES, j1);
    } else if constexpr (P == Prec::TF32X3) {
      launch(h, st, PLAIN, tc::tc_bwd1_ts_kernel<IN, OUT, WGRADS, DX>, dim3(p.grid1), dim3(tc::TsCfg::THREADS), tc::TsCfg::SMEM_BYTES, j1);
    } else {
      launch(h, st, PLAIN, tc::tc_bwd1_kernel<false, IN, OUT, WGRADS, DX>, dim3(p.grid1), dim3(tc::Pipe<false, tc::BWD1_NPW>::THREADS),
             tc::FwdSmem<false, tc::BWD1_NPW>::BYTES, j1);
    }
    mark_at(mk.mid);
    if (!WGRADS) return p;
    tc::Bwd2Job j2{jb.X, jb.dOut, jb.h2, jb.params, h->pw2_tc, h->small2, jb.rows, jb.n_nets, p.splits};
    if constexpr (F16X3) {
      if (p.pair2)
        launch(h, st2, PDL, tc::tc_bwd2_h2_kernel<IN, OUT>, dim3(2 * p.splits, jb.n_nets), dim3(tc::B2PCfg::THREADS), tc::B2PCfg::BYTES, j2);
      else
        launch(h, st2, PDL, tc::tc_bwd2_h_kernel<IN, OUT>, dim3(p.splits, jb.n_nets), dim3(tc::B2HCfg::THREADS), tc::B2HCfg::BYTES, j2);
    } else {
      constexpr bool TF32 = P == Prec::TF32X3;
      launch(h, st2, PLAIN, tc::tc_bwd2_kernel<TF32, IN, OUT>, dim3(p.splits, jb.n_nets), dim3(tc::B2_THREADS), tc::B2Cfg<TF32>::BYTES, j2);
    }
    if (p.fork) {
      CQL_CUDA(cudaEventRecord(h->ev_join, st2));
      CQL_CUDA(cudaStreamWaitEvent(st, h->ev_join, 0));
    }
    mark_at(mk.end);
    if (!p.fold)
      launch(h, st, pdl_skip(64), tc::k_reduce_grads_tc, dim3((NET_STRIDE / 4 + 31) / 32, jb.n_nets), dim3(256), 0, h->small1,
             p.slots1, h->small2, h->pw2_tc, p.splits, IN, OUT, grads_out, h->dp_fused ? h->dp : DpPeer{}, IN == 3 ? 1 : 2,
             (long long)(IN == 3 ? NET_STRIDE : 0));
    mark_at(mk.done);
  }
  return p;
}

struct NetGroup { int first_slot, n_nets, in_dim, out_dim; float lr; };
inline NetGroup critic_group(const Handle* h) { return NetGroup{slot_critic(0), h->C, 3, 1, h->cfg.critic_lr}; }
inline NetGroup actor_group(const Handle* h) { return NetGroup{slot_actor(), 1, 2, 2, h->cfg.actor_lr}; }

inline void adam_pack(Handle* h, const NetGroup& g, const BwdPlan& plan, cudaStream_t st, bool last) {
  const cql_config& c = h->cfg;
  const bool critic = g.in_dim == 3;
  tc::AdamPackJobs j{};
  j.in_dim = g.in_dim; j.out_dim = g.out_dim;
  j.lr = g.lr; j.beta1 = c.beta1; j.beta2 = c.beta2; j.eps = c.adam_eps; j.tau = c.tau;
  j.step_inc = last ? h->step_dev : nullptr;
  j.dp = h->dp_fused ? h->dp : DpPeer{};
  j.dp_group = critic ? 1 : 2;
  j.dp_off = (long long)g.first_slot * NET_STRIDE;
  for (int i = 0; i < g.n_nets; ++i) {
    const int slot = g.first_slot + i, tslot = slot + 1 + h->C;
    tc::AdamPackNet& n = j.n[i];
    n.p = h->net_params(slot);
    n.m = h->adam_m + (size_t)slot * NET_STRIDE;
    n.v = h->adam_v + (size_t)slot * NET_STRIDE;
    n.g = h->grads + (size_t)slot * NET_STRIDE;
    n.targ = h->net_params(tslot);
    n.fwd = h->packed_fwd + (size_t)slot * h->packed_net_bytes;
    n.bwd = h->packed_bwd + (size_t)slot * h->packed_net_bytes_bwd;
    n.tfwd = h->packed_fwd + (size_t)tslot * h->packed_net_bytes;
    n.fwd2 = critic ? h->packed_fwd2 + (size_t)slot * h->packed_net_bytes2 : nullptr;
    n.bwd2 = critic ? h->packed_bwd2 + (size_t)slot * h->packed_net_bytes2 : nullptr;
    n.tfwd2 = critic ? h->packed_fwd2 + (size_t)tslot * h->packed_net_bytes2 : nullptr;
    n.w2max = h->w2max + slot * 4;
  }
  if (plan.fold) {
    j.small1 = h->small1; j.small2 = h->small2; j.pw2 = h->pw2_tc;
    j.slots1 = plan.slots1; j.splits = plan.splits;
    j.wmax_acc = h->ap_wmax;
  }
  const int blocks = tc::AP_W2_BLOCKS + (plan.fold ? tc::ap_small_blocks(g.in_dim, g.out_dim) : 1);
  launch(h, st, pdl_skip(128), tc::k_adam_pack, dim3(blocks, g.n_nets), dim3(1024), 0, j, h->stepinfo);
}

template <Prec P>
inline void optimizer_step(Handle* h, const NetGroup& g, const BwdPlan& plan, cudaStream_t st, bool last) {
  if (P == Prec::F16X3 && !switches().no_fused_adam) {
    adam_pack(h, g, plan, st, last);
    return;
  }
  const cql_config& c = h->cfg;
  const int64_t cnt = (int64_t)g.n_nets * NET_STRIDE, off = (int64_t)g.first_slot * NET_STRIDE;
  const int tslot = g.first_slot + 1 + h->C;
  launch(h, st, PDL, k_adam_polyak, dim3((int)((cnt + 255) / 256)), dim3(256), 0, h->net_params(g.first_slot), h->adam_m + off,
         h->adam_v + off, h->grads + off, h->net_params(tslot), cnt, g.lr, c.beta1, c.beta2, c.adam_eps, c.tau, h->stepinfo);
  int slots[2 * CQL_MAX_CRITICS], n = 0;
  for (int i = 0; i < g.n_nets; ++i) slots[n++] = g.first_slot + i;
  if (g.in_dim == 3)
    for (int i = 0; i < g.n_nets; ++i) slots[n++] = tslot + i;
  pack_slots<P>(h, slots, n, st);
  if (last) launch(h, st, PDL, k_step_end, dim3(1), dim3(1), 0, h->step_dev);
}

inline LossConsts loss_consts(const Handle* h) {
  const cql_config& c = h->cfg;
  return LossConsts{h->B, h->n, h->C, c.gamma, c.conservative_weight, c.alpha_threshold,
                    c.temp_lr, c.alpha_lr, c.beta1, c.beta2, c.adam_eps, h->n_steps > 1 ? 1 : 0};
}

constexpr int TIMED_FWD_REPS = 4;
enum class BatchSource { Sampled, Provided };
enum class NoiseSource { Philox, Provided };

template <Prec P>
inline void phase0(Handle* h, cudaStream_t st, BatchSource bs, NoiseSource ns) {
  NvtxRange nvtx("cql.update.phase0: sample, actor forward, critic forwards, temp/alpha gradients");
  const int B = h->B, C = h->C, n3 = 3 * h->n;
  const cql_config& c = h->cfg;
  mark(h, st, 0);
  const float4* batch4 = reinterpret_cast<const float4*>(h->batch);
  if (bs == BatchSource::Sampled && ns == NoiseSource::Philox) {
    CQL_REQUIRE(h->n_trans > 0, "cql_update: no transitions loaded (call cql_load_transitions first)");
    const int64_t nthr = h->noise_floats > B ? h->noise_floats : B;
    launch(h, st, pdl_skip(256), k_step_head, dim3((int)((nthr + 255) / 256)), dim3(256), 0, reinterpret_cast<const float4*>(h->table),
           h->n_trans, h->step_dev, h->stepinfo, c.beta1, c.beta2, B, h->n, c.rank, c.world_size, c.seed,
           reinterpret_cast<float4*>(h->batch), h->XA, h->noise, h->noise_floats, h->table_sharded ? 0 : c.rank,
           h->table_sharded ? 1 : c.world_size, h->prep);
  } else {
    launch(h, st, PLAIN, k_step_begin, dim3(1), dim3(1), 0, h->step_dev, h->stepinfo, c.beta1, c.beta2);
    if (bs == BatchSource::Sampled) {
      CQL_REQUIRE(h->n_trans > 0, "cql_update: no transitions loaded (call cql_load_transitions first)");
      launch(h, st, PLAIN, k_sample, dim3((B + 127) / 128), dim3(128), 0, reinterpret_cast<const float4*>(h->table), h->n_trans,
             nullptr, h->step_dev, 0, B, (int64_t)B * (h->table_sharded ? 1 : c.world_size), h->table_sharded ? 0 : c.rank,
             h->table_sharded ? 1 : c.world_size, c.seed, reinterpret_cast<float4*>(h->staged_batch()));
    }
    if (ns == NoiseSource::Philox)
      launch(h, st, PLAIN, k_noise, dim3((int)((h->noise_floats + 255) / 256)), dim3(256), 0, h->noise, h->noise_floats, B, h->n,
             c.seed, h->step_dev, c.rank);
    launch(h, st, PLAIN, k_actor_rows, dim3((2 * B + 255) / 256), dim3(256), 0, reinterpret_cast<const float4*>(h->staged_batch()),
           B, reinterpret_cast<float4*>(h->batch), h->XA, h->prep);
  }
  {
    FwdJobs jobs{};
    jobs.n = 2;
    jobs.j[0] = FwdJob{h->XA, h->net_params(slot_actor()), h->outA, h->h2A, B, 1, 0};
    jobs.j[1] = FwdJob{h->XA + B, h->net_params(slot_actor()), h->outA + 2 * (size_t)B, nullptr, B, 1, 0};
    mark(h, st, 1);
    QSrc srcA[2];
    launch_fwd<P, 2, 2>(h, jobs, st, srcA);
    mark(h, st, 2);
    launch(h, st, pdl_skip(1), k_prep, dim3((B * 64 + 255) / 256), dim3(256), 0, batch4, srcA[0], srcA[1], h->outA, h->noise, B,
           h->n, c.squash, h->XAl, h->offAl, h->XC, h->offC, h->XT, h->XP, reinterpret_cast<float4*>(h->perb));
  }
  {
    FwdJobs jobs{};
    jobs.n = 3;
    jobs.j[0] = FwdJob{h->XAl, h->net_params(slot_critic(0)), h->QAl, nullptr, B * n3, C, 0};
    jobs.j[1] = FwdJob{h->XC, h->net_params(slot_critic(0)), h->QC, h->h2C, B * (n3 + 1), C, 0};
    jobs.j[2] = FwdJob{h->XT, h->net_params(slot_targ_critic(C, 0)), h->QT, nullptr, B, C, 0};
    mark(h, st, 3);
    QSrc srcQ[3];
    const bool pdl_off = h->pdl_off;
    for (int rep = 0; rep < (h->timing ? TIMED_FWD_REPS : 1); ++rep) {
      h->pdl_off = pdl_off && rep == 0;
      launch_fwd<P, 3, 1>(h, jobs, st, srcQ);
    }
    h->pdl_off = pdl_off;
    mark(h, st, 4);
    const int64_t so = scalars_off(C);
    ScalarReduceArgs ra{reinterpret_cast<const float4*>(h->perb), h->scalars(), h->adam_m + so, h->adam_v + so, h->g_scalars(),
                        h->loss_sums, h->metrics, reinterpret_cast<unsigned int*>(h->loss_sums + 15), h->dp_fused ? h->dp : DpPeer{}};
    launch(h, st, pdl_skip(2), k_lse, dim3((C * B * 32 + 255) / 256), dim3(256), 0, batch4, srcQ[0], h->offAl, srcQ[1], h->offC,
           srcQ[2], loss_consts(h), h->dQ, reinterpret_cast<PairVals*>(h->pairv), ra);
  }
}

template <Prec P>
inline void phase1(Handle* h, cudaStream_t st) {
  NvtxRange nvtx("cql.update.phase1: temp/alpha Adam, critic backward");
  const int B = h->B, C = h->C, rows = B * (3 * h->n + 1);
  const int64_t so = scalars_off(C);
  launch(h, st, pdl_skip(8), k_scalar_adam_dq, dim3((int)(((int64_t)C * rows + 255) / 256)), dim3(256), 0, h->scalars(),
         h->adam_m + so, h->adam_v + so, h->g_scalars(), h->stepinfo, loss_consts(h), h->loss_sums, h->metrics,
         reinterpret_cast<const PairVals*>(h->pairv), h->dQ, h->dp_fused ? h->dp : DpPeer{}, (long long)(1 + C) * NET_STRIDE);
  mark(h, st, 5);
  launch_bwd<P, 3, 1, true, false>(h, critic_bwd_job(h), h->g_critics(), st, BwdMarks{6, 7, -1});
}

template <Prec P>
inline void phase2(Handle* h, cudaStream_t st) {
  NvtxRange nvtx("cql.update.phase2: critic Adam + Polyak + pack, actor step forward/backward");
  const int B = h->B, C = h->C;
  optimizer_step<P>(h, critic_group(h), bwd_plan<P, 3, 1, true, false>(h, critic_bwd_job(h)), st, false);
  FwdJobs jobs{};
  jobs.n = 1;
  jobs.j[0] = FwdJob{h->XP, h->net_params(slot_critic(0)), h->QP, h->h2P, B, C, 0};
  mark(h, st, 8);
  QSrc srcP;
  launch_fwd<P, 3, 1>(h, jobs, st, &srcP);
  mark(h, st, 9);
  const bool fold_dq = srcP.n_parts > 0;
  const float4* perb = reinterpret_cast<const float4*>(h->perb);
  if (!fold_dq)
    launch(h, st, pdl_skip(16), k_actor_dq, dim3(1), dim3(1024), 0, srcP, perb, h->scalars(), B, C, h->dQP, h->metrics);
  BwdJob jd{h->XP, h->dQP, h->h2P, h->net_params(slot_critic(0)), nullptr, h->dXP, nullptr, B, C, 1};
  if (fold_dq) { jd.q_part = srcP.q; jd.q_parts = srcP.n_parts; jd.dq_scale = -1.f / (float)B; }
  const BwdPlan dx = launch_bwd<P, 3, 1, false, true>(h, jd, nullptr, st);
  launch(h, st, pdl_skip(32), k_actor_dout, dim3((B + 127) / 128), dim3(128), 0, h->outA, h->noise + B + 6 * (int64_t)B * h->n,
         dx.dx, h->scalars(), B, dx.dx_parts, h->cfg.squash, h->dOutA, fold_dq ? srcP : QSrc{}, perb, C, h->actor_part,
         reinterpret_cast<unsigned int*>(h->loss_sums + 14), h->metrics);
  mark(h, st, 10);
  launch_bwd<P, 2, 2, true, false>(h, actor_bwd_job(h), h->g_actor(), st, BwdMarks{-1, -1, 11});
}

template <Prec P>
inline void phase3(Handle* h, cudaStream_t st) {
  NvtxRange nvtx("cql.update.phase3: actor Adam + Polyak + pack");
  optimizer_step<P>(h, actor_group(h), bwd_plan<P, 2, 2, true, false>(h, actor_bwd_job(h)), st, true);
  mark(h, st, 12);
}

}
```

Baseline: 4999.

## Prefetch weight slices and per-net constants before PDL grid dependency wait

Tensor-core forward and backward kernels now issue the first weight-slice bulk load and the first net's W1/b1/W3 constants before grid_dep_wait, so these loads overlap the tail of the preceding kernel under programmatic dependent launch. The host tracks whether the previous launch wrote weights (pack, adam) and turns the early prefetch off in that case to avoid reading stale data. Loads use __ldcg so they bypass possibly stale non-coherent cache lines. The correctness risk is that the dependency tracking is based only on the last launch and a single flag.

Measured after the change: 5026 (median of 6 runs). Within noise of the previous version (+0.5%).

```diff
diff --git a/replay_cql_b200/csrc/engine.cuh b/replay_cql_b200/csrc/engine.cuh
--- a/replay_cql_b200/csrc/engine.cuh
+++ b/replay_cql_b200/csrc/engine.cuh
@@ -68,6 +68,7 @@
   int pair_swap;
   int dp_debug;
   bool no_fused_dp;
+  bool no_prefetch;
 };
 inline const Switches& switches() {
   static const Switches s = [] {
@@ -89,6 +90,7 @@
     w.pair_swap = num("CQL_PAIR_SWAP", 0);
     w.dp_debug = num("CQL_DP_DEBUG", 0);
     w.no_fused_dp = set("CQL_NO_FUSED_DP");
+    w.no_prefetch = set("CQL_NO_PREFETCH");
     return w;
   }();
   return s;
@@ -191,6 +193,7 @@
 
   bool timing = false;
   bool pdl_off = false;
+  bool last_wrote_weights = false;
   cudaEvent_t ev[16] = {};
 
   MdpSession* mdp = nullptr;
diff --git a/replay_cql_b200/csrc/mlp_tc.cuh b/replay_cql_b200/csrc/mlp_tc.cuh
--- a/replay_cql_b200/csrc/mlp_tc.cuh
+++ b/replay_cql_b200/csrc/mlp_tc.cuh
@@ -113,6 +113,7 @@
   int n;
   int item_begin[4];
   int h2_cost = 0;
+  int early = 0;
 };
 
 struct ItemInfo { int job, net, slice, tile, pair_id; };
diff --git a/replay_cql_b200/csrc/mlp_tc_bwd1.cuh b/replay_cql_b200/csrc/mlp_tc_bwd1.cuh
--- a/replay_cql_b200/csrc/mlp_tc_bwd1.cuh
+++ b/replay_cql_b200/csrc/mlp_tc_bwd1.cuh
@@ -18,6 +18,7 @@
   int q_parts = 0;
   float dq_scale = 0.f;
   int zero_small1 = 0;
+  int early = 0;
 };
 template <int IN>
 __device__ __forceinline__ void zero_small1_slots(const Bwd1Job& jb, int per_cta) {
diff --git a/replay_cql_b200/csrc/mlp_tc_bwd2.cuh b/replay_cql_b200/csrc/mlp_tc_bwd2.cuh
--- a/replay_cql_b200/csrc/mlp_tc_bwd2.cuh
+++ b/replay_cql_b200/csrc/mlp_tc_bwd2.cuh
@@ -34,6 +34,7 @@
   float* pw2;
   float* small2;
   int rows, n_nets, splits;
+  int early = 0;
 };
 
 template <bool TF32, int IN, int OUT>
diff --git a/replay_cql_b200/csrc/mlp_tc_h.cuh b/replay_cql_b200/csrc/mlp_tc_h.cuh
--- a/replay_cql_b200/csrc/mlp_tc_h.cuh
+++ b/replay_cql_b200/csrc/mlp_tc_h.cuh
@@ -170,6 +170,25 @@
   return fmaf(fabsf(x.x), wm.x, fmaf(fabsf(x.y), wm.y, fmaf(fabsf(x.z), wm.z, wm.w)));
 }
 
+template <int IN, int NT>
+__device__ __forceinline__ float4 load_fwd_consts(const float* net, const HMeta* meta, float4* w1p, int ptid) {
+  for (int pr = ptid; pr < H / 2; pr += NT) {
+    const int k = 2 * pr;
+    const float* wa = net + off_W1(IN) + k * IN;
+    const float* wb = wa + IN;
+    w1p[2 * pr] = make_float4(__ldcg(wa), __ldcg(wb), __ldcg(wa + 1), __ldcg(wb + 1));
+    w1p[2 * pr + 1] = make_float4(IN == 3 ? __ldcg(wa + 2) : 0.f, IN == 3 ? __ldcg(wb + 2) : 0.f, __ldcg(net + off_b1(IN) + k),
+                                  __ldcg(net + off_b1(IN) + k + 1));
+  }
+  return make_float4(__ldcg(&meta->wmax[0]), __ldcg(&meta->wmax[1]), IN == 3 ? __ldcg(&meta->wmax[2]) : 0.f, __ldcg(&meta->wmax[3]));
+}
+template <int IN, int OUT, int NT>
+__device__ __forceinline__ float2 load_bwd1_consts(const float* net, const HMeta* meta, float2* w3s, int ptid) {
+  for (int j = ptid; j < H; j += NT)
+    w3s[j] = make_float2(__ldcg(net + off_W3(IN) + j), OUT == 2 ? __ldcg(net + off_W3(IN) + H + j) : 0.f);
+  return make_float2(__ldcg(&meta->wmax[4]), OUT == 2 ? __ldcg(&meta->wmax[5]) : 0.f);
+}
+
 template <int IN, int OUT, class C = HCfg>
 __global__ void __launch_bounds__(HCfg::THREADS, 1) tc_fwd_h_kernel(const TcFwdJobs jobs) {
   extern __shared__ __align__(1024) uint8_t sm[];
@@ -220,9 +239,15 @@
   __syncthreads();
   tc_fence_after();
   const uint32_t tmem = *slot;
-  grid_dep_wait();
+  const bool pre = jobs.early && item_lo < item_hi;
 
   if (warp == C::MMA_WARP) {
+    if (pre) {
+      const HItem i0 = decode_item_h<C::SLICES>(jobs, item_lo);
+      if (elect_one()) load_operand_slice<C>(Bs, jobs.j[i0.job].packed + (size_t)i0.net * HCfg::PACKED_NET_BYTES, i0.slice, bload);
+      __syncwarp();
+    }
+    grid_dep_wait();
     const uint32_t idesc = instr_desc(FMT_F16, TM, C::NS);
     const uint32_t b_lbo = C::NS * 16;
     const uint32_t b_base = smem_u32(Bs);
@@ -238,7 +263,8 @@
           ++nd;
         }
         const TcFwdJob& jb = jobs.j[ii.job];
-        if (elect_one()) load_operand_slice<C>(Bs, jb.packed + (size_t)ii.net * HCfg::PACKED_NET_BYTES, ii.slice, bload);
+        if (!(pre && cur_pair < 0) && elect_one())
+          load_operand_slice<C>(Bs, jb.packed + (size_t)ii.net * HCfg::PACKED_NET_BYTES, ii.slice, bload);
         __syncwarp();
         mbar_wait(bload, nb & 1);
         ++nb;
@@ -277,6 +303,16 @@
     const uint32_t lane_base = tmem + ((uint32_t)((warp & 3) * 32) << 16) + C::A_COL0 + kq * (C::KPW / 2);
     int cur_netkey = -1;
     float4 wm = make_float4(0.f, 0.f, 0.f, 0.f);
+    if (pre) {
+      const HItem i0 = decode_item_h<C::SLICES>(jobs, item_lo);
+      const TcFwdJob& j0 = jobs.j[i0.job];
+      cur_netkey = i0.job * 64 + i0.net;
+      wm = load_fwd_consts<IN, C::PROD_THREADS>(
+          j0.params + (size_t)i0.net * NET_STRIDE,
+          reinterpret_cast<const HMeta*>(j0.packed + (size_t)i0.net * HCfg::PACKED_NET_BYTES + HCfg::META_OFF), w1p, ptid);
+      asm volatile("bar.sync 1, %0;" ::"n"(C::PROD_THREADS));
+    }
+    grid_dep_wait();
     uint32_t it = 0;
     auto load_x = [&](const HItem& ni) {
       const TcFwdJob& nj = jobs.j[ni.job];
@@ -293,16 +329,9 @@
       if (netkey != cur_netkey) {
         cur_netkey = netkey;
         asm volatile("bar.sync 1, %0;" ::"n"(C::PROD_THREADS));
-        const float* net = jb.params + (size_t)ii.net * NET_STRIDE;
-        for (int pr = ptid; pr < H / 2; pr += C::PROD_THREADS) {
-          const int k = 2 * pr;
-          const float* wa = net + off_W1(IN) + k * IN;
-          const float* wb = wa + IN;
-          w1p[2 * pr] = make_float4(wa[0], wb[0], wa[1], wb[1]);
-          w1p[2 * pr + 1] = make_float4(IN == 3 ? wa[2] : 0.f, IN == 3 ? wb[2] : 0.f, net[off_b1(IN) + k], net[off_b1(IN) + k + 1]);
-        }
-        const HMeta* meta = reinterpret_cast<const HMeta*>(jb.packed + (size_t)ii.net * HCfg::PACKED_NET_BYTES + HCfg::META_OFF);
-        wm = make_float4(__ldg(&meta->wmax[0]), __ldg(&meta->wmax[1]), IN == 3 ? __ldg(&meta->wmax[2]) : 0.f, __ldg(&meta->wmax[3]));
+        wm = load_fwd_consts<IN, C::PROD_THREADS>(
+            jb.params + (size_t)ii.net * NET_STRIDE,
+            reinterpret_cast<const HMeta*>(jb.packed + (size_t)ii.net * HCfg::PACKED_NET_BYTES + HCfg::META_OFF), w1p, ptid);
         asm volatile("bar.sync 1, %0;" ::"n"(C::PROD_THREADS));
       }
       const float4 x = (item == item_lo) ? load_x(ii) : x_next;
@@ -334,6 +363,7 @@
       }
     }
   } else {
+    grid_dep_wait();
     const int grp = warp >> 2, qw = warp & 3, gtid = tid & 127;
     float4* ebg = ebs + grp * C::NS;
     float2* efg = reinterpret_cast<float2*>(sm + C::OFF_FLUSH) + grp * C::NS;
@@ -456,6 +486,23 @@
   __syncthreads();
   tc_fence_after();
   const uint32_t tmem = *slot;
+  const bool pre = jb.early && item_lo < item_hi;
+  int pre_net = -1;
+  float2 pre_w3m = make_float2(0.f, 0.f);
+  if (pre) {
+    const int pair0 = item_lo / tiles, net0 = pair0 / C::SLICES;
+    if (warp == C::MMA_WARP) {
+      if (elect_one()) load_operand_slice<C>(Bs, jb.packedT + (size_t)net0 * HCfg::PACKED_NET_BYTES, pair0 % C::SLICES, bload);
+      __syncwarp();
+    } else if (warp >= C::NEW) {
+      pre_net = net0;
+      pre_w3m = load_bwd1_consts<IN, OUT, C::PROD_THREADS>(
+          jb.params + (size_t)net0 * NET_STRIDE,
+          reinterpret_cast<const HMeta*>(jb.packedT + (size_t)net0 * HCfg::PACKED_NET_BYTES + HCfg::META_OFF), w3s,
+          tid - C::NEW * 32);
+      asm volatile("bar.sync 1, %0;" ::"n"(C::PROD_THREADS));
+    }
+  }
   grid_dep_wait();
   if (WGRADS) zero_small1_slots<IN>(jb, 2);
 
@@ -469,7 +516,8 @@
       const int pair = item / tiles;
       if (pair != cur_pair) {
         if (cur_pair >= 0) { if (elect_one()) umma_commit(drain); __syncwarp(); mbar_wait(drain, nd & 1); ++nd; }
-        if (elect_one()) load_operand_slice<C>(Bs, jb.packedT + (size_t)(pair / C::SLICES) * HCfg::PACKED_NET_BYTES, pair % C::SLICES, bload);
+        if (!(pre && cur_pair < 0) && elect_one())
+          load_operand_slice<C>(Bs, jb.packedT + (size_t)(pair / C::SLICES) * HCfg::PACKED_NET_BYTES, pair % C::SLICES, bload);
         __syncwarp();
         mbar_wait(bload, nb & 1);
         ++nb;
@@ -506,20 +554,19 @@
     const int pw = warp - C::NEW, ptid = tid - C::NEW * 32;
     const int kq = pw >> 2;
     const uint32_t lane_base = tmem + ((uint32_t)((warp & 3) * 32) << 16) + C::A_COL0 + kq * (C::KPW / 2);
-    int cur_net = -1;
-    float w3m0 = 0.f, w3m1 = 0.f;
+    int cur_net = pre_net;
+    float w3m0 = pre_w3m.x, w3m1 = pre_w3m.y;
     uint32_t it = 0;
     for (int item = item_lo; item < item_hi; ++item) {
       const int pair = item / tiles, tile = item % tiles, net_i = pair / C::SLICES;
       if (net_i != cur_net) {
         cur_net = net_i;
         asm volatile("bar.sync 1, %0;" ::"n"(C::PROD_THREADS));
-        const float* net = jb.params + (size_t)net_i * NET_STRIDE;
-        for (int j = ptid; j < H; j += C::PROD_THREADS)
-          w3s[j] = make_float2(net[off_W3(IN) + j], OUT == 2 ? net[off_W3(IN) + H + j] : 0.f);
-        const HMeta* meta = reinterpret_cast<const HMeta*>(jb.packedT + (size_t)net_i * HCfg::PACKED_NET_BYTES + HCfg::META_OFF);
-        w3m0 = __ldg(&meta->wmax[4]);
-        w3m1 = OUT == 2 ? __ldg(&meta->wmax[5]) : 0.f;
+        const float2 w3m = load_bwd1_consts<IN, OUT, C::PROD_THREADS>(
+            jb.params + (size_t)net_i * NET_STRIDE,
+            reinterpret_cast<const HMeta*>(jb.packedT + (size_t)net_i * HCfg::PACKED_NET_BYTES + HCfg::META_OFF), w3s, ptid);
+        w3m0 = w3m.x;
+        w3m1 = w3m.y;
         asm volatile("bar.sync 1, %0;" ::"n"(C::PROD_THREADS));
       }
       const int r = tile * TM + (warp & 3) * 32 + lane;
diff --git a/replay_cql_b200/csrc/mlp_tc_h2.cuh b/replay_cql_b200/csrc/mlp_tc_h2.cuh
--- a/replay_cql_b200/csrc/mlp_tc_h2.cuh
+++ b/replay_cql_b200/csrc/mlp_tc_h2.cuh
@@ -205,6 +205,27 @@
   cluster_sync_all();
   tc_fence_after();
   const uint32_t tmem = *slot;
+  const bool pre = jobs.early && item_lo < item_hi;
+  int pre_key = -1;
+  float4 pre_wm = make_float4(0.f, 0.f, 0.f, 0.f);
+  if (pre) {
+    const H2Item i0 = decode_item_h2(jobs, pbeg, item_lo);
+    const TcFwdJob& j0 = jobs.j[i0.job];
+    const uint8_t* pnet = j0.packed + (size_t)i0.net * C::PACKED_NET_BYTES;
+    if (warp == C::MMA_WARP) {
+      if (elect_one()) {
+        const uint8_t* src = pnet + (size_t)(rank ^ (uint32_t)swap_b) * C::B_BYTES;
+        mbar_arrive_expect_tx(bload, C::B_BYTES);
+        for (uint32_t o = 0; o < C::B_BYTES; o += 32768) bulk_g2s(Bs + o, src + o, 32768, bload);
+      }
+      __syncwarp();
+    } else if (warp >= C::NEW) {
+      pre_key = i0.netkey;
+      pre_wm = load_fwd_consts<IN, C::PROD_THREADS>(j0.params + (size_t)i0.net * NET_STRIDE,
+                                                    reinterpret_cast<const HMeta*>(pnet + C::META_OFF), w1p, tid - C::NEW * 32);
+      asm volatile("bar.sync 1, %0;" ::"n"(C::PROD_THREADS));
+    }
+  }
   grid_dep_wait();
 
   if (warp == C::MMA_WARP) {
@@ -224,7 +245,7 @@
         }
         const TcFwdJob& jb = jobs.j[ii.job];
         const uint8_t* src = jb.packed + (size_t)ii.net * C::PACKED_NET_BYTES + (size_t)(rank ^ (uint32_t)swap_b) * C::B_BYTES;
-        if (elect_one()) {
+        if (!(pre && cur_key < 0) && elect_one()) {
           mbar_arrive_expect_tx(bload, C::B_BYTES);
           for (uint32_t o = 0; o < C::B_BYTES; o += 32768) bulk_g2s(Bs + o, src + o, 32768, bload);
         }
@@ -271,8 +292,8 @@
     const int pw = warp - C::NEW, ptid = tid - C::NEW * 32;
     const int kq = pw >> 2;
     const uint32_t lane_base = tmem + ((uint32_t)((warp & 3) * 32) << 16) + C::A_COL0 + kq * (C::KPW / 2);
-    int cur_key = -1;
-    float4 wm = make_float4(0.f, 0.f, 0.f, 0.f);
+    int cur_key = pre_key;
+    float4 wm = pre_wm;
     uint32_t tcount = 0;
     auto load_x = [&](const H2Item& ni) {
       const TcFwdJob& nj = jobs.j[ni.job];
@@ -288,16 +309,9 @@
       if (ii.netkey != cur_key) {
         cur_key = ii.netkey;
         asm volatile("bar.sync 1, %0;" ::"n"(C::PROD_THREADS));
-        const float* net = jb.params + (size_t)ii.net * NET_STRIDE;
-        for (int pr = ptid; pr < H / 2; pr += C::PROD_THREADS) {
-          const int k = 2 * pr;
-          const float* wa = net + off_W1(IN) + k * IN;
-          const float* wb = wa + IN;
-          w1p[2 * pr] = make_float4(wa[0], wb[0], wa[1], wb[1]);
-          w1p[2 * pr + 1] = make_float4(IN == 3 ? wa[2] : 0.f, IN == 3 ? wb[2] : 0.f, net[off_b1(IN) + k], net[off_b1(IN) + k + 1]);
-        }
-        const HMeta* meta = reinterpret_cast<const HMeta*>(jb.packed + (size_t)ii.net * C::PACKED_NET_BYTES + C::META_OFF);
-        wm = make_float4(__ldg(&meta->wmax[0]), __ldg(&meta->wmax[1]), IN == 3 ? __ldg(&meta->wmax[2]) : 0.f, __ldg(&meta->wmax[3]));
+        wm = load_fwd_consts<IN, C::PROD_THREADS>(
+            jb.params + (size_t)ii.net * NET_STRIDE,
+            reinterpret_cast<const HMeta*>(jb.packed + (size_t)ii.net * C::PACKED_NET_BYTES + C::META_OFF), w1p, ptid);
         asm volatile("bar.sync 1, %0;" ::"n"(C::PROD_THREADS));
       }
       const float4 x = (item == item_lo) ? load_x(ii) : x_next;
@@ -498,6 +512,27 @@
   cluster_sync_all();
   tc_fence_after();
   const uint32_t tmem = *slot;
+  const bool pre = jb.early && item_lo < item_hi;
+  int pre_net = -1;
+  float2 pre_w3m = make_float2(0.f, 0.f);
+  if (pre) {
+    const int net0 = item_lo / tiles;
+    const uint8_t* pnet = jb.packedT + (size_t)net0 * C::PACKED_NET_BYTES;
+    if (warp == C::MMA_WARP) {
+      if (elect_one()) {
+        const uint8_t* src = pnet + (size_t)(rank ^ (uint32_t)swap_b) * C::B_BYTES;
+        mbar_arrive_expect_tx(bload, C::B_BYTES);
+        for (uint32_t o = 0; o < C::B_BYTES; o += 32768) bulk_g2s(Bs + o, src + o, 32768, bload);
+      }
+      __syncwarp();
+    } else if (warp >= C::NEW) {
+      pre_net = net0;
+      pre_w3m = load_bwd1_consts<IN, OUT, C::PROD_THREADS>(jb.params + (size_t)net0 * NET_STRIDE,
+                                                           reinterpret_cast<const HMeta*>(pnet + C::META_OFF), w3s,
+                                                           tid - C::NEW * 32);
+      asm volatile("bar.sync 1, %0;" ::"n"(C::PROD_THREADS));
+    }
+  }
   grid_dep_wait();
   if (WGRADS) zero_small1_slots<IN>(jb, 2);
 
@@ -517,7 +552,7 @@
           ++nd;
         }
         const uint8_t* src = jb.packedT + (size_t)net_i * C::PACKED_NET_BYTES + (size_t)(rank ^ (uint32_t)swap_b) * C::B_BYTES;
-        if (elect_one()) {
+        if (!(pre && cur_net < 0) && elect_one()) {
           mbar_arrive_expect_tx(bload, C::B_BYTES);
           for (uint32_t o = 0; o < C::B_BYTES; o += 32768) bulk_g2s(Bs + o, src + o, 32768, bload);
         }
@@ -564,20 +599,19 @@
     const int pw = warp - C::NEW, ptid = tid - C::NEW * 32;
     const int kq = pw >> 2;
     const uint32_t lane_base = tmem + ((uint32_t)((warp & 3) * 32) << 16) + C::A_COL0 + kq * (C::KPW / 2);
-    int cur_net = -1;
-    float w3m0 = 0.f, w3m1 = 0.f;
+    int cur_net = pre_net;
+    float w3m0 = pre_w3m.x, w3m1 = pre_w3m.y;
     uint32_t tcount = 0;
     for (int item = item_lo; item < item_hi; ++item, ++tcount) {
       const int net_i = item / tiles, tp = item % tiles;
       if (net_i != cur_net) {
         cur_net = net_i;
         asm volatile("bar.sync 1, %0;" ::"n"(C::PROD_THREADS));
-        const float* net = jb.params + (size_t)net_i * NET_STRIDE;
-        for (int j = ptid; j < H; j += C::PROD_THREADS)
-          w3s[j] = make_float2(net[off_W3(IN) + j], OUT == 2 ? net[off_W3(IN) + H + j] : 0.f);
-        const HMeta* meta = reinterpret_cast<const HMeta*>(jb.packedT + (size_t)net_i * C::PACKED_NET_BYTES + C::META_OFF);
-        w3m0 = __ldg(&meta->wmax[4]);
-        w3m1 = OUT == 2 ? __ldg(&meta->wmax[5]) : 0.f;
+        const float2 w3m = load_bwd1_consts<IN, OUT, C::PROD_THREADS>(
+            jb.params + (size_t)net_i * NET_STRIDE,
+            reinterpret_cast<const HMeta*>(jb.packedT + (size_t)net_i * C::PACKED_NET_BYTES + C::META_OFF), w3s, ptid);
+        w3m0 = w3m.x;
+        w3m1 = w3m.y;
         asm volatile("bar.sync 1, %0;" ::"n"(C::PROD_THREADS));
       }
       const int r = tp * C::TMP + (int)rank * TM + (warp & 3) * 32 + lane;
@@ -835,7 +869,19 @@
   cluster_sync_all();
   tc_fence_after();
   const uint32_t tmem = *slot;
+  const int t = (int)rank * C::HU + (warp & 3) * 32 + lane;
+  float w3[OUT], w1x = 0.f, w1y = 0.f, w1z = 0.f, b1v = 0.f;
+  auto load_unit = [&] {
+#pragma unroll
+    for (int o = 0; o < OUT; ++o) w3[o] = __ldcg(net + off_W3(IN) + o * H + t);
+    w1x = __ldcg(net + off_W1(IN) + t * IN);
+    w1y = __ldcg(net + off_W1(IN) + t * IN + 1);
+    w1z = IN == 3 ? __ldcg(net + off_W1(IN) + t * IN + 2) : 0.f;
+    b1v = __ldcg(net + off_b1(IN) + t);
+  };
+  if (jb.early && warp != C::MMA_WARP) load_unit();
   grid_dep_wait();
+  if (!jb.early && warp != C::MMA_WARP) load_unit();
 
   if (warp == C::MMA_WARP) {
     if (leader) {
@@ -866,13 +912,6 @@
     }
   } else {
     const int u = (warp & 3) * 32 + lane, g = warp >> 2;
-    const int t = (int)rank * C::HU + u;
-    float w3[OUT];
-#pragma unroll
-    for (int o = 0; o < OUT; ++o) w3[o] = net[off_W3(IN) + o * H + t];
-    const float w1x = net[off_W1(IN) + t * IN], w1y = net[off_W1(IN) + t * IN + 1];
-    const float w1z = IN == 3 ? net[off_W1(IN) + t * IN + 2] : 0.f;
-    const float b1v = net[off_b1(IN) + t];
     {
       float mx0 = 0.f, mx1 = 0.f, mx2 = 0.f, md0 = 0.f, md1 = 0.f;
       const int r_lo = st_lo * C::RS, r_hi = min(jb.rows, st_hi * C::RS);
diff --git a/replay_cql_b200/csrc/update.cuh b/replay_cql_b200/csrc/update.cuh
--- a/replay_cql_b200/csrc/update.cuh
+++ b/replay_cql_b200/csrc/update.cuh
@@ -674,9 +674,9 @@
   if (targ) targ[i] = targ[i] * (1.f - tau) + tau * pn;
 }
 
-struct LaunchMode { bool pdl; int skip; };
-constexpr LaunchMode PLAIN{false, 0}, PDL{true, 0};
-constexpr LaunchMode pdl_skip(int bit) { return LaunchMode{true, bit}; }
+struct LaunchMode { bool pdl; int skip; bool weights = false; };
+constexpr LaunchMode PLAIN{false, 0}, PDL{true, 0}, PLAIN_W{false, 0, true}, PDL_W{true, 0, true};
+constexpr LaunchMode pdl_skip(int bit, bool weights = false) { return LaunchMode{true, bit, weights}; }
 
 template <typename... KArgs, typename... Args>
 inline void launch(Handle* h, cudaStream_t st, LaunchMode mode, void (*kernel)(KArgs...), dim3 grid, dim3 block,
@@ -691,7 +691,10 @@
   cfg.numAttrs = mode.pdl && !switches().no_pdl && !h->pdl_off ? 1 : 0;
   CQL_CUDA(cudaLaunchKernelEx(&cfg, kernel, KArgs(std::forward<Args>(args))...));
   CQL_LAUNCH_CHECK(h);
-}
+  h->last_wrote_weights = mode.weights;
+}
+
+inline int prefetch_ok(const Handle* h) { return !switches().no_prefetch && !h->last_wrote_weights ? 1 : 0; }
 
 enum class Prec { FP32, TF32X3, BF16, F16X3 };
 template <typename F>
@@ -748,6 +751,7 @@
     }
     tj.item_begin[jobs.n] = items;
     tj.h2_cost = sw.h2_cost;
+    tj.early = prefetch_ok(h);
     CQL_REQUIRE(part_off <= h->part_floats, "internal: partial-sum scratch too small");
     if (items == 0) return;
     const int grid = items < h->num_sms ? items : h->num_sms;
@@ -792,7 +796,7 @@
     if (slot <= h->C) jobs.j[jobs.n++] = {h->net_params(slot), h->packed_bwd + (size_t)slot * h->packed_net_bytes_bwd, in_dim, 1};
   }
   if constexpr (P == Prec::F16X3) {
-    launch(h, st, PDL, tc::k_pack_multi_h, dim3(H * 32 / 256, jobs.n), dim3(256), 0, jobs, 2);
+    launch(h, st, PDL_W, tc::k_pack_multi_h, dim3(H * 32 / 256, jobs.n), dim3(256), 0, jobs, 2);
     tc::PackJobs jp{};
     for (int i = 0; i < n_slots; ++i) {
       const int slot = slots[i];
@@ -801,11 +805,11 @@
       jp.j[jp.n++] = {h->net_params(slot), h->packed_fwd2 + (size_t)slot * h->packed_net_bytes2, 3, 0};
       if (slot <= h->C) jp.j[jp.n++] = {h->net_params(slot), h->packed_bwd2 + (size_t)slot * h->packed_net_bytes2, 3, 1};
     }
-    if (jp.n) launch(h, st, PDL, tc::k_pack_pair_h, dim3(H * 32 / 256, jp.n), dim3(256), 0, jp, 2);
+    if (jp.n) launch(h, st, PDL_W, tc::k_pack_pair_h, dim3(H * 32 / 256, jp.n), dim3(256), 0, jp, 2);
   } else {
     constexpr bool TF32 = P == Prec::TF32X3;
     const int chunks = H * (H / tc::Cfg<TF32>::EPC);
-    launch(h, st, PLAIN, tc::k_pack_multi<TF32>, dim3((chunks + 255) / 256, jobs.n), dim3(256), 0, jobs);
+    launch(h, st, PLAIN_W, tc::k_pack_multi<TF32>, dim3((chunks + 255) / 256, jobs.n), dim3(256), 0, jobs);
   }
 }
 template <Prec P>
@@ -818,7 +822,7 @@
 template <Prec P>
 inline void pack_all_weights(Handle* h, cudaStream_t st) {
   if constexpr (P == Prec::F16X3)
-    launch(h, st, PLAIN, tc::k_w2max_init, dim3(2 + 2 * h->C), dim3(256), 0, h->params, 2 + 2 * h->C, h->w2max);
+    launch(h, st, PLAIN_W, tc::k_w2max_init, dim3(2 + 2 * h->C), dim3(256), 0, h->params, 2 + 2 * h->C, h->w2max);
   pack_weights<P>(h, slot_actor(), 1, st);
   pack_weights<P>(h, slot_critic(0), h->C, st);
   pack_weights<P>(h, slot_targ_actor(h->C), 1, st);
@@ -912,6 +916,7 @@
                    h->small1, DX ? h->dX_part : nullptr, jb.rows, jb.n_nets, p.slots1};
     j1.q_part = jb.q_part; j1.q_parts = jb.q_parts; j1.dq_scale = jb.dq_scale;
     j1.zero_small1 = p.fold ? 1 : 0;
+    j1.early = prefetch_ok(h);
     cudaStream_t st2 = st;
     if (p.fork) {
       CQL_CUDA(cudaEventRecord(h->ev_fork, st));
@@ -935,7 +940,7 @@
     }
     mark_at(mk.mid);
     if (!WGRADS) return p;
-    tc::Bwd2Job j2{jb.X, jb.dOut, jb.h2, jb.params, h->pw2_tc, h->small2, jb.rows, jb.n_nets, p.splits};
+    tc::Bwd2Job j2{jb.X, jb.dOut, jb.h2, jb.params, h->pw2_tc, h->small2, jb.rows, jb.n_nets, p.splits, prefetch_ok(h)};
     if constexpr (F16X3) {
       if (p.pair2)
         launch(h, st2, PDL, tc::tc_bwd2_h2_kernel<IN, OUT>, dim3(2 * p.splits, jb.n_nets), dim3(tc::B2PCfg::THREADS), tc::B2PCfg::BYTES, j2);
@@ -995,7 +1000,7 @@
     j.wmax_acc = h->ap_wmax;
   }
   const int blocks = tc::AP_W2_BLOCKS + (plan.fold ? tc::ap_small_blocks(g.in_dim, g.out_dim) : 1);
-  launch(h, st, pdl_skip(128), tc::k_adam_pack, dim3(blocks, g.n_nets), dim3(1024), 0, j, h->stepinfo);
+  launch(h, st, pdl_skip(128, true), tc::k_adam_pack, dim3(blocks, g.n_nets), dim3(1024), 0, j, h->stepinfo);
 }
 
 template <Prec P>
@@ -1007,7 +1012,7 @@
   const cql_config& c = h->cfg;
   const int64_t cnt = (int64_t)g.n_nets * NET_STRIDE, off = (int64_t)g.first_slot * NET_STRIDE;
   const int tslot = g.first_slot + 1 + h->C;
-  launch(h, st, PDL, k_adam_polyak, dim3((int)((cnt + 255) / 256)), dim3(256), 0, h->net_params(g.first_slot), h->adam_m + off,
+  launch(h, st, PDL_W, k_adam_polyak, dim3((int)((cnt + 255) / 256)), dim3(256), 0, h->net_params(g.first_slot), h->adam_m + off,
          h->adam_v + off, h->grads + off, h->net_params(tslot), cnt, g.lr, c.beta1, c.beta2, c.adam_eps, c.tau, h->stepinfo);
   int slots[2 * CQL_MAX_CRITICS], n = 0;
   for (int i = 0; i < g.n_nets; ++i) slots[n++] = g.first_slot + i;
```
